# USDA-ARS-GBRU/itsxpress

Measured on AMD Instinct MI355X. Metric: reads/sec trimmed (ITS2, stand-in taxon Tracheophyta for Fungi), higher is better.
Workload: dtype u8+f32

## Files before the change

### include/itsx_hip.h

```cpp
#ifndef ITSX_HIP_H
#define ITSX_HIP_H
#include <stdint.h>

#ifdef __cplusplus
extern "C" {
#endif

#define ITSX_ABI_VERSION 6

enum {
  ITSX_OK            =  0,
  ITSX_E_ARG         = -1,
  ITSX_E_IO          = -2,
  ITSX_E_FORMAT      = -3,
  ITSX_E_DEVICE      = -4,
  ITSX_E_UNSUPPORTED = -5,
  ITSX_E_COLLISION   = -6,
  ITSX_E_NOMEM       = -7
};

typedef struct itsx_ctx itsx_ctx;
typedef struct itsx_stream itsx_stream;
typedef struct itsx_keyset itsx_keyset;
typedef struct itsx_twriter itsx_twriter;
// ... 158 lines not shown
int itsx_keep_pair_records(itsx_ctx *ctx, int on);
int itsx_write_trimmed_paired_samples(itsx_ctx *ctx, const char *const *out1_paths, const char *const *out2_paths, int32_t n_samples,
                                      int compression, int trim_ccs, const char *left_prefix, const char *right_prefix,
                                      const int32_t *start, const int32_t *stop, const int32_t *tlen, int64_t *n_written_per_sample);
int64_t itsx_deflate_block_bytes(void);
int64_t itsx_deflate_bound(int64_t nbytes, int32_t n_ranges);
int itsx_deflate_device(itsx_ctx *ctx, const char *text, int64_t nbytes, const int64_t *bounds, int32_t n_ranges, char *out, int64_t out_cap,
                        int64_t *out_bounds);
int itsx_inflate_device(itsx_ctx *ctx, const char *gz, int64_t nbytes, int64_t *text_len, int64_t *n_members);
int itsx_inflate_fetch(itsx_ctx *ctx, char *out, int64_t out_cap);
int itsx_debug_inflate_host(const char *gz, int64_t nbytes, char *out, int64_t out_cap, int64_t *text_len, int64_t *n_members, int32_t *reason);
int64_t itsx_debug_inflate_candidates(const char *gz, int64_t nbytes, int64_t *positions, int64_t cap);
int itsx_debug_inflate_where(itsx_ctx *ctx, int64_t *where, int64_t n);
int itsx_set_device_inflate(itsx_ctx *ctx, int on);
int itsx_parse_device(itsx_ctx *ctx, const char *text, int64_t nbytes, int keep_qual, int64_t *n_records);
#define ITSX_PARSE_OFF 0
#define ITSX_PARSE_TOFF 1
#define ITSX_PARSE_SEQ 2
#define ITSX_PARSE_QUAL 3
#define ITSX_PARSE_TITLES 4
int itsx_parse_fetch(itsx_ctx *ctx, int32_t plane, int64_t lo, int64_t hi, void *out);
int itsx_debug_parse_host(const char *text, int64_t nbytes, int64_t *off, int64_t *toff, int64_t cap_records, char *seq, char *qual, int64_t cap_bases,
                          char *titles, int64_t cap_titles, int64_t *n_records, int64_t *n_bases, int64_t *n_title_bytes, int32_t *reason, int64_t *bad_record);
int itsx_parse_pairs_device(itsx_ctx *ctx, const char *text1, int64_t nbytes1, const char *text2, int64_t nbytes2, int64_t *n_pairs, int32_t *flags, int64_t *max_total);
int itsx_parse_pairs_fetch(itsx_ctx *ctx, int32_t side, int32_t plane, int64_t lo, int64_t hi, void *out);
int itsx_debug_parse_pairs_host(const char *text1, int64_t nbytes1, const char *text2, int64_t nbytes2, int64_t *off1, int64_t *toff1, char *seq1, char *qual1, char *titles1,
                                int64_t *off2, int64_t *toff2, char *seq2, char *qual2, char *titles2, int64_t cap_records, int64_t cap_bases, int64_t cap_titles,
                                int64_t *n_pairs, int64_t *sizes, int32_t *flags, int64_t *max_total, int32_t *reason, int32_t *bad_side, int64_t *bad_record);
int itsx_debug_pair_pass_host(char *seq, const char *qual, int64_t nbytes, int32_t *flags);
int itsx_set_device_parse(itsx_ctx *ctx, int on);
int itsx_debug_huffman_lengths(const uint32_t *freq, int32_t n, int32_t maxbits, uint8_t *lengths);

int itsx_derep(itsx_ctx *ctx, int strand_both, int minseqlength, int64_t *n_unique);
int itsx_cluster(itsx_ctx *ctx, double id, int strand_both, int64_t *n_unique);
int itsx_cluster_multi(itsx_ctx *ctx, itsx_ctx *const *helpers, int32_t n_helpers, double id, int strand_both, int64_t *n_unique);
int itsx_get_cluster(const itsx_ctx *ctx, double *pct_id, int64_t *order, int64_t *n_order);
int itsx_cluster_samples(itsx_ctx *ctx, double id, int strand_both, int64_t *n_unique);
int itsx_align_clusters(itsx_ctx *ctx, int64_t *n_aligned, float *ms_kernels);
int itsx_get_cluster_cigars(const itsx_ctx *ctx, int64_t *offs , char *text);
int itsx_get_derep(const itsx_ctx *ctx, int64_t *rep_of, int8_t *strand, int64_t *uniq_of);
int itsx_unique_keys(itsx_ctx *ctx, uint64_t seed, uint64_t *fwd, uint64_t *rc);
int itsx_set_active_uniques(itsx_ctx *ctx, const uint8_t *active);
int itsx_get_uniques(const itsx_ctx *ctx, int64_t *seed_read, int64_t *abundance);

int itsx_search(itsx_ctx *ctx, double T, double F1, double F2, double F3);
enum { ITSX_ROWS_FULL = 0, ITSX_ROWS_COMPACT = 1, ITSX_ROWS_LAZY = 2 };
int itsx_set_rows_mode(itsx_ctx *ctx, int mode);
int itsx_set_kept_rows(itsx_ctx *ctx, int on);
int64_t itsx_lazy_pending(const itsx_ctx *ctx);
int itsx_lazy_pending_profiles(const itsx_ctx *ctx, int32_t *flags);
int itsx_lazy_pending_uniques(itsx_ctx *ctx, uint8_t *flags);
int itsx_set_partial_coords(itsx_ctx *ctx, int on);
int itsx_lazy_complete(itsx_ctx *ctx, const int32_t *flags);
int64_t itsx_domz_count(const itsx_ctx *ctx);
int itsx_get_domz(const itsx_ctx *ctx, int64_t *domZ );
int itsx_set_domz(itsx_ctx *ctx, const int64_t *domZ );
int itsx_search_finalize(itsx_ctx *ctx, double domE);
int64_t itsx_num_domains(const itsx_ctx *ctx);
int itsx_get_domains(const itsx_ctx *ctx, itsx_domain *rows );
int itsx_align_domains(itsx_ctx *ctx, int64_t *n_aligned, float *ms_kernels);
int itsx_get_alignments(const itsx_ctx *ctx, itsx_alignment *out );
int64_t itsx_num_pairtraces(const itsx_ctx *ctx);
int itsx_get_pairtraces(const itsx_ctx *ctx, itsx_pairtrace *rows, int64_t row_size);

int itsx_trim_coords(itsx_ctx *ctx, const char *left_prefix, const char *right_prefix,
                     int32_t *start, int32_t *stop, int32_t *tlen, int32_t *in_ddict);
int itsx_rep_coords(itsx_ctx *ctx, const char *left_prefix, const char *right_prefix,
                    int32_t *start, int32_t *stop, int32_t *tlen, int32_t *in_ddict);

int itsx_domz_device(itsx_ctx *ctx, int64_t **d_domz, int64_t *n);
int itsx_trim_coords_device(itsx_ctx *ctx, const char *left_prefix, const char *right_prefix, int32_t **d_rows, int64_t *n_rows);
int itsx_rep_coords_device(itsx_ctx *ctx, const char *left_prefix, const char *right_prefix, int32_t **d_rows, int64_t *n_rows);
int itsx_derep_device(itsx_ctx *ctx, const int32_t **d_rep_of, const int32_t **d_uniq_of, const int8_t **d_strand, const int32_t **d_seed_read);
int itsx_unique_keys128_device(itsx_ctx *ctx, uint64_t seed_a, uint64_t seed_b, int64_t gidx_base, int64_t **d_tuples, int64_t *n_unique);
int itsx_unique_keys128(itsx_ctx *ctx, uint64_t seed_a, uint64_t seed_b, int64_t gidx_base, int64_t *tuples);

int itsx_write_uc(const itsx_ctx *ctx, const char *path);
int itsx_write_rep_fasta(const itsx_ctx *ctx, const char *path);
int itsx_write_domtbl(const itsx_ctx *ctx, const char *path);
int itsx_write_derep_arrays(const char *uc_path, const char *rep_path, int64_t n, const int64_t *rep_of, const int8_t *strand,
                            const int32_t *len, const char *names, const int64_t *name_offsets, const char *seed_bases,
                            const int64_t *seed_offs, int64_t n_seeds);
int itsx_write_domtbl_arrays(const char *path, const itsx_domain *rows, int64_t n_rows, int64_t Z, const int64_t *domz, int32_t n_profiles,
                             const char *prof_names, const int64_t *prof_name_offsets, const int32_t *prof_M, const float *prof_tau,
                             const float *prof_lambda, const char *target_names, const int64_t *target_name_offsets);
int itsx_write_domtbl_arrays_ali(const char *path, const itsx_domain *rows, int64_t n_rows, int64_t Z, const int64_t *domz, int32_t n_profiles,
                                 const char *prof_names, const int64_t *prof_name_offsets, const int32_t *prof_M, const float *prof_tau,
                                 const float *prof_lambda, const char *target_names, const int64_t *target_name_offsets,
                                 const itsx_alignment *ali);
const char *itsx_writers_last_error(void);
int itsx_profile_params(const itsx_ctx *ctx, int i, int32_t *M, float *evparam6);
int itsx_get_unique_seqs(itsx_ctx *ctx, char *bases, int64_t cap, int64_t *offsets);

int itsx_get_read_names(const itsx_ctx *ctx, char *names, int64_t cap, int64_t *offsets);

int itsx_get_stats(const itsx_ctx *ctx, itsx_stats *out, int64_t out_size);
int itsx_release_scratch(itsx_ctx *ctx);
int64_t itsx_switches(const itsx_ctx *ctx, char *buf, int64_t cap);
int64_t itsx_switch_registry(char *buf, int64_t cap);

int itsx_write_trimmed_fastq(const char *seq_path, const char *out_path, int compression, int trim_ccs,
                             const int32_t *start, const int32_t *stop, int64_t n_records,
                             int64_t *n_written, int64_t *total_len);
int itsx_twriter_open(const char *out_path, int compression, int trim_ccs, itsx_twriter **w);
int itsx_twriter_set_mode(itsx_twriter *w, int32_t mode);
int itsx_twriter_set_device(itsx_twriter *w, itsx_ctx *ctx);
// ... 42 lines not shown
```

### itsxpress_amd/_lib.py

```python
import ctypes as C
import os
import subprocess

import numpy as np

_HERE = os.path.dirname(os.path.abspath(__file__))
LIB_PATH = os.path.join(_HERE, "libitsx_hip.so")
ABI_VERSION = 6
_LIB = None


class EngineError(subprocess.SubprocessError):

    def __init__(self, code, message):
        super().__init__("itsx_hip error %d: %s" % (code, message))
        self.code = code
        self.message = message


DOMAIN_DTYPE = np.dtype([("rep", "<i8"), ("prof", "<i4"), ("tlen", "<i4"), ("ienv", "<i4"), ("jenv", "<i4"),
                         ("dom_idx", "<i4"), ("ndom", "<i4"), ("flags", "<i4"), ("envsc", "<f4"),
                         ("domcorrection", "<f4"), ("dombias", "<f4"), ("bitscore", "<f4"), ("lnP", "<f8"),
                         ("seq_score", "<f4"), ("seq_bias", "<f4"), ("seq_reported", "<i4"),
                         ("dom_reported", "<i4")], align=True)
# ... 18 lines not shown
                ("n_uniq_multi_winner", "<i8"), ("n_reads_multi_winner", "<i8"), ("n_uniq_region_cap", "<i8"),
                ("n_reads_region_cap", "<i8"), ("n_mr_clustered", "<i8"), ("n_mr_failed", "<i8"), ("n_mr_envelopes", "<i8"),
                ("ms_ensemble", "<f4"), ("ms_deflate", "<f4"), ("n_mr_distinct", "<i8"), ("n_slab_shrinks", "<i8"), ("ms_vit_kernel", "<f4"), ("n_tw_units_host", "<i4"),
                ("n_mr_fail_kind", "<i8", (8,)), ("n_rows_resident", "<i8"),
                ("lazy", "<i4"), ("n_bound_launches", "<i4"), ("n_lazy_pending_profiles", "<i8"), ("n_lazy_completed", "<i8"), ("n_lazy_completed_profiles", "<i8"), ("n_mr_overflow", "<i8"), ("ms_lazy_complete", "<f4"), ("lazy_bound_maxdiff", "<f4"), ("n_lazy_evaluated", "<i8"), ("n_lazy_round1", "<i8"),
                ("n_lazy_pending", "<i8"), ("n_lazy_reruns", "<i8"), ("bound_rows", "<i8"), ("ms_bound_kernel", "<f4"),
                ("ms_lazy_select", "<f4"),
                ("share_B", "<i4"), ("share_batches", "<i4"), ("share_nodes", "<i8"), ("share_chains", "<i8"), ("msv_rows", "<i8"), ("msv_rows_full", "<i8"),
                ("bound_rows_full", "<i8"), ("n_share_helpers", "<i8"), ("share_mismatch", "<i8"), ("ms_share_build", "<f4"), ("share_frac", "<f4"),
                ("two_sided", "<i4"), ("n_bwd_launches", "<i4"), ("n_joined", "<i8"), ("bwd_chains", "<i8"), ("gamma_nodes", "<i8"), ("bwd_rows", "<i8"),
                ("two_fwd_rows", "<i8"), ("two_bwd_rows", "<i8"), ("two_rows_full", "<i8"), ("join_maxdiff", "<f4"), ("ms_bwd_bound", "<f4"),
                ("n_lazy_topup", "<i8"), ("ms_lazy_topup", "<f4"), ("ms_lazy_topup_stages", "<f4"),
                ("ms_inflate", "<f4"), ("n_inflate_members", "<i4"), ("n_inflate_device", "<i8"), ("n_inflate_declined", "<i8")]
STATS_TAIL_FIELDS = [("ms_parse", "<f4"), ("parse_reserved", "<i4"), ("n_parse_device", "<i8"), ("n_parse_declined", "<i8")]
STATS_DTYPE_ALL = np.dtype(STATS_FIELDS + STATS_TAIL_FIELDS, align=True)
_head = np.dtype(STATS_FIELDS, align=True)
STATS_DTYPE = np.dtype({"names": list(_head.names), "formats": [_head.fields[k][0] for k in _head.names],
                        "offsets": [_head.fields[k][1] for k in _head.names], "itemsize": STATS_DTYPE_ALL.itemsize})

EXPORTS = ["itsx_abi_version", "itsx_last_error", "itsx_create", "itsx_destroy", "itsx_load_profiles_file",
           "itsx_load_profiles_mem", "itsx_profile_name", "itsx_profile_tables", "itsx_set_reads", "itsx_set_reads_view", "itsx_set_reads_device", "itsx_domz_device", "itsx_trim_coords_device",
           "itsx_rep_coords_device", "itsx_derep_device", "itsx_unique_keys128_device",
           "itsx_load_reads_file", "itsx_derep", "itsx_cluster", "itsx_cluster_multi", "itsx_cluster_samples", "itsx_get_cluster", "itsx_get_derep", "itsx_unique_keys", "itsx_set_active_uniques", "itsx_get_uniques",
           "itsx_search", "itsx_get_domz", "itsx_set_domz", "itsx_search_finalize", "itsx_num_domains",
           "itsx_get_domains", "itsx_num_pairtraces", "itsx_get_pairtraces", "itsx_trim_coords",
           "itsx_rep_coords", "itsx_write_uc", "itsx_write_rep_fasta", "itsx_write_domtbl", "itsx_get_stats", "itsx_switches", "itsx_switch_registry", "itsx_release_scratch",
           "itsx_debug_read_hashes", "itsx_debug_read_samples", "itsx_debug_sorted_uniques", "itsx_debug_packed_read", "itsx_debug_detmath", "itsx_debug_logf", "itsx_debug_dust", "itsx_debug_calibrate", "itsx_debug_issue", "itsx_shard_text", "itsx_shard_last_error", "itsx_owner_verdicts",
           "itsx_write_trimmed_fastq", "itsx_write_trimmed_paired", "itsx_trim_last_error",
           "itsx_merge_buffers", "itsx_merge_pairs_files", "itsx_merge_pairs_load", "itsx_merge_tables",
           "itsx_orient_load_db", "itsx_orient", "itsx_orient_apply", "itsx_write_oriented_fastq",
           "itsx_io_read", "itsx_io_free", "itsx_io_codecs", "itsx_fastq_ids",
           "itsx_load_reads_files", "itsx_set_samples", "itsx_num_samples", "itsx_select_sample",
           "itsx_io_parallel_inflates", "itsx_io_cache_clear", "itsx_get_read_names",
           "itsx_set_rows_mode", "itsx_lazy_pending", "itsx_domz_count", "itsx_lazy_pending_profiles", "itsx_lazy_complete",
           "itsx_load_reads_file_shard", "itsx_unique_keys128", "itsx_write_derep_arrays", "itsx_write_domtbl_arrays",
           "itsx_writers_last_error", "itsx_profile_params", "itsx_get_unique_seqs",
           "itsx_load_reads_text", "itsx_stream_open", "itsx_stream_next", "itsx_stream_close", "itsx_stream_last_error", "itsx_stream_records_bound",
           "itsx_stream_open_shared", "itsx_stream_open_threads", "itsx_stream_base", "itsx_stream_progress", "itsx_stream_next_records", "itsx_count_records",
           "itsx_merge_pairs_load_text", "itsx_merge_pair_index", "itsx_merge_pairs_load_files", "itsx_twriter_set_mode", "itsx_write_range",
           "itsx_keyset_create", "itsx_keyset_destroy", "itsx_keyset_size", "itsx_keyset_assign",
           "itsx_twriter_open", "itsx_twriter_text", "itsx_twriter_coords", "itsx_twriter_update", "itsx_twriter_close",
           "itsx_lazy_pending_uniques", "itsx_set_partial_coords", "itsx_set_kept_rows",
           "itsx_keep_records", "itsx_write_trimmed_samples",
           "itsx_keep_pair_records", "itsx_write_trimmed_paired_samples",
           "itsx_deflate_block_bytes", "itsx_deflate_bound", "itsx_deflate_device", "itsx_debug_huffman_lengths",
           "itsx_twriter_set_device",
           "itsx_inflate_device", "itsx_inflate_fetch", "itsx_debug_inflate_host", "itsx_debug_inflate_candidates", "itsx_debug_inflate_where", "itsx_set_device_inflate",
           "itsx_parse_device", "itsx_parse_fetch", "itsx_debug_parse_host", "itsx_set_device_parse",
           "itsx_parse_pairs_device", "itsx_parse_pairs_fetch", "itsx_debug_parse_pairs_host", "itsx_debug_pair_pass_host",
           "itsx_debug_set_domains", "itsx_debug_get_rows",
           "itsx_debug_scan", "itsx_debug_select", "itsx_debug_region_keys", "itsx_debug_lazy_pairs",
           "itsx_set_sample_sharing", "itsx_sample_sharing_info", "itsx_sample_sharing_times", "itsx_debug_sample_classes",
           "itsx_align_domains", "itsx_get_alignments", "itsx_write_domtbl_arrays_ali",
           "itsx_align_clusters", "itsx_get_cluster_cigars"]


def lib():
    global _LIB
    if _LIB is not None:
        return _LIB
    if not os.path.exists(LIB_PATH):
        raise FileNotFoundError(
            "%s not found: build the HIP engine first (python -c 'import __graft_entry__ as g; g.build()' "
            "or make -C itsxpress_amd/csrc). There is no CPU fallback." % LIB_PATH)
    L = C.CDLL(LIB_PATH)
    vp, i32, i64, f64, cp = C.c_void_p, C.c_int, C.c_int64, C.c_double, C.c_char_p
    sig = {
        "itsx_abi_version": (i32, []),
        "itsx_last_error": (cp, [vp]),
        "itsx_create": (vp, [i32, i32]),
        "itsx_destroy": (None, [vp]),
        "itsx_load_profiles_file": (i32, [vp, cp, vp]),
        "itsx_load_profiles_mem": (i32, [vp, cp, i64, vp]),
        "itsx_profile_name": (i32, [vp, i32, vp, i32]),
        "itsx_profile_tables": (i32, [vp, i32, vp, vp, vp, vp]),
        "itsx_set_reads": (i32, [vp, vp, vp, i64, vp, vp]),
        "itsx_set_reads_view": (i32, [vp, vp, vp, i64, vp, vp]),
        "itsx_set_reads_device": (i32, [vp, vp, vp, i64, vp, vp]),
        "itsx_domz_device": (i32, [vp, vp, vp]),
        "itsx_trim_coords_device": (i32, [vp, cp, cp, vp, vp]),
        "itsx_rep_coords_device": (i32, [vp, cp, cp, vp, vp]),
        "itsx_derep_device": (i32, [vp, vp, vp, vp, vp]),
        "itsx_unique_keys128_device": (i32, [vp, C.c_uint64, C.c_uint64, i64, vp, vp]),
        "itsx_load_reads_file": (i32, [vp, cp, vp]),
        "itsx_load_reads_file_shard": (i32, [vp, cp, i32, i32, vp, vp, vp]),
        "itsx_load_reads_text": (i32, [vp, vp, i64, vp]),
        "itsx_stream_open": (i32, [cp, vp]),
        "itsx_stream_next": (i32, [vp, i64, vp, vp, vp]),
        "itsx_stream_close": (i32, [vp, i32]),
        "itsx_stream_records_bound": (i64, [vp]),
        "itsx_stream_open_shared": (i32, [cp, cp, vp, vp]),
        "itsx_stream_open_threads": (i32, [cp, i32, vp]),
        "itsx_stream_base": (vp, [vp]),
        "itsx_stream_progress": (i32, [vp, vp, vp, vp]),
        "itsx_stream_next_records": (i32, [vp, i64, vp, vp, vp, vp]),
        "itsx_count_records": (i64, [vp, i64]),
        "itsx_merge_pairs_load_text": (i32, [vp, vp, i64, vp, i64, i32, f64, i32, vp, vp]),
        "itsx_merge_pair_index": (i32, [vp, vp, i64]),
        "itsx_merge_pairs_load_files": (i32, [vp, vp, vp, vp, i32, i32, f64, i32, vp, vp]),
        "itsx_twriter_set_mode": (i32, [vp, i32]),
        "itsx_write_range": (i32, [cp, vp, i64]),
        "itsx_stream_last_error": (cp, []),
        "itsx_keyset_create": (vp, []),
        "itsx_keyset_destroy": (None, [vp]),
        "itsx_keyset_size": (i64, [vp]),
        "itsx_keyset_assign": (i32, [vp, vp, i64, i32, vp, vp]),
        "itsx_twriter_open": (i32, [cp, i32, i32, vp]),
# ... 8 lines not shown
        "itsx_keep_records": (i32, [vp, i32]),
        "itsx_write_trimmed_samples": (i32, [vp, vp, i32, i32, i32, cp, cp, vp, vp, vp, vp]),
        "itsx_keep_pair_records": (i32, [vp, i32]),
        "itsx_write_trimmed_paired_samples": (i32, [vp, vp, vp, i32, i32, i32, cp, cp, vp, vp, vp, vp]),
        "itsx_deflate_block_bytes": (i64, []),
        "itsx_deflate_bound": (i64, [i64, i32]),
        "itsx_deflate_device": (i32, [vp, vp, i64, vp, i32, vp, i64, vp]),
        "itsx_debug_huffman_lengths": (i32, [vp, i32, i32, vp]),
        "itsx_inflate_device": (i32, [vp, vp, i64, vp, vp]),
        "itsx_inflate_fetch": (i32, [vp, vp, i64]),
        "itsx_debug_inflate_host": (i32, [vp, i64, vp, i64, vp, vp, vp]),
        "itsx_debug_inflate_candidates": (i64, [vp, i64, vp, i64]),
        "itsx_debug_inflate_where": (i32, [vp, vp, i64]),
        "itsx_set_device_inflate": (i32, [vp, i32]),
        "itsx_parse_device": (i32, [vp, vp, i64, i32, vp]),
        "itsx_parse_fetch": (i32, [vp, i32, i64, i64, vp]),
        "itsx_debug_parse_host": (i32, [vp, i64, vp, vp, i64, vp, vp, i64, vp, i64, vp, vp, vp, vp, vp]),
        "itsx_set_device_parse": (i32, [vp, i32]),
        "itsx_parse_pairs_device": (i32, [vp, vp, i64, vp, i64, vp, vp, vp]),
        "itsx_parse_pairs_fetch": (i32, [vp, i32, i32, i64, i64, vp]),
        "itsx_debug_parse_pairs_host": (i32, [vp, i64, vp, i64, vp, vp, vp, vp, vp, vp, vp, vp, vp, vp, i64, i64, i64, vp, vp, vp, vp, vp, vp, vp]),
        "itsx_debug_pair_pass_host": (i32, [vp, vp, i64, vp]),
        "itsx_debug_set_domains": (i32, [vp, vp, i64, vp, i32, i32]),
        "itsx_debug_get_rows": (i64, [vp, vp, i64]),
        "itsx_unique_keys128": (i32, [vp, C.c_uint64, C.c_uint64, i64, vp]),
        "itsx_write_derep_arrays": (i32, [cp, cp, i64, vp, vp, vp, vp, vp, vp, vp, i64]),
        "itsx_write_domtbl_arrays": (i32, [cp, vp, i64, i64, vp, i32, vp, vp, vp, vp, vp, vp, vp]),
        "itsx_write_domtbl_arrays_ali": (i32, [cp, vp, i64, i64, vp, i32, vp, vp, vp, vp, vp, vp, vp, vp]),
        "itsx_writers_last_error": (cp, []),
        "itsx_profile_params": (i32, [vp, i32, vp, vp]),
        "itsx_get_unique_seqs": (i32, [vp, vp, i64, vp]),
        "itsx_derep": (i32, [vp, i32, i32, vp]),
        "itsx_cluster": (i32, [vp, f64, i32, vp]),
        "itsx_cluster_multi": (i32, [vp, vp, i32, f64, i32, vp]),
        "itsx_cluster_samples": (i32, [vp, f64, i32, vp]),
        "itsx_get_cluster": (i32, [vp, vp, vp, vp]),
        "itsx_align_clusters": (i32, [vp, vp, vp]),
        "itsx_get_cluster_cigars": (i32, [vp, vp, vp]),
        "itsx_merge_buffers": (i32, [vp, cp, cp, vp, cp, cp, vp, i64, i32, f64, i32, vp, vp, vp, vp, vp, vp]),
        "itsx_merge_pairs_files": (i32, [vp, cp, cp, cp, i32, f64, i32, vp, vp]),
        "itsx_merge_pairs_load": (i32, [vp, cp, cp, i32, f64, i32, vp, vp]),
        "itsx_merge_tables": (i32, [vp, vp, vp, vp, vp]),
        "itsx_orient_load_db": (i32, [vp, cp, vp]),
        "itsx_orient": (i32, [vp, vp, vp, vp]),
        "itsx_orient_apply": (i32, [vp, vp, vp, vp, vp]),
        "itsx_write_oriented_fastq": (i32, [cp, cp, vp, i64, vp]),
        "itsx_unique_keys": (i32, [vp, C.c_uint64, vp, vp]),
        "itsx_set_active_uniques": (i32, [vp, vp]),
        "itsx_get_derep": (i32, [vp, vp, vp, vp]),
        "itsx_get_uniques": (i32, [vp, vp, vp]),
        "itsx_search": (i32, [vp, f64, f64, f64, f64]),
        "itsx_set_rows_mode": (i32, [vp, i32]),
        "itsx_lazy_pending": (i64, [vp]),
        "itsx_lazy_pending_profiles": (i32, [vp, vp]),
        "itsx_lazy_complete": (i32, [vp, vp]),
        "itsx_domz_count": (i64, [vp]),
        "itsx_get_domz": (i32, [vp, vp]),
        "itsx_set_domz": (i32, [vp, vp]),
        "itsx_search_finalize": (i32, [vp, f64]),
        "itsx_num_domains": (i64, [vp]),
        "itsx_get_domains": (i32, [vp, vp]),
        "itsx_align_domains": (i32, [vp, vp, vp]),
        "itsx_get_alignments": (i32, [vp, vp]),
        "itsx_num_pairtraces": (i64, [vp]),
        "itsx_get_pairtraces": (i32, [vp, vp, i64]),
        "itsx_trim_coords": (i32, [vp, cp, cp, vp, vp, vp, vp]),
        "itsx_rep_coords": (i32, [vp, cp, cp, vp, vp, vp, vp]),
        "itsx_write_uc": (i32, [vp, cp]),
        "itsx_write_rep_fasta": (i32, [vp, cp]),
        "itsx_write_domtbl": (i32, [vp, cp]),
        "itsx_get_stats": (i32, [vp, vp, i64]),
        "itsx_switches": (i64, [vp, vp, i64]),
        "itsx_release_scratch": (i32, [vp]),
        "itsx_switch_registry": (i64, [vp, i64]),
        "itsx_debug_read_hashes": (i32, [vp, vp, vp]),
        "itsx_debug_read_samples": (i32, [vp, vp, vp]),
        "itsx_debug_sorted_uniques": (i32, [vp, vp]),
        "itsx_debug_packed_read": (i32, [vp, i64, vp, vp, vp, vp]),
        "itsx_debug_detmath": (i32, [vp, vp, i64, vp, vp]),
        "itsx_debug_logf": (i32, [vp, vp, i64, vp]),
        "itsx_debug_dust": (i32, [vp, vp]),
        "itsx_debug_scan": (i32, [vp, vp, i64, vp, i32]),
        "itsx_debug_select": (i32, [vp, i32, vp, i64, vp, i32, vp, vp, vp, i32, vp, i64, vp, i64, vp, vp, i32, vp, vp, i64, vp, vp, vp]),
        "itsx_debug_region_keys": (i32, [vp, vp, i64, vp, i64, vp, vp]),
        "itsx_debug_lazy_pairs": (i64, [vp, vp, i64, vp]),
        "itsx_debug_calibrate": (i32, [vp, i32, f64, i32, vp, vp]),
        "itsx_debug_issue": (i32, [vp, i32, i32, i32, vp, vp]),
        "itsx_shard_text": (i32, [C.c_char_p, i32, vp, C.c_char_p, vp, vp]),
        "itsx_shard_last_error": (C.c_char_p, []),
        "itsx_owner_verdicts": (i32, [vp, vp, i64, vp]),
        "itsx_write_trimmed_fastq": (i32, [cp, cp, i32, i32, vp, vp, i64, vp, vp]),
        "itsx_write_trimmed_paired": (i32, [cp, cp, cp, cp, i32, i32, vp, vp, i64, vp, vp, vp, vp]),
        "itsx_trim_last_error": (cp, []),
        "itsx_io_read": (i32, [cp, vp, vp]),
        "itsx_fastq_ids": (i32, [cp, vp, vp, vp]),
        "itsx_io_free": (None, [vp]),
        "itsx_io_codecs": (i32, []),
        "itsx_io_parallel_inflates": (i64, []),
        "itsx_io_cache_clear": (None, []),
        "itsx_get_read_names": (i32, [vp, vp, i64, vp]),
        "itsx_load_reads_files": (i32, [vp, vp, i32, vp]),
        "itsx_set_samples": (i32, [vp, vp, i32]),
        "itsx_num_samples": (i32, [vp]),
        "itsx_select_sample": (i32, [vp, i32]),
        "itsx_set_sample_sharing": (i32, [vp, i32]),
        "itsx_sample_sharing_info": (i32, [vp, vp, vp, vp]),
# ... 12 lines not shown
```

### itsxpress_amd/csrc/engine.hip

```cpp
#include <algorithm>
#include <chrono>
#include <cmath>
#include <cstdio>
#include <cstring>
#include <functional>
#include <map>
#include <memory>
#include <numeric>
#include <atomic>
#include <condition_variable>
#include <mutex>
#include <string_view>
#include <thread>
#include <unordered_map>
#include "detmath.h"
#include "engine.h"
#include "k_api.h"
#include "deflate_codes.h"
#include "inflate_codes.h"
#include "fastq_rec.h"
#include "twriter_dev.h"
#include "cluster_multi.h"
#include "fastq_io.h"
#include "iupac.h"
// ... 343 lines not shown
  bool compact_rows = false; double compact_zmax = 1e9, compact_dome_min = 1e-2, compact_lnp = 0; int compact_ncls = 0;
  DBuf<itsx_domain> w_domscratch; DBuf<int8_t> w_cls; DBuf<unsigned long long> w_bestc; DBuf<int32_t> w_keep, w_keeppos, w_keeptmp;
  int64_t rows_before_compaction = 0;
  int rows_mode = -1;
  bool lazy = false;
  bool domz_exchanged = false;
  int64_t lazy_pending = 0;
  double sF1 = 1e-6, sF3 = 1e-6;
  std::vector<int64_t> domz_ub;
  std::vector<int64_t> domz_loc, domz_ub_loc;
  bool completing = false;
  std::vector<int32_t> h_plist; DBuf<int32_t> d_plist;
  int64_t s_Uc = 0; int s_Lcap = 0;
  DBuf<float> l_fb; DBuf<uint32_t> l_b10, l_thr; DBuf<uint8_t> l_done; DBuf<unsigned long long> l_smask; DBuf<int32_t> l_scnt, l_spos, l_scan, l_has; DBuf<unsigned long long> l_gtop, l_sure;
  DBuf<PairRec> l_pairs; DBuf<int64_t> l_seg, l_zub; DBuf<int32_t> l_pflag; DBuf<uint8_t> l_uflag; bool partial_coords = false; bool kept_rows = false; std::vector<int32_t> lazy_pending_prof;
  std::vector<uint16_t> thr_memo; std::vector<char> thr_memo_have; double thr_memo_F1 = -1.0; int thr_memo_Ppad = 0;
  DBuf<int32_t> w_coords4; DBuf<int64_t> w_keys128; DBuf<uint64_t> w_hf1, w_hr1;
  std::vector<int32_t> h_sorted_active;
  DBuf<LenTables> d_lt;
  std::vector<int64_t> domz;
  std::vector<itsx_domain> h_dom;
  struct AliRow { int32_t prof, dom_idx; int64_t rep; itsx_alignment a; };
  bool have_ali = false; std::vector<AliRow> h_ali;
  void drop_alignments() { have_ali = false; std::vector<AliRow>().swap(h_ali); }
  bool alignments_live() const { return have_ali && have_search && have_final; }
  DBuf<PairRec> w_al_pairs; DBuf<RegionRec> w_al_regions; DBuf<RegionOut> w_al_rout; DBuf<int32_t> w_al_rep; DBuf<WaveDesc> w_al_waves; DBuf<itsx_alignment> w_al_out;
  std::vector<itsx_pairtrace> h_trace;

  DBuf<uint64_t> w_hf, w_hr; DBuf<unsigned long long> w_keys; DBuf<int32_t> w_vals, w_is_seed, w_seed_rank, w_scan_tmp, w_hist, w_cursor, w_tmp2;
  DBuf<uint32_t> w_slot_of; DBuf<unsigned int> w_ncoll;
  DBuf<uint16_t> w_thr, w_res; DBuf<int32_t> w_tjb, w_cnt, w_total, w_rows, w_rcnt, w_rpref, w_scan2, w_b, w_rrows;
  DBuf<int64_t> w_seg_start, w_idx, w_rseg, w_dz, w_counters, w_useg;
  DBuf<int32_t> w_rrep, w_ruq, w_rurank;
  DBuf<WaveDesc> w_waves, w_rw; DBuf<RegionRec> w_raw; DBuf<float> w_slab, w_eslab;
  DBuf<int32_t> w_mrcnt, w_mroff, w_mrlen, w_mrloff, w_mrrows, w_mrulist, w_mrulist2, w_mru; DBuf<int64_t> w_mrrowoff; DBuf<MrRec> w_mr; DBuf<MrOut> w_mrout; DBuf<int64_t> w_n2off; DBuf<float> w_n2sc, w_mrslab;
  DBuf<uint8_t> w_mrscratch; DBuf<WaveDesc> w_mrwaves;
  DBuf<RegionRec> w_pool, w_pool_sorted; DBuf<int32_t> w_pool_k; DBuf<unsigned long long> w_pool_n, w_pool_key; int64_t pool_cap = 0;
  DBuf<int32_t> w_mrsel; DBuf<int64_t> w_mrselrow; DBuf<MrBig> w_mrbig; DBuf<uint8_t> w_mrarena; DBuf<int32_t> w_mrenv; DBuf<WaveDesc> w_mrbigwaves;
  DBuf<int32_t> w_cl, w_cr;
  DBuf<int8_t> w_side; DBuf<unsigned long long> w_bl, w_br; DBuf<int32_t> w_uind, w_us, w_ue, w_ut, w_rs, w_re, w_rt, w_ri, w_uflag;

  struct ShareBatch { int32_t k0, k1; int64_t node0, nnodes; int32_t nsplit; int64_t gnode0, gnnodes; };
  bool share_on = false; int share_B = 32, share_logB = 5, share_maxd = 0;
  DBuf<unsigned long long> sh_tab, sh_mask_s, sh_mask, sh_counters, msv_xb; DBuf<uint8_t> sh_depth_s, sh_depth;
  DBuf<int32_t> sh_src, sh_parent_s, sh_parent, sh_nn_s, sh_nn, sh_node0_s, sh_node0, sh_order, sh_ulen, sh_uorder, sh_inv, sh_flag, sh_pos, sh_bstart, sh_cursor, sh_segk, sh_scan, sh_cuts;
  std::vector<ShareBatch> sh_batches; std::vector<int32_t> sh_segk_h;
  DBuf<uint4> sh_mgslots; size_t sh_mgslots_half = 0;
  DBuf<uint4> sh_mslots; size_t sh_mslots_half = 0, sh_fslots_half = 0; DBuf<uint32_t> sh_pass, sh_need; DBuf<int32_t> sh_real, sh_segflat, sh_segdepth, sh_wc, sh_woff; DBuf<int64_t> sh_bnd;
  DBuf<uint16_t> sh_res_chk; DBuf<float> sh_fb_chk;
  ShareDev sh_dev{};
  std::string switches_at_search;
  struct TopUp { bool valid = false, list_live = false ; int64_t NP = 0; std::vector<int64_t> seg_start; std::vector<int32_t> total; int32_t u0 = 0, Uc = 0; } topup;
  DBuf<unsigned long long> l_zneed, l_zsplit, l_tcnt; DBuf<int32_t> l_slot, l_pslot; DBuf<uint32_t> l_cut;
  std::vector<unsigned long long> h_zneed;
  bool prev_lazy = false; int prev_P = 0; int64_t prev_U = 0, prev_Uc = 0;
  std::vector<int32_t> h_merge_index;
  bool keep_records = false;
  struct Records {
    bool have = false;
    DBuf<uint8_t> seq, qual, titles;
    const uint8_t *seq_p = nullptr;
    DBuf<int64_t> off, toff;
    NameList h_titles;
    void drop() { have = false; seq_p = nullptr; seq.release(); qual.release(); titles.release(); off.release(); toff.release(); h_titles.clear(); }
  } rec;
  bool keep_pair_records = false;
  struct PairRecords {
    bool have = false; int64_t n = 0;
    DBuf<uint8_t> s1, q1, t1, s2, q2, t2;
    DBuf<int64_t> o1, to1, o2, to2;
    DBuf<int32_t> pair_read;
    std::vector<int64_t> pstart;
    void drop()
    {
      have = false; n = 0; pstart.clear(); pair_read.release();
      s1.release(); q1.release(); t1.release(); s2.release(); q2.release(); t2.release(); o1.release(); to1.release(); o2.release(); to2.release();
    }
  } prec;
  DBuf<TrimRec> w_trec2; DBuf<int32_t> w_ttlen;
  DBuf<TrimRec> w_trec; DBuf<int64_t> w_tcnt, w_ttot, w_tblk, w_tfirst, w_tbounds; DBuf<int32_t> w_tstart, w_tstop; DBuf<uint32_t> w_tout;
  DBuf<DeflateBlock> w_dblk; DBuf<uint32_t> w_dtok, w_dtext; DBuf<uint8_t> w_dslots, w_dpacked; DBuf<int32_t> w_dsizes; DBuf<int64_t> w_ddst;
  DBuf<uint8_t> tw_raw; DBuf<int32_t> tw_ls, tw_le; DBuf<int64_t> tw_lblk, tw_qsrc, tw_info;
  std::mutex tw_mu; bool tw_failed = false; float tw_ms_deflate = 0;
  DBuf<uint8_t> inf_gz, inf_text; DBuf<int64_t> inf_counts, inf_base, inf_list, inf_where; DBuf<InflateMember> inf_mem; DBuf<int32_t> inf_status;
  int64_t inf_len = -1, n_inf_device = 0, n_inf_declined = 0; bool device_inflate = false; std::mutex inf_mu;
  DBuf<uint8_t> ps_text, ps_seq, ps_qual, ps_titles; DBuf<int64_t> ps_lblk, ps_nl, ps_blk, ps_off, ps_toff, ps_info;
  int64_t ps_n = -1, ps_nb = 0, ps_nt = 0, n_parse_device = 0, n_parse_declined = 0; bool ps_qual_kept = false, device_parse = false; std::mutex ps_mu;
  struct PairSide { DBuf<uint8_t> seq, qual, titles; DBuf<int64_t> off, toff; int64_t nb = 0, nt = 0; } pp[2];
  int64_t pp_n = -1; DBuf<unsigned long long> pp_info;
  bool two_on = false; int share_maxrd = 0; int32_t Ub = 0; size_t sh_gslots_off = 0;
  DBuf<uint8_t> sh_rdepth_s, sh_rdepth; DBuf<unsigned long long> sh_rmask_s, sh_rmask, sh_keys, sh_keys2;
  DBuf<int32_t> sh_rparent_s, sh_rparent, sh_jlev_s, sh_jown_s, sh_endrow_s, sh_rsteps_s, sh_rnn_s, sh_rnode0_s, sh_endrow, sh_jlev, sh_jsrc, sh_jownb;
  DBuf<int32_t> sh_border_s, sh_invb, sh_bsegk, sh_rnn, sh_rnode0, sh_border, sh_bulen, sh_rsrc, sh_bsteps, sh_vals;
  DBuf<uint8_t> sh_sorttmp;
  std::vector<int32_t> sh_bsegk_h;
  BShareDev sh_bdev{};
  DBuf<uint32_t> sh_needb; DBuf<uint16_t> sh_resb; DBuf<int32_t> sh_cntb, sh_totalb, sh_realb, sh_bsegflat, sh_bsegdepth, sh_bwc, sh_bwoff; DBuf<int64_t> sh_bbnd, sh_bseg_start;
  DBuf<PairRec> sh_bpairs; DBuf<WaveDesc> sh_bwaves;
};

#define CTXCHK(c)                                   \
  if (!(c)) return ITSX_E_ARG;
#define SET_ERR(ctx, code, msg) do { (ctx)->set_error(msg); return (code); } while (0)
#undef HIPCHK
#define HIPCHK(expr)                                                                      \
  do {                                                                                    \
// ... 1695 lines not shown
  hipStream_t st = ctx->st;
  launch_compact_best(d_rows, NR, ctx->w_cls.p, ctx->compact_ncls, ctx->compact_lnp, ctx->w_bestc.p, st);
  HIPCHK(ctx->w_keep.alloc((size_t)NR + 1)); HIPCHK(ctx->w_keeppos.alloc((size_t)NR + 1)); HIPCHK(ctx->w_keeptmp.alloc((size_t)scan_tmp_elems(NR + 1)));
  launch_compact_mark(d_rows, NR, ctx->w_cls.p, ctx->compact_ncls, ctx->compact_lnp, ctx->w_bestc.p, ctx->w_keep.p, st);
  launch_exclusive_scan(ctx->w_keep.p, ctx->w_keeppos.p, NR + 1, ctx->w_keeptmp.p, st);
  int32_t kept = 0;
  HIPCHK(hipMemcpyAsync(&kept, ctx->w_keeppos.p + NR, sizeof(kept), hipMemcpyDeviceToHost, st));
  HIPCHK(hipStreamSynchronize(st));
  DBuf<itsx_domain> &small = *ctx->dom_bufs[di];
  HIPCHK(small.alloc((size_t)std::max<int32_t>(kept, 1), true));
  launch_compact_scatter(d_rows, NR, ctx->w_keep.p, ctx->w_keeppos.p, small.p, st);
  ctx->rows_before_compaction += NR;
  ctx->dom_n[di] = kept;
  return ITSX_OK;
}

static int search_rows_mode(const itsx_ctx *ctx)
{
  int mode = ctx->rows_mode;
  if (mode < 0) {
    mode = ITSX_ROWS_FULL;
    if (sw_get("ITSX_COMPACT_ROWS") && atoi(sw_get("ITSX_COMPACT_ROWS")) != 0) mode = ITSX_ROWS_COMPACT;
    if (const char *e = sw_get("ITSX_ROWS")) mode = !strcmp(e, "lazy") ? ITSX_ROWS_LAZY : !strcmp(e, "compact") ? ITSX_ROWS_COMPACT : ITSX_ROWS_FULL;
  }
  if (mode == ITSX_ROWS_LAZY && sw_get("ITSX_KEEP_TRACE")) mode = ITSX_ROWS_COMPACT;
  return mode;
}

static int search_active(itsx_ctx *ctx, double T, double F1, double F2, double F3)
{
  CTXCHK(ctx);
  if (!ctx->have_derep) SET_ERR(ctx, ITSX_E_ARG, "itsx_search called before itsx_derep / itsx_cluster");
  if (ctx->P <= 0) SET_ERR(ctx, ITSX_E_ARG, "no profiles loaded");
  ctx->F2 = F2; ctx->have_vit = F2 < F1;
  ctx->switches_at_search = sw_report();
  HIPCHK(hipSetDevice(ctx->device));
  hipStream_t st = ctx->st;
  const int P = ctx->P, G = ctx->G, Ppad = G * 64, U = ctx->U_active;
  ctx->T = T;
  ctx->h_dom.clear(); ctx->drop_alignments(); ctx->h_trace.clear(); ctx->trace_sorted = false;
  ctx->domz.assign((size_t)P * ctx->S, 0);
  itsx_stats &S = ctx->stats;
  S.n_pairs = (int64_t)U * P; S.n_past_msv = S.n_past_bias = S.n_past_fwd = S.n_regions = S.n_multidomain = S.n_domains = S.n_domain_overflow = 0;
  S.ms_msv = S.ms_filters = S.ms_domains = S.ms_msv_kernel = S.ms_fwd_kernel = S.ms_bwd_kernel = S.ms_env_kernel = S.ms_bias_kernel = S.ms_decode_kernel = 0; S.n_batches = 0; S.ms_ensemble = 0; S.n_mr_clustered = S.n_mr_distinct = S.n_mr_failed = S.n_mr_envelopes = 0; S.n_slab_shrinks = 0; S.n_mr_overflow = 0; S.ms_vit_kernel = 0; for (int k = 0; k < 8; k++) S.n_mr_fail_kind[k] = 0; S.n_rows_resident = 0; S.msv_cells = 0; S.msv_launches = 0; S.fwd_rows = 0; S.env_rows = 0; S.n_env_unique = 0;
  ctx->npairs_padded = 0; ctx->dom_n.clear(); ctx->trace_u0 = 0; ctx->n_chunks = 0;
  ctx->have_search = true; ctx->have_final = false; ctx->domz_on_device = false; ctx->topup.valid = false; ctx->topup.list_live = false; ctx->injected = false;
  const int mode = search_rows_mode(ctx);
  ctx->compact_rows = mode != ITSX_ROWS_FULL;
  ctx->lazy = mode == ITSX_ROWS_LAZY;
  ctx->lazy_pending = 0; ctx->domz_exchanged = false; ctx->sF1 = F1; ctx->sF3 = F3;
  ctx->domz_ub.assign((size_t)P * ctx->S, 0);
  if (ctx->compact_rows)
    for (auto &b : ctx->dom_bufs) if (b && b->cap * sizeof(itsx_domain) > ((size_t)256 << 20)) b->release();
  S.lazy = ctx->lazy; S.n_lazy_evaluated = S.n_lazy_round1 = S.n_lazy_pending = S.n_lazy_reruns = 0; S.n_lazy_completed = S.n_lazy_completed_profiles = S.n_lazy_pending_profiles = 0; S.ms_lazy_complete = 0; S.lazy_bound_maxdiff = 0; S.ms_bound_kernel = S.ms_lazy_select = 0; S.bound_rows = 0; S.n_bound_launches = 0; S.n_lazy_topup = 0; S.ms_lazy_topup = 0; S.ms_lazy_topup_stages = 0;
  if (ctx->compact_rows && U > 0) { const int rc = compact_setup(ctx); if (rc != ITSX_OK) return rc; }
  if (U == 0) return ITSX_OK;

  const int Lcap = ctx->Lmax + 1;
  std::vector<LenTables> lt((size_t)Lcap);
  std::vector<int32_t> tjb((size_t)Lcap, 0);
  std::vector<char> present((size_t)Lcap, 0);
  int64_t cells_active = 0;
  {
    const int32_t Ua = ctx->U, Uact = ctx->U_active;
    const int Th = Ua >= (1 << 19) ? std::max(1, std::min(8, itsx_io::io_threads())) : 1;
    std::vector<std::vector<char>> pres((size_t)Th); std::vector<int64_t> csum((size_t)Th, 0);
    on_threads(Th, [&](int t) {
      std::vector<char> &pr = pres[(size_t)t]; pr.assign((size_t)Lcap, 0);
      int64_t c = 0;
      for (int64_t u = (int64_t)Ua * t / Th, hi = (int64_t)Ua * (t + 1) / Th; u < hi; u++) {
        const int32_t L = ctx->h_len[ctx->h_seed_read[(size_t)u]];
        pr[(size_t)L] = 1;
        if (Uact == Ua) c += L;
      }
      csum[(size_t)t] = c;
    });
    for (int t = 0; t < Th; t++) { cells_active += csum[(size_t)t]; for (int L = 0; L < Lcap; L++) present[(size_t)L] |= pres[(size_t)t][(size_t)L]; }
    if (Uact != Ua) for (int32_t u : ctx->h_sorted_active) cells_active += ctx->h_len[ctx->h_seed_read[(size_t)u]];
  }
  for (int L = 0; L < Lcap; L++) {
    LenTables &t = lt[L]; memset(&t, 0, sizeof(t));
    if (L == 0) continue;
    const float p1 = (float)L / (float)(L + 1);
    t.p1 = p1;
    t.nullsc = (float)((double)(float)L * log((double)p1) + log(1. - (double)p1));
    t.bias_a = (float)L * logf(p1);
    t.bias_b = logf((float)(1. - (double)p1));
    t.lognn3 = log((double)((float)L / (float)(L + 3)));
    t.tjb = host_tjb_b(L);
    tjb[L] = t.tjb;
    {
      const double n = (double)L;
      const double c = 1.0 + (2.0 * log(2.0 * (n + 3.0) / (3.0 * (n + 2.0))) + n * log((n + 3.0) / (n + 2.0))) / 0.69314718055994529;
      const double margin = std::max(0.02, 6.0 * (n + (double)MMAX) * 5.9604644775390625e-8 / 0.69314718055994529);
      t.lazy_c = nextafterf((float)(c + margin), 1e30f);
    }
    { const float w = roundf((float)(500.0 / 0.69314718055994529) * logf((2.0f + 1.0f) / ((float)L + 2.0f + 1.0f)));
      t.vmove = (w >= 32767.0f) ? 32767 : (w <= -32768.0f) ? -32768 : (int)w; }
  }
  if (ctx->thr_memo_F1 != F1 || ctx->thr_memo_Ppad != Ppad) { ctx->thr_memo.clear(); ctx->thr_memo_have.clear(); ctx->thr_memo_F1 = F1; ctx->thr_memo_Ppad = Ppad; }
  if (ctx->thr_memo_have.size() < (size_t)Lcap) { ctx->thr_memo_have.resize((size_t)Lcap, 0); ctx->thr_memo.resize((size_t)Lcap * Ppad, 257); }
  std::vector<uint16_t> thr((size_t)Lcap * Ppad, 257);
  for (int L = 1; L < Lcap; L++) {
    if (!present[L]) continue;
    if (ctx->thr_memo_have[(size_t)L]) { memcpy(&thr[(size_t)L * Ppad], &ctx->thr_memo[(size_t)L * Ppad], (size_t)Ppad * sizeof(uint16_t)); continue; }
    ctx->thr_memo_have[(size_t)L] = 2;
    for (int p = 0; p < P; p++) {
// ... 198 lines not shown
  if (n_uniques_shared) *n_uniques_shared = ctx->sc.n_shared;
  if (n_rows_expanded) *n_rows_expanded = ctx->sc.n_expanded;
  return ITSX_OK;
}
int itsx_sample_sharing_times(const itsx_ctx *ctx, float *ms_classes, float *ms_expand)
{
  CTXCHK(ctx && ctx->have_search);
  if (ms_classes) *ms_classes = ctx->sc.ms_classes;
  if (ms_expand) *ms_expand = ctx->sc.ms_expand;
  return ITSX_OK;
}
int itsx_debug_sample_classes(itsx_ctx *ctx, int32_t *class_of, int64_t n)
{
  CTXCHK(ctx && ctx->have_search && (class_of || n == 0));
  if (ctx->sc.n_classes <= 0) SET_ERR(ctx, ITSX_E_ARG, "itsx_debug_sample_classes: the last search built no score classes (itsx_sample_sharing_info reports 0)");
  if (n != (int64_t)ctx->U) SET_ERR(ctx, ITSX_E_ARG, "itsx_debug_sample_classes: n is not the number of uniques");
  HIPCHK(hipSetDevice(ctx->device));
  if (n) { HIPCHK(hipMemcpyAsync(class_of, ctx->sc_class_of.p, (size_t)n * 4, hipMemcpyDeviceToHost, ctx->st)); HIPCHK(hipStreamSynchronize(ctx->st)); }
  return ITSX_OK;
}

struct PairList {
  PairRec *pairs = nullptr; PairOut *pout = nullptr;
  int64_t NP = 0;
  std::vector<int64_t> seg_start;
  std::vector<int32_t> total;
  const int64_t *d_seg_start = nullptr;
};

static int build_waves(itsx_ctx *ctx, const PairList &pl, std::vector<WaveDesc> &waves, std::vector<char> &wgeneric, std::vector<int32_t> &rows)
{
  hipStream_t st = ctx->st;
  const int P = ctx->P;
  waves.clear(); wgeneric.clear();
  for (int pass = 0; pass < 2; pass++)
    for (int p = 0; p < P; p++) {
      if ((int)ctx->generic_q[p] != pass) continue;
      for (int64_t k = 0; k < pl.total[(size_t)p]; k += 64) {
        WaveDesc w{}; w.prof = p; w.first = pl.seg_start[(size_t)p] + k; w.count = (int32_t)std::min<int64_t>(64, pl.total[(size_t)p] - k);
        waves.push_back(w); wgeneric.push_back((char)pass);
      }
    }
  const int NW = (int)waves.size();
  DBuf<WaveDesc> &d_waves = ctx->w_waves; DBuf<int32_t> &d_rows = ctx->w_rows;
  HIPCHK(upload(d_waves, waves, st)); HIPCHK(d_rows.alloc((size_t)std::max(NW, 1)));
  rows.assign((size_t)NW, 0);
  if (NW == 0) return ITSX_OK;
  hipLaunchKernelGGL(k_wave_rows_pairs, dim3((NW + 255) / 256), dim3(256), 0, st, d_waves.p, NW, pl.pairs, d_rows.p);
  HIPCHK(hipMemcpyAsync(rows.data(), d_rows.p, (size_t)NW * 4, hipMemcpyDeviceToHost, st));
  HIPCHK(hipStreamSynchronize(st));
  return ITSX_OK;
}

static int domain_pipeline(itsx_ctx *ctx, const PairList &pl, const int32_t *d_sorted, double T, double F1, double F3, const std::function<int()> *next_msv)
{
  hipStream_t st = ctx->st;
  const int P = ctx->P;
  itsx_stats &S = ctx->stats;
  const int64_t NP = pl.NP;
  const size_t di = ctx->dom_n.size();
  ctx->dom_n.push_back(0);
  while (ctx->dom_bufs.size() <= di) ctx->dom_bufs.emplace_back(new DBuf<itsx_domain>());
  DBuf<itsx_domain> &d_dom = ctx->compact_rows ? ctx->w_domscratch : *ctx->dom_bufs[di];
  if (NP == 0) return ITSX_OK;
  StageTimer tm_list(st);
  std::vector<WaveDesc> waves; std::vector<char> wgeneric; std::vector<int32_t> rows;
  { const int rc = build_waves(ctx, pl, waves, wgeneric, rows); if (rc != ITSX_OK) return rc; }
  const int NW = (int)waves.size();
  DBuf<WaveDesc> &d_waves = ctx->w_waves;
  S.ms_msv += tm_list.stop();

  if (ctx->slab_gb <= 0.0) {
    ctx->slab_gb = 16.0;
    size_t fr = 0, tot = 0;
    if (hipMemGetInfo(&fr, &tot) == hipSuccess) ctx->slab_gb = std::min(64.0, std::max(1.0, (double)fr / (double)(1ull << 30) / 4.0));
  }
  double slab_gb = ctx->slab_gb;
  if (const char *e = sw_get("ITSX_SLAB_GB")) slab_gb = std::max(0.25, atof(e));
  {
    size_t fr = 0, tot = 0;
    if (hipMemGetInfo(&fr, &tot) == hipSuccess) {
      const double room = ((double)fr / 4.0 + (double)ctx->w_slab.cap * 4.0) / (double)(1ull << 30);
      if (slab_gb > room) { slab_gb = std::max(0.0625, room); S.n_slab_shrinks++; }
    }
  }
  const int64_t row_bytes = 12 * 64 * 4;
  int64_t budget_rows = (int64_t)(slab_gb * (1 << 30)) / row_bytes;
  static const bool adapt = !(sw_get("ITSX_SLAB_ADAPT") && atoi(sw_get("ITSX_SLAB_ADAPT")) == 0);
  if (adapt && !sw_get("ITSX_SLAB_GB")) {
    int64_t total_rows = 0;
    for (int w = 0; w < NW; w++) total_rows += rows[(size_t)w];
    const int64_t floor_rows = ((int64_t)4 << 30) / row_bytes, have_rows = (int64_t)(ctx->w_slab.cap / (12 * 64));
    const int64_t want_rows = std::max(total_rows / 8 + 1, floor_rows);
    budget_rows = std::min(budget_rows, 2 * have_rows >= want_rows ? have_rows : want_rows);
  }
  DBuf<RegionRec> &d_raw = ctx->w_raw;
  HIPCHK(d_raw.alloc((size_t)NP * MAXDOM));
  if (ctx->pool_cap <= 0) ctx->pool_cap = 1 << 16;
  RegionPoolView pv{nullptr, nullptr, 0};
 pool_retry:
  HIPCHK(ctx->w_pool.alloc((size_t)ctx->pool_cap)); HIPCHK(ctx->w_pool_k.alloc((size_t)ctx->pool_cap)); HIPCHK(ctx->w_pool_n.alloc(2));
  HIPCHK(hipMemsetAsync(ctx->w_pool_n.p, 0, 2 * sizeof(unsigned long long), st));
  const itsx_stats stats_before = S;
  {
    StageTimer tm(st);
    struct Batch { int w0, w1; int64_t r; };
    std::vector<Batch> batches;
// ... 55 lines not shown
    for (size_t bi = 0; bi < batches.size(); bi++) {
      const Batch &bt = batches[bi];
      const int w0 = bt.w0, w1 = bt.w1;
      a.slab_plane = bt.r * 6 * 64;
      const bool more = bi + 1 < batches.size();
      if (ctx->have_vit) { const size_t t = lazy.begin(&S.ms_vit_kernel); launch_vit(va, w1 - w0, w0, st); lazy.end(t); }
      { const size_t t = lazy.begin(&S.ms_fwd_kernel); launch_filters_fwd(a, w1 - w0, w0, wgeneric[w0], st); lazy.end(t); }
      { const size_t t = lazy.begin(&S.ms_bwd_kernel); launch_bwd_decode(a, w1 - w0, w0, wgeneric[w0], st); lazy.end(t); }
      if (more && overlap) {
        HIPCHK(hipEventRecord(ctx->ev_a, st)); HIPCHK(hipStreamWaitEvent(ctx->st2, ctx->ev_a, 0));
        bias_batch(batches[bi + 1], ctx->st2, lazy2);
        HIPCHK(hipEventRecord(ctx->ev_b, ctx->st2));
      }
      { const size_t t = lazy.begin(&S.ms_decode_kernel); launch_decode(a, w1 - w0, w0, st); lazy.end(t); }
      if (more && overlap) HIPCHK(hipStreamWaitEvent(st, ctx->ev_b, 0));
      else if (more) bias_batch(batches[bi + 1], st, lazy);
      for (int w = w0; w < w1; w++) S.fwd_rows += (int64_t)(rows[w] - 1) * waves[w].count;
      S.n_batches++;
    }
    lazy2.collect();
    lazy.collect();
    S.ms_filters += tm.stop();
  }
  {
    unsigned long long pn = 0;
    HIPCHK(hipMemcpyAsync(&pn, ctx->w_pool_n.p, sizeof(pn), hipMemcpyDeviceToHost, st));
    HIPCHK(hipStreamSynchronize(st));
    if ((int64_t)pn > ctx->pool_cap) {
      while (ctx->pool_cap < (int64_t)pn) ctx->pool_cap *= 2;
      const float keep_ms = S.ms_filters;
      S = stats_before; S.ms_filters = keep_ms; S.n_slab_shrinks++;
      goto pool_retry;
    }
    if (pn > 0) {
      std::vector<RegionRec> hr((size_t)pn); std::vector<int32_t> hk((size_t)pn);
      HIPCHK(hipMemcpyAsync(hr.data(), ctx->w_pool.p, (size_t)pn * sizeof(RegionRec), hipMemcpyDeviceToHost, st));
      HIPCHK(hipMemcpyAsync(hk.data(), ctx->w_pool_k.p, (size_t)pn * 4, hipMemcpyDeviceToHost, st));
      HIPCHK(hipStreamSynchronize(st));
      std::vector<size_t> ord((size_t)pn);
      std::iota(ord.begin(), ord.end(), (size_t)0);
      auto key = [&](size_t i) { return ((unsigned long long)(uint32_t)hr[i].pair << 24) | (unsigned long long)(uint32_t)hk[i]; };
      std::sort(ord.begin(), ord.end(), [&](size_t x, size_t y) { return key(x) < key(y); });
      std::vector<RegionRec> sr((size_t)pn); std::vector<unsigned long long> sk((size_t)pn);
      for (size_t i = 0; i < (size_t)pn; i++) { sr[i] = hr[ord[i]]; sk[i] = key(ord[i]); }
      HIPCHK(upload(ctx->w_pool_sorted, sr, st)); HIPCHK(upload(ctx->w_pool_key, sk, st));
      HIPCHK(hipStreamSynchronize(st));
      pv.rec = ctx->w_pool_sorted.p; pv.key = ctx->w_pool_key.p; pv.n = (int64_t)pn;
    }
  }
  if (next_msv) { const int rc = (*next_msv)(); if (rc != ITSX_OK) return rc; }
  StageTimer tm_dom(st);
  int64_t NMR = 0;
  const bool ensemble = !(sw_get("ITSX_NO_ENSEMBLE") && atoi(sw_get("ITSX_NO_ENSEMBLE")) != 0);
  if (ensemble) {
    DBuf<int32_t> &mrcnt = ctx->w_mrcnt, &mroff = ctx->w_mroff, &stmp = ctx->w_scan2;
    HIPCHK(mrcnt.alloc((size_t)NP + 2)); HIPCHK(mroff.alloc((size_t)NP + 2)); HIPCHK(stmp.alloc((size_t)scan_tmp_elems(NP + 2)));
    launch_mr_count(pl.pout, d_raw.p, pv, NP, mrcnt.p, st);
    launch_exclusive_scan(mrcnt.p, mroff.p, NP + 1, stmp.p, st);
    int32_t tot = 0;
    HIPCHK(hipMemcpyAsync(&tot, mroff.p + NP, 4, hipMemcpyDeviceToHost, st));
    HIPCHK(hipStreamSynchronize(st));
    NMR = tot;
    if (NMR > 0) {
      StageTimer tm_e(st);
      static_assert(sizeof(MrRec) == sizeof(RegionRec), "MrRec is handed to the region memoisation kernels as a RegionRec");
      HIPCHK(ctx->w_mr.alloc((size_t)NMR));
      launch_mr_fill(pl.pout, d_raw.p, pv, NP, mroff.p, ctx->w_mr.p, st);
      DBuf<unsigned long long> &rkeys = ctx->w_keys; DBuf<int32_t> &rvals = ctx->w_vals; DBuf<uint32_t> &rslot = ctx->w_slot_of;
      DBuf<int32_t> &rrep = ctx->w_rrep, &ruq = ctx->w_ruq, &rurank = ctx->w_rurank, &rscan = ctx->w_scan_tmp;
      const uint64_t tsize = region_table_size(NMR);
      HIPCHK(rkeys.alloc(tsize)); HIPCHK(rvals.alloc(tsize)); HIPCHK(rslot.alloc((size_t)NMR + 1));
      HIPCHK(rrep.alloc((size_t)NMR + 1)); HIPCHK(ruq.alloc((size_t)NMR + 1)); HIPCHK(rurank.alloc((size_t)NMR + 1)); HIPCHK(rscan.alloc((size_t)scan_tmp_elems(NMR + 1)));
      HIPCHK(hipMemsetAsync(rkeys.p, 0, tsize * sizeof(unsigned long long), st));
      HIPCHK(hipMemsetAsync(rvals.p, 0x7f, tsize * sizeof(int32_t), st));
      HIPCHK(hipMemsetAsync(ruq.p, 0, ((size_t)NMR + 1) * sizeof(int32_t), st));
      const RegionRec *mr_as_regions = (const RegionRec *)ctx->w_mr.p;
      launch_region_keys(ctx->rd, mr_as_regions, NMR, pl.pairs, d_sorted, ctx->d_seed_read.p, rkeys.p, rvals.p, tsize - 1, rslot.p, st);
      launch_region_resolve(ctx->rd, mr_as_regions, NMR, pl.pairs, d_sorted, ctx->d_seed_read.p, rvals.p, rslot.p, rrep.p, ruq.p, st);
      launch_exclusive_scan(ruq.p, rurank.p, NMR + 1, rscan.p, st);
      int32_t NU = 0;
      HIPCHK(hipMemcpyAsync(&NU, rurank.p + NMR, 4, hipMemcpyDeviceToHost, st));
      HIPCHK(hipStreamSynchronize(st));
      DBuf<int32_t> &ulist0 = ctx->w_mrulist, &ulist = ctx->w_mrulist2, &ulen = ctx->w_mrlen, &newpos = ctx->w_mrloff, &mru = ctx->w_mru;
      HIPCHK(ulist0.alloc((size_t)NU + 1)); HIPCHK(ulist.alloc((size_t)NU + 1)); HIPCHK(ulen.alloc((size_t)NU + 2)); HIPCHK(newpos.alloc((size_t)NU + 2)); HIPCHK(mru.alloc((size_t)NMR + 1));
      launch_mr_ulist(NMR, ctx->w_mr.p, rrep.p, ruq.p, rurank.p, ulist0.p, ulen.p, mru.p, st);
      std::vector<int32_t> hlen((size_t)NU), ord((size_t)NU), hpos((size_t)NU);
      HIPCHK(hipMemcpyAsync(hlen.data(), ulen.p, (size_t)NU * 4, hipMemcpyDeviceToHost, st));
      HIPCHK(hipStreamSynchronize(st));
      std::iota(ord.begin(), ord.end(), 0);
      std::stable_sort(ord.begin(), ord.end(), [&](int32_t x, int32_t y) { return hlen[(size_t)x] < hlen[(size_t)y]; });
      std::vector<int64_t> hn2((size_t)NU + 1, 0), hrow((size_t)NU + 1, 0);
      for (int32_t x = 0; x < NU; x++) {
        const int32_t o = ord[(size_t)x];
        hpos[(size_t)o] = x;
        hn2[(size_t)x + 1] = hn2[(size_t)x] + hlen[(size_t)o];
        hrow[(size_t)x + 1] = hrow[(size_t)x] + hlen[(size_t)o] + 1;
      }
      HIPCHK(hipMemcpyAsync(newpos.p, hpos.data(), (size_t)NU * 4, hipMemcpyHostToDevice, st));
      launch_mr_reorder(NU, NMR, newpos.p, ulist0.p, ulist.p, mru.p, st);
      HIPCHK(upload(ctx->w_n2off, hn2, st)); HIPCHK(upload(ctx->w_mrrowoff, hrow, st));
      HIPCHK(ctx->w_mrout.alloc((size_t)NU)); HIPCHK(ctx->w_n2sc.alloc((size_t)hn2[(size_t)NU] + 1));
      static const int lanes_long = sw_get("ITSX_MR_LONG_LANES") ? std::max(1, std::min(MR_LANES, atoi(sw_get("ITSX_MR_LONG_LANES")))) : MR_LANES_LONG;
      static const double frac_long = sw_get("ITSX_MR_LONG_FRAC") ? atof(sw_get("ITSX_MR_LONG_FRAC")) : MR_LONG_FRAC;
      const int64_t n_long = std::min<int64_t>(NU, (int64_t)(frac_long * (double)NU));
      const int64_t waves_target = sw_get("ITSX_MR_WAVES") ? atoll(sw_get("ITSX_MR_WAVES")) : 4096;
      const int lanes_norm = waves_target <= 0 ? MR_LANES : (int)std::max<int64_t>(2, std::min<int64_t>(MR_LANES, (NU + waves_target - 1) / waves_target));
      std::vector<WaveDesc> mw;
// ... 90 lines not shown
              WaveDesc d{}; d.prof = -1; d.first = (int64_t)(x - x0); d.count = (int32_t)std::min<size_t>(MR_LANES_LONG, x1 - x);
              d.rows = hlen[(size_t)ord[(size_t)sel[x + d.count - 1]]] + 1;
              bw.push_back(d);
            }
            std::vector<int32_t> selb(sel.begin() + x0, sel.begin() + x1);
            HIPCHK(upload(ctx->w_mrsel, selb, st)); HIPCHK(upload(ctx->w_mrselrow, srow, st)); HIPCHK(upload(ctx->w_mrbig, big, st)); HIPCHK(upload(ctx->w_mrbigwaves, bw, st));
            if ((size_t)rows * MRV * 4 > ctx->w_mrslab.cap) HIPCHK(ctx->w_mrslab.alloc((size_t)rows * MRV * 4));
            HIPCHK(ctx->w_mrarena.alloc((size_t)arena));
            MrArgs mb{};
            mb.rd = ctx->rd; mb.sorted_uniq = d_sorted; mb.seed_read = ctx->d_seed_read.p; mb.prof = ctx->d_prof.p; mb.pairs = pl.pairs;
            mb.mr = ctx->w_mr.p; mb.ulist = ulist.p; mb.u0 = 0; mb.waves = ctx->w_mrbigwaves.p; mb.slab = (float4 *)ctx->w_mrslab.p;
            mb.rowoff = ctx->w_mrrowoff.p; mb.rowoff0 = 0; mb.n2off = ctx->w_n2off.p; mb.n2sc = ctx->w_n2sc.p; mb.out = ctx->w_mrout.p;
            mb.scratch = nullptr; mb.sel = ctx->w_mrsel.p; mb.sel_rowoff = ctx->w_mrselrow.p; mb.big = ctx->w_mrbig.p; mb.arena = ctx->w_mrarena.p; mb.envpool = ctx->w_mrenv.p;
            launch_mr_ensemble_big(mb, (int)bw.size(), st);
            x0 = x1;
          }
        }
      }
      S.ms_ensemble += tm_e.stop();
      HIPCHK(hipGetLastError());
      S.n_mr_clustered += NMR; S.n_mr_distinct += NU;
    }
  }
  DBuf<int32_t> &d_rcnt = ctx->w_rcnt, &d_rpref = ctx->w_rpref, &d_scan_tmp = ctx->w_scan2;
  HIPCHK(d_rcnt.alloc((size_t)NP + 1)); HIPCHK(d_rpref.alloc((size_t)NP + 1)); HIPCHK(d_scan_tmp.alloc((size_t)scan_tmp_elems(NP + 1)));
  HIPCHK(hipMemsetAsync(d_rcnt.p, 0, ((size_t)NP + 1) * 4, st));
  RegionListArgs rl{};
  rl.pout = pl.pout; rl.raw = d_raw.p; rl.pv = pv; rl.npairs = NP;
  if (NMR > 0) { rl.mr_off = ctx->w_mroff.p; rl.mr_u = ctx->w_mru.p; rl.mrout = ctx->w_mrout.p; rl.envpool = ctx->w_mrenv.p; }
  {
    DBuf<int64_t> &d_c = ctx->w_counters;
    HIPCHK(d_c.alloc(16));
    HIPCHK(hipMemsetAsync(d_c.p, 0, 16 * sizeof(int64_t), st));
    launch_region_list_count(rl, d_rcnt.p, (unsigned long long *)d_c.p, st);
    int64_t hc[10] = {0};
    HIPCHK(hipMemcpyAsync(hc, d_c.p, sizeof(hc), hipMemcpyDeviceToHost, st));
    HIPCHK(hipStreamSynchronize(st));
    S.n_mr_failed += hc[0]; S.n_mr_envelopes += hc[1];
    for (int k = 0; k < 8; k++) S.n_mr_fail_kind[k] += hc[2 + k];
  }
  launch_exclusive_scan(d_rcnt.p, d_rpref.p, NP + 1, d_scan_tmp.p, st);
  std::vector<int32_t> bound((size_t)P + 1);
  {
    DBuf<int64_t> &d_idx = ctx->w_idx; DBuf<int32_t> &d_b = ctx->w_b;
    HIPCHK(upload(d_idx, pl.seg_start, st)); HIPCHK(d_b.alloc((size_t)P + 1));
    hipLaunchKernelGGL(k_gather_i32, dim3((P + 1 + 255) / 256), dim3(256), 0, st, d_rpref.p, d_idx.p, P + 1, d_b.p);
    HIPCHK(hipMemcpyAsync(bound.data(), d_b.p, ((size_t)P + 1) * 4, hipMemcpyDeviceToHost, st));
    HIPCHK(hipStreamSynchronize(st));
  }
  std::vector<int64_t> rseg((size_t)P + 1, 0);
  std::vector<int32_t> rtotal((size_t)P);
  for (int p = 0; p < P; p++) { rtotal[p] = bound[p + 1] - bound[p]; rseg[p + 1] = rseg[p] + ((int64_t)rtotal[p] + 63) / 64 * 64; S.n_domains += rtotal[p]; }
  const int64_t NR = rseg[P];
  ctx->dom_n[di] = NR;
  HIPCHK(ctx->d_pair_region0.alloc((size_t)NP));
  HIPCHK(ctx->d_regions.alloc((size_t)std::max<int64_t>(NR, 1)));
  HIPCHK(d_dom.alloc((size_t)std::max<int64_t>(NR, 1)));
  HIPCHK(hipMemsetAsync(d_dom.p, 0xFF, (size_t)std::max<int64_t>(NR, 1) * sizeof(itsx_domain), st));
  if (NR > 0) {
    DBuf<int64_t> &d_rseg = ctx->w_rseg;
    HIPCHK(upload(d_rseg, rseg, st));
    launch_region_offsets(NP, pl.pairs, d_rpref.p, pl.d_seg_start, d_rseg.p, ctx->d_pair_region0.p, st);
    HIPCHK(hipMemsetAsync(ctx->d_regions.p, 0xFF, (size_t)NR * sizeof(RegionRec), st));
    launch_region_list_fill(rl, ctx->d_pair_region0.p, ctx->d_regions.p, st);
    DBuf<unsigned long long> &rkeys = ctx->w_keys; DBuf<int32_t> &rvals = ctx->w_vals; DBuf<uint32_t> &rslot = ctx->w_slot_of;
    DBuf<int32_t> &rrep = ctx->w_rrep, &ruq = ctx->w_ruq, &rurank = ctx->w_rurank, &rscan = ctx->w_scan_tmp;
    const uint64_t tsize = region_table_size(NR);
    HIPCHK(rkeys.alloc(tsize)); HIPCHK(rvals.alloc(tsize)); HIPCHK(rslot.alloc((size_t)NR + 1));
    HIPCHK(rrep.alloc((size_t)NR + 1)); HIPCHK(ruq.alloc((size_t)NR + 1)); HIPCHK(rurank.alloc((size_t)NR + 1));
    HIPCHK(rscan.alloc((size_t)scan_tmp_elems(NR + 1))); HIPCHK(ctx->d_upos.alloc((size_t)NR + 1));
    HIPCHK(hipMemsetAsync(rkeys.p, 0, tsize * sizeof(unsigned long long), st));
    HIPCHK(hipMemsetAsync(rvals.p, 0x7f, tsize * sizeof(int32_t), st));
    HIPCHK(hipMemsetAsync(ruq.p, 0, ((size_t)NR + 1) * sizeof(int32_t), st));
    launch_region_keys(ctx->rd, ctx->d_regions.p, NR, pl.pairs, d_sorted, ctx->d_seed_read.p, rkeys.p, rvals.p, tsize - 1, rslot.p, st);
    launch_region_resolve(ctx->rd, ctx->d_regions.p, NR, pl.pairs, d_sorted, ctx->d_seed_read.p, rvals.p, rslot.p, rrep.p, ruq.p, st);
    launch_exclusive_scan(ruq.p, rurank.p, NR + 1, rscan.p, st);
    std::vector<int32_t> ub((size_t)P + 1);
    {
      DBuf<int64_t> &d_idx = ctx->w_idx; DBuf<int32_t> &d_b = ctx->w_b;
      HIPCHK(upload(d_idx, rseg, st)); HIPCHK(d_b.alloc((size_t)P + 1));
      hipLaunchKernelGGL(k_gather_i32, dim3((P + 1 + 255) / 256), dim3(256), 0, st, rurank.p, d_idx.p, P + 1, d_b.p);
      HIPCHK(hipMemcpyAsync(ub.data(), d_b.p, ((size_t)P + 1) * 4, hipMemcpyDeviceToHost, st));
      HIPCHK(hipStreamSynchronize(st));
    }
    std::vector<int64_t> useg((size_t)P + 1, 0);
    std::vector<int32_t> utotal((size_t)P);
    for (int p = 0; p < P; p++) { utotal[p] = ub[p + 1] - ub[p]; useg[p + 1] = useg[p] + ((int64_t)utotal[p] + 63) / 64 * 64; S.n_env_unique += utotal[p]; }
    const int64_t NU = useg[P];
    DBuf<int64_t> &d_useg = ctx->w_useg;
    HIPCHK(upload(d_useg, useg, st));
    HIPCHK(ctx->d_ulist.alloc((size_t)std::max<int64_t>(NU, 1))); HIPCHK(ctx->d_rout.alloc((size_t)std::max<int64_t>(NU, 1)));
    HIPCHK(hipMemsetAsync(ctx->d_rout.p, 0, (size_t)std::max<int64_t>(NU, 1) * sizeof(RegionOut), st));
    launch_region_upos(NR, ctx->d_regions.p, pl.pairs, ruq.p, rurank.p, d_rseg.p, d_useg.p, ctx->d_upos.p, ctx->d_ulist.p, st);
    launch_region_upos_follow(NR, rrep.p, ruq.p, ctx->d_upos.p, st);
    std::vector<WaveDesc> rw; std::vector<char> rgen;
    for (int pass = 0; pass < 2; pass++)
      for (int p = 0; p < P; p++) {
        if ((int)ctx->generic_q[p] != pass) continue;
        for (int64_t k = 0; k < utotal[p]; k += 64) {
          WaveDesc w{}; w.prof = p; w.first = useg[p] + k; w.count = (int32_t)std::min<int64_t>(64, utotal[p] - k);
          rw.push_back(w); rgen.push_back((char)pass);
        }
      }
    const int NRW = (int)rw.size();
    DBuf<WaveDesc> &d_rw = ctx->w_rw; DBuf<int32_t> &d_rrows = ctx->w_rrows;
    HIPCHK(upload(d_rw, rw, st)); HIPCHK(d_rrows.alloc((size_t)NRW));
    hipLaunchKernelGGL(k_wave_rows_regions, dim3((NRW + 255) / 256), dim3(256), 0, st, d_rw.p, NRW, ctx->d_ulist.p, d_rrows.p);
    std::vector<int32_t> rrows((size_t)NRW);
    HIPCHK(hipMemcpyAsync(rrows.data(), d_rrows.p, (size_t)NRW * 4, hipMemcpyDeviceToHost, st));
    HIPCHK(hipStreamSynchronize(st));
    const int64_t erow_bytes = 104 * 64 * 4;
    int64_t ebudget = (int64_t)(slab_gb * (1 << 30)) / erow_bytes;
    LazyTimers elazy(st);
    DBuf<float> &d_eslab = ctx->w_eslab; int64_t ealloc = (int64_t)(d_eslab.cap / (104 * 64));
    if (adapt && !sw_get("ITSX_SLAB_GB")) {
      int64_t total_rows = 0;
      for (int w = 0; w < NRW; w++) total_rows += rrows[(size_t)w];
      ebudget = std::min(ebudget, std::max(std::max(total_rows / 4 + 1, ((int64_t)2 << 30) / erow_bytes), ealloc));
    }
    int w0 = 0;
    while (w0 < NRW) {
      int w1 = w0; int64_t r = 0;
      while (w1 < NRW && rgen[w1] == rgen[w0] && (w1 == w0 || r + rrows[w1] <= ebudget)) { rw[w1].slab = r; rw[w1].rows = rrows[w1]; r += rrows[w1]; w1++; }
      if (r > ealloc) {
        if (d_eslab.alloc((size_t)r * 104 * 64) != hipSuccess) {
          (void)hipGetLastError();
          ealloc = 0;
          if (w1 - w0 <= 1) SET_ERR(ctx, ITSX_E_NOMEM, "no device memory left for the envelope slab of a single wave");
          ebudget = std::max<int64_t>(r / 2, rrows[(size_t)w0]);
          S.n_slab_shrinks++;
          continue;
        }
        ealloc = r;
      }
      HIPCHK(hipMemcpyAsync(d_rw.p + w0, rw.data() + w0, (size_t)(w1 - w0) * sizeof(WaveDesc), hipMemcpyHostToDevice, st));
      EnvArgs a{};
      a.rd = ctx->rd; a.sorted_uniq = d_sorted; a.seed_read = ctx->d_seed_read.p; a.prof = ctx->d_prof.p; a.lt = ctx->d_lt.p;
      a.pairs = pl.pairs; a.regions = ctx->d_ulist.p; a.rout = ctx->d_rout.p; a.waves = d_rw.p; a.slab = d_eslab.p;
      { const size_t t = elazy.begin(&S.ms_env_kernel); launch_envelopes(a, w1 - w0, w0, rgen[w0], st); elazy.end(t); }
      for (int w = w0; w < w1; w++) S.env_rows += (int64_t)(rrows[w] - 1) * rw[w].count;
      w0 = w1;
    }
    ScoreArgs sa{};
    sa.rd = ctx->rd; sa.sorted_uniq = d_sorted; sa.seed_read = ctx->d_seed_read.p; sa.prof = ctx->d_prof.p; sa.lt = ctx->d_lt.p;
    sa.flogsum = ctx->d_flogsum.p; sa.pairs = pl.pairs; sa.pout = pl.pout; sa.regions = ctx->d_regions.p; sa.rout = ctx->d_rout.p;
    sa.pair_region0 = ctx->d_pair_region0.p; sa.upos = ctx->d_upos.p; sa.dom = d_dom.p; sa.npairs = NP; sa.T = T;
    if (NMR > 0) { sa.mr = ctx->w_mr.p; sa.mr_u = ctx->w_mru.p; sa.mrout = ctx->w_mrout.p; sa.n2off = ctx->w_n2off.p; sa.n2sc = ctx->w_n2sc.p; sa.mr_off = ctx->w_mroff.p; }
    sa.domz = ctx->d_domz32.p; sa.usample = ctx->dev_usample(); sa.P = ctx->P;
    launch_score(sa, st);
    if (ctx->compact_rows) {
      { const int rc = compact_segment(ctx, d_dom.p, NR, di); if (rc != ITSX_OK) return rc; }
    }
  }
  S.ms_domains += tm_dom.stop();
  {
    DBuf<int64_t> &d_c = ctx->w_counters;
    HIPCHK(d_c.alloc(8));
    HIPCHK(hipMemsetAsync(d_c.p, 0, 8 * sizeof(int64_t), st));
    hipLaunchKernelGGL(k_pair_counters, dim3((unsigned)std::min<int64_t>(4096, (NP + 255) / 256)), dim3(256), 0, st, pl.pout, NP, (unsigned long long *)d_c.p);
    int64_t hc[8];
    HIPCHK(hipMemcpyAsync(hc, d_c.p, sizeof(hc), hipMemcpyDeviceToHost, st));
    HIPCHK(hipStreamSynchronize(st));
    S.n_past_bias += hc[0]; S.n_past_fwd += hc[1]; S.n_regions += hc[2]; S.n_domain_overflow += hc[3]; S.n_multidomain += hc[4];
  }
  HIPCHK(hipGetLastError());
  return ITSX_OK;
}


namespace itsx {
__global__ void k_dbg_group_count(const PairRec *__restrict__ pairs, int64_t NP, const unsigned long long *__restrict__ smask, const int8_t *__restrict__ cls, int ncls, unsigned long long *__restrict__ cnt)
{
  const int64_t i = (int64_t)blockIdx.x * blockDim.x + threadIdx.x;
  if (i >= NP || !((smask[i >> 6] >> (i & 63)) & 1ull)) return;
  const PairRec pr = pairs[i];
  if (pr.prof < 0) return;
  atomicAdd(&cnt[(size_t)pr.useq * ncls + cls[pr.prof]], 1ull);
}
__global__ void k_dbg_group_hist(const unsigned long long *__restrict__ cnt, int64_t ng, unsigned long long *__restrict__ hist)
{
  const int64_t i = (int64_t)blockIdx.x * blockDim.x + threadIdx.x;
  if (i >= ng) return;
  const unsigned long long c = cnt[i];
  const int b = c <= 4 ? (int)c : c <= 8 ? 5 : c <= 16 ? 6 : 7;
  atomicAdd(&hist[b], 1ull);
  if (c > 1) atomicAdd(&hist[8], c - 1);
  if (c > 2) atomicAdd(&hist[9], c - 2);
}
}

static int select_compact(itsx_ctx *ctx, const PairRec *pairs, int64_t NP, int P, const std::vector<int64_t> &seg_start, const int64_t *d_seg_start, PairList &sub, int64_t &nsel)
{
  hipStream_t st = ctx->st;
  const int64_t nch = (NP + 63) >> 6;
  launch_exclusive_scan(ctx->l_scnt.p, ctx->l_spos.p, nch + 1, ctx->l_scan.p, st);
  std::vector<int32_t> bound((size_t)P + 1);
  {
    DBuf<int64_t> &d_idx = ctx->w_idx; DBuf<int32_t> &d_b = ctx->w_b;
    HIPCHK(upload(d_idx, seg_start, st)); HIPCHK(d_b.alloc((size_t)P + 1));
    hipLaunchKernelGGL(k_gather_chunk_i32, dim3((P + 1 + 255) / 256), dim3(256), 0, st, ctx->l_spos.p, d_idx.p, P + 1, d_b.p);
    HIPCHK(hipMemcpyAsync(bound.data(), d_b.p, ((size_t)P + 1) * 4, hipMemcpyDeviceToHost, st));
    HIPCHK(hipStreamSynchronize(st));
  }
  sub.seg_start.assign((size_t)P + 1, 0); sub.total.assign((size_t)P, 0);
  for (int p = 0; p < P; p++) { sub.total[(size_t)p] = bound[(size_t)p + 1] - bound[(size_t)p]; sub.seg_start[(size_t)p + 1] = sub.seg_start[(size_t)p] + ((int64_t)sub.total[(size_t)p] + 63) / 64 * 64; }
  sub.NP = sub.seg_start[(size_t)P];
  nsel = (int64_t)bound[(size_t)P] - bound[0];
  if (sub.NP == 0) return ITSX_OK;
  HIPCHK(ctx->l_pairs.alloc((size_t)sub.NP)); HIPCHK(ctx->d_pout.alloc((size_t)sub.NP));
  HIPCHK(hipMemsetAsync(ctx->l_pairs.p, 0xFF, (size_t)sub.NP * sizeof(PairRec), st));
  HIPCHK(hipMemsetAsync(ctx->d_pout.p, 0, (size_t)sub.NP * sizeof(PairOut), st));
  HIPCHK(upload(ctx->l_seg, sub.seg_start, st));
  launch_lazy_scatter(pairs, NP, ctx->l_smask.p, ctx->l_spos.p, d_seg_start, ctx->l_seg.p, ctx->l_pairs.p, st);
  sub.pairs = ctx->l_pairs.p; sub.pout = ctx->d_pout.p; sub.d_seg_start = ctx->l_seg.p;
  return ITSX_OK;
}
static int select_alloc(itsx_ctx *ctx, int64_t NP)
{
  if (NP & 63) SET_ERR(ctx, ITSX_E_DEVICE, "lazy stage: the pair list is not padded to whole chunks of 64");
  const int64_t nch = NP >> 6;
  HIPCHK(ctx->l_smask.alloc((size_t)nch + 1)); HIPCHK(ctx->l_scnt.alloc((size_t)nch + 2)); HIPCHK(ctx->l_spos.alloc((size_t)nch + 2));
  HIPCHK(ctx->l_scan.alloc((size_t)scan_tmp_elems(nch + 2)));
  return ITSX_OK;
}

static int lazy_rounds(itsx_ctx *ctx, const PairList &pl, const int32_t *d_sorted, int32_t u0, int32_t Uc, double T, double F1, double F3, const std::function<int()> *next_msv)
{
  hipStream_t st = ctx->st;
  const int P = ctx->P, ncls = ctx->compact_ncls;
  itsx_stats &S = ctx->stats;
  const int64_t NP = pl.NP;
  HIPCHK(ctx->l_fb.alloc((size_t)NP + 1)); HIPCHK(ctx->l_b10.alloc((size_t)NP + 1)); HIPCHK(ctx->l_done.alloc((size_t)NP + 1));
  { const int rc = select_alloc(ctx, NP); if (rc != ITSX_OK) return rc; }
  HIPCHK(ctx->l_gtop.alloc((size_t)Uc * ncls + 1));
  HIPCHK(hipMemsetAsync(ctx->l_done.p, 0, (size_t)NP + 1, st));
  HIPCHK(hipMemsetAsync(ctx->l_gtop.p, 0, ((size_t)Uc * ncls + 1) * sizeof(unsigned long long), st));
  if (ctx->share_on) {
    const int maxd = ctx->share_maxd, DS = maxd + 1;
    const bool two = ctx->two_on;
    std::vector<int32_t> segflat, segdepth, segbatch;
    for (size_t bi = 0; bi < ctx->sh_batches.size(); bi++) {
      const auto &b = ctx->sh_batches[bi];
      if (b.k0 < u0 || b.k0 >= u0 + Uc) continue;
      for (int d = 0; d < DS; d++) { segflat.push_back(ctx->sh_segk_h[bi * SHARE_SEGS + d] - u0); segdepth.push_back(d); segbatch.push_back((int32_t)bi); }
    }
    const int nseg = (int)segdepth.size();
    segflat.push_back(Uc);
    if ((int64_t)nseg * P + 1 >= (1ll << 31)) SET_ERR(ctx, ITSX_E_UNSUPPORTED, "prefix sharing: too many (batch, depth, profile) segments in one chunk");
    HIPCHK(upload(ctx->sh_segflat, segflat, st)); HIPCHK(upload(ctx->sh_segdepth, segdepth, st, 1)); HIPCHK(upload(ctx->w_rcnt, pl.total, st));
    HIPCHK(ctx->sh_bnd.alloc((size_t)(nseg + 1) * P)); HIPCHK(ctx->sh_wc.alloc((size_t)nseg * P + 2)); HIPCHK(ctx->sh_woff.alloc((size_t)nseg * P + 2));
    HIPCHK(ctx->sh_scan.alloc((size_t)scan_tmp_elems((int64_t)nseg * P + 2)));
    launch_share_bounds(pl.pairs, pl.d_seg_start, ctx->w_rcnt.p, ctx->sh_segflat.p, nseg, P, ctx->sh_bnd.p, st);
    launch_share_wcount(ctx->sh_bnd.p, nseg, P, ctx->sh_wc.p, st);
    launch_exclusive_scan(ctx->sh_wc.p, ctx->sh_woff.p, (int64_t)nseg * P + 1, ctx->sh_scan.p, st);
    std::vector<int32_t> woff((size_t)nseg * P + 1);
    HIPCHK(hipMemcpyAsync(woff.data(), ctx->sh_woff.p, woff.size() * 4, hipMemcpyDeviceToHost, st));
    HIPCHK(hipStreamSynchronize(st));
    const int NW = woff.back();
    HIPCHK(ctx->w_waves.alloc((size_t)std::max(NW, 1))); HIPCHK(ctx->w_counters.alloc(512));
    HIPCHK(hipMemsetAsync(ctx->w_counters.p, 0, 512 * sizeof(int64_t), st));
    const bool dump = sw_get("ITSX_PASSA_DUMP") != nullptr;
    const bool share_check = sw_get("ITSX_SHARE_CHECK") && atoi(sw_get("ITSX_SHARE_CHECK")) != 0;
    const bool want_check = sw_get("ITSX_LAZY_CHECK_BOUND") || share_check;
    const bool need_rows = dump || (want_check && !two);
    const int Wn = (P + 31) / 32;
    launch_share_rows(Uc, Wn, ctx->sh_need.p, ctx->sh_ulen.p + u0, two ? ctx->sh_endrow.p + u0 : nullptr, ctx->sh_segflat.p, nseg, ctx->sh_segdepth.p, ctx->share_B, 0,
// ... 417 lines not shown
  if (NP == 0) { S.ms_msv += tm_list.stop(); ctx->dom_n.push_back(0); while (ctx->dom_bufs.size() < ctx->dom_n.size()) ctx->dom_bufs.emplace_back(new DBuf<itsx_domain>()); return ITSX_OK; }
  if (NP >= (1ll << 31)) SET_ERR(ctx, ITSX_E_UNSUPPORTED, "more than 2^31 surviving (representative, profile) pairs");
  DBuf<int64_t> &d_seg_start = ctx->w_seg_start;
  HIPCHK(upload(d_seg_start, seg_start, st));
  ctx->topup.list_live = false;
  HIPCHK(ctx->d_pairs.alloc((size_t)NP));
  if (!lazy_now) {
    HIPCHK(ctx->d_pout.alloc((size_t)NP));
    HIPCHK(hipMemsetAsync(ctx->d_pout.p, 0, (size_t)NP * sizeof(PairOut), st));
  }
  launch_pair_fill(d_res.p, P, U, nchunks, d_cnt.p, d_seg_start.p, d_total.p, d_ulen, ctx->d_pairs.p, st);
  S.ms_msv += tm_list.stop();
  const int64_t zub_scale = sw_get("ITSX_LAZY_ZUB_SCALE") ? std::max<int64_t>(1, atoll(sw_get("ITSX_LAZY_ZUB_SCALE"))) : 1;
  if (!ctx->completing)
    for (int p = 0; p < P; p++)
      for (int32_t sm = 0; sm < ctx->S; sm++) ctx->domz_ub_loc[(size_t)sm * P + p] += (int64_t)real[p] * zub_scale;
  PairList pl;
  pl.pairs = ctx->d_pairs.p; pl.pout = lazy_now ? nullptr : ctx->d_pout.p; pl.NP = NP; pl.seg_start = seg_start; pl.total = total; pl.d_seg_start = d_seg_start.p;
  const std::function<int()> next_msv = [&]() -> int {
    const bool msv_overlap = !(sw_get("ITSX_MSV_OVERLAP") && atoi(sw_get("ITSX_MSV_OVERLAP")) == 0);
    if (msv_overlap && ctx->next_u0 >= 0 && ctx->st2 && !ctx->keep_trace) {
      if (!ctx->ev_msv0) {
        HIPCHK(hipEventCreate(&ctx->ev_msv0)); HIPCHK(hipEventCreate(&ctx->ev_msv1));
        HIPCHK(hipEventCreateWithFlags(&ctx->ev_c, hipEventDisableTiming));
      }
      HIPCHK(hipEventRecord(ctx->ev_c, st)); HIPCHK(hipStreamWaitEvent(ctx->st2, ctx->ev_c, 0));
      HIPCHK(hipEventRecord(ctx->ev_msv0, ctx->st2));
      msv_for(ctx->next_u0, ctx->next_U, ctx->st2, sw_get("ITSX_MSV_PAD") ? atoi(sw_get("ITSX_MSV_PAD")) : 40000);
      HIPCHK(hipEventRecord(ctx->ev_msv1, ctx->st2));
      ctx->msv_pre_u0 = ctx->next_u0;
    }
    return ITSX_OK;
  };
  if (lazy_now) return lazy_rounds(ctx, pl, d_sorted, u0, U, T, F1, F3, &next_msv);
  { const int rc = domain_pipeline(ctx, pl, d_sorted, T, F1, F3, &next_msv); if (rc != ITSX_OK) return rc; }
  if (ctx->keep_trace) { const int rc = append_traces(ctx); if (rc != ITSX_OK) return rc; }
  return ITSX_OK;
}

int itsx_set_rows_mode(itsx_ctx *ctx, int mode)
{
  CTXCHK(ctx);
  if (mode < -1 || mode > ITSX_ROWS_LAZY) SET_ERR(ctx, ITSX_E_ARG, "itsx_set_rows_mode: mode must be -1 (environment), 0 (full), 1 (compact) or 2 (lazy)");
  ctx->rows_mode = mode;
  return ITSX_OK;
}
int64_t itsx_lazy_pending(const itsx_ctx *ctx) { return ctx ? ctx->lazy_pending : -1; }
int itsx_lazy_pending_profiles(const itsx_ctx *ctx, int32_t *flags)
{
  CTXCHK(ctx && flags && ctx->have_search);
  for (int p = 0; p < ctx->P; p++) flags[p] = (ctx->lazy && (size_t)p < ctx->lazy_pending_prof.size()) ? (ctx->lazy_pending_prof[(size_t)p] != 0) : 0;
  return ITSX_OK;
}
int itsx_set_partial_coords(itsx_ctx *ctx, int on) { CTXCHK(ctx); ctx->partial_coords = on != 0; return ITSX_OK; }
int itsx_set_kept_rows(itsx_ctx *ctx, int on) { CTXCHK(ctx); if (ctx->kept_rows != (on != 0)) { ctx->h_dom.clear(); ctx->drop_alignments(); } ctx->kept_rows = on != 0; return ITSX_OK; }
int itsx_lazy_pending_uniques(itsx_ctx *ctx, uint8_t *flags)
{
  CTXCHK(ctx && flags && ctx->have_search);
  if (ctx->U <= 0) return ITSX_OK;
  if (!ctx->lazy || !ctx->have_final || ctx->l_uflag.n < (size_t)ctx->U) { memset(flags, 0, (size_t)ctx->U); return ITSX_OK; }
  HIPCHK(hipSetDevice(ctx->device));
  HIPCHK(hipMemcpyAsync(flags, ctx->l_uflag.p, (size_t)ctx->U, hipMemcpyDeviceToHost, ctx->st));
  HIPCHK(hipStreamSynchronize(ctx->st));
  return ITSX_OK;
}
int itsx_lazy_complete(itsx_ctx *ctx, const int32_t *flags)
{
  CTXCHK(ctx && flags && ctx->have_search);
  if (!ctx->lazy) SET_ERR(ctx, ITSX_E_ARG, "itsx_lazy_complete: the last search was not a lazy one");
  if (ctx->injected) SET_ERR(ctx, ITSX_E_ARG, "itsx_lazy_complete: the row table was handed in (itsx_debug_set_domains): there are no pairs to evaluate");
  HIPCHK(hipSetDevice(ctx->device));
  hipStream_t st = ctx->st;
  const int P = ctx->P;
  ctx->h_plist.clear();
  for (int p = 0; p < P; p++) if (flags[p]) ctx->h_plist.push_back(p);
  if (ctx->h_plist.empty() || ctx->U_active == 0) return ITSX_OK;
  StageTimer tm(st);
  HIPCHK(upload(ctx->d_plist, ctx->h_plist, st));
  std::vector<int32_t> dz32((size_t)P * ctx->S, 0);
  HIPCHK(hipMemcpyAsync(dz32.data(), ctx->d_domz32.p, dz32.size() * 4, hipMemcpyDeviceToHost, st));
  HIPCHK(hipStreamSynchronize(st));
  for (int32_t sm = 0; sm < ctx->S; sm++) for (int p : ctx->h_plist) dz32[(size_t)sm * P + p] = 0;
  HIPCHK(hipMemcpyAsync(ctx->d_domz32.p, dz32.data(), dz32.size() * 4, hipMemcpyHostToDevice, st));
  ctx->completing = true;
  const int rc = run_chunks(ctx, ctx->T, ctx->sF1, ctx->sF3);
  ctx->completing = false;
  if (rc != ITSX_OK) { ctx->have_search = false; return rc; }
  HIPCHK(hipMemcpyAsync(dz32.data(), ctx->d_domz32.p, dz32.size() * 4, hipMemcpyDeviceToHost, st));
  HIPCHK(hipStreamSynchronize(st));
  for (int32_t sm = 0; sm < ctx->S; sm++)
    for (int p : ctx->h_plist) {
      const size_t z = (size_t)sm * P + p;
      ctx->domz_loc[z] = ctx->domz_ub_loc[z] = dz32[z];
      if (!ctx->domz_exchanged) ctx->domz[z] = ctx->domz_ub[z] = dz32[z];
    }
  ctx->have_final = false; ctx->drop_alignments();
  ctx->stats.n_lazy_completed_profiles += (int64_t)ctx->h_plist.size();
  ctx->stats.n_rows_resident = 0;
  for (int64_t r : ctx->dom_n) ctx->stats.n_rows_resident += r;
  ctx->stats.ms_lazy_complete += tm.stop();
  return ITSX_OK;
}

int itsx_get_domz(const itsx_ctx *ctx, int64_t *domZ)
{
  CTXCHK(ctx && domZ && ctx->have_search);
// ... 7 lines not shown
  for (size_t p = 0; p < ctx->domz.size(); p++) ctx->domz[p] = domZ[p];
  if (ctx->lazy) for (size_t p = 0; p < ctx->domz_ub.size(); p++) ctx->domz_ub[p] = domZ[ctx->domz.size() + p];
  ctx->domz_on_device = false; ctx->domz_exchanged = true;
  ctx->drop_alignments();
  return ITSX_OK;
}
int64_t itsx_domz_count(const itsx_ctx *ctx) { return ctx ? (int64_t)ctx->domz.size() * (ctx->lazy ? 2 : 1) : -1; }

int itsx_domz_device(itsx_ctx *ctx, int64_t **d_domz, int64_t *n)
{
  CTXCHK(ctx && d_domz && ctx->have_search);
  HIPCHK(hipSetDevice(ctx->device));
  const size_t m = ctx->domz.size(), mm = m * (ctx->lazy ? 2 : 1);
  HIPCHK(ctx->d_domz64.alloc(std::max<size_t>(mm, 1)));
  if (m) HIPCHK(hipMemcpyAsync(ctx->d_domz64.p, ctx->domz_loc.data(), m * 8, hipMemcpyHostToDevice, ctx->st));
  if (m && ctx->lazy) HIPCHK(hipMemcpyAsync(ctx->d_domz64.p + m, ctx->domz_ub_loc.data(), m * 8, hipMemcpyHostToDevice, ctx->st));
  HIPCHK(hipStreamSynchronize(ctx->st));
  ctx->domz_on_device = true; ctx->domz_exchanged = true;
  *d_domz = ctx->d_domz64.p;
  if (n) *n = (int64_t)mm;
  return ITSX_OK;
}

int itsx_debug_set_domains(itsx_ctx *ctx, const itsx_domain *rows, int64_t n_rows, const int64_t *seg_rows, int32_t n_segs, int mode)
{
  CTXCHK(ctx);
  if (!ctx->have_derep) SET_ERR(ctx, ITSX_E_ARG, "itsx_debug_set_domains called before itsx_derep / itsx_cluster");
  if (ctx->P <= 0) SET_ERR(ctx, ITSX_E_ARG, "no profiles loaded");
  if (mode < ITSX_ROWS_FULL || mode > ITSX_ROWS_LAZY) SET_ERR(ctx, ITSX_E_ARG, "itsx_debug_set_domains: mode must be 0 (full), 1 (compact) or 2 (lazy)");
  if (n_rows < 0 || n_segs < 0 || (n_rows > 0 && !rows) || (n_segs > 0 && !seg_rows)) SET_ERR(ctx, ITSX_E_ARG, "itsx_debug_set_domains: missing arrays");
  int64_t sum = 0;
  for (int32_t s = 0; s < n_segs; s++) {
    if (seg_rows[s] < 0 || seg_rows[s] > (int64_t)INT32_MAX - 4096) SET_ERR(ctx, ITSX_E_ARG, "itsx_debug_set_domains: segment " + std::to_string(s) + " has a row count outside [0, 2^31 - 4096]");
    sum += seg_rows[s];
  }
  if (sum != n_rows) SET_ERR(ctx, ITSX_E_ARG, "itsx_debug_set_domains: the segments hold " + std::to_string(sum) + " rows, " + std::to_string(n_rows) + " were given");
  for (int64_t i = 0; i < n_rows; i++) {
    const itsx_domain &d = rows[i];
    if (d.dom_idx < 0) continue;
    if (d.rep < 0 || d.rep >= ctx->U) SET_ERR(ctx, ITSX_E_ARG, "itsx_debug_set_domains: row " + std::to_string(i) + " names representative " + std::to_string(d.rep) + " of " + std::to_string(ctx->U));
    if (d.prof < 0 || d.prof >= ctx->P) SET_ERR(ctx, ITSX_E_ARG, "itsx_debug_set_domains: row " + std::to_string(i) + " names profile " + std::to_string(d.prof) + " of " + std::to_string(ctx->P));
  }
  HIPCHK(hipSetDevice(ctx->device));
  hipStream_t st = ctx->st;
  const size_t m = (size_t)ctx->P * ctx->S;
  ctx->switches_at_search = sw_report();
  ctx->searched_holders = false; ctx->h_dom.clear(); ctx->drop_alignments(); ctx->h_trace.clear(); ctx->trace_sorted = false;
  ctx->domz.assign(m, 0); ctx->domz_ub.assign(m, 0); ctx->domz_loc.assign(m, 0); ctx->domz_ub_loc.assign(m, 0);
  ctx->npairs_padded = 0; ctx->dom_n.clear(); ctx->n_chunks = n_segs;
  ctx->have_search = false; ctx->have_final = false; ctx->domz_on_device = false; ctx->topup.valid = false; ctx->topup.list_live = false; ctx->injected = true;
  ctx->compact_rows = mode != ITSX_ROWS_FULL; ctx->lazy = mode == ITSX_ROWS_LAZY;
  ctx->lazy_pending = 0; ctx->domz_exchanged = false; ctx->lazy_pending_prof.clear();
  itsx_stats &S = ctx->stats;
  S.lazy = ctx->lazy; S.n_domains = 0; S.n_lazy_pending = S.n_lazy_reruns = S.n_lazy_topup = S.n_lazy_completed = S.n_lazy_completed_profiles = S.n_lazy_pending_profiles = 0;
  for (int64_t i = 0; i < n_rows; i++) S.n_domains += rows[i].dom_idx >= 0;
  HIPCHK(ctx->d_domz32.alloc(std::max<size_t>(m, 1)));
  HIPCHK(hipMemsetAsync(ctx->d_domz32.p, 0, std::max<size_t>(m, 1) * 4, st));
  if (ctx->compact_rows) { const int rc = compact_setup(ctx); if (rc != ITSX_OK) return rc; }
  int64_t o = 0;
  for (int32_t s = 0; s < n_segs; s++) {
    const size_t di = ctx->dom_n.size();
    const int64_t NR = seg_rows[s];
    ctx->dom_n.push_back(0);
    while (ctx->dom_bufs.size() <= di) ctx->dom_bufs.emplace_back(new DBuf<itsx_domain>());
    if (NR > 0) {
      DBuf<itsx_domain> &d_dom = mode == ITSX_ROWS_COMPACT ? ctx->w_domscratch : *ctx->dom_bufs[di];
      HIPCHK(d_dom.alloc((size_t)NR));
      HIPCHK(hipMemcpyAsync(d_dom.p, rows + o, (size_t)NR * sizeof(itsx_domain), hipMemcpyHostToDevice, st));
      HIPCHK(hipStreamSynchronize(st));
      ctx->dom_n[di] = NR;
      if (mode == ITSX_ROWS_COMPACT) { const int rc = compact_segment(ctx, d_dom.p, NR, di); if (rc != ITSX_OK) return rc; }
    }
    o += NR;
  }
  HIPCHK(hipStreamSynchronize(st));
  HIPCHK(hipGetLastError());
  S.n_rows_resident = 0;
  for (int64_t r : ctx->dom_n) S.n_rows_resident += r;
  ctx->have_search = true;
  return ITSX_OK;
}

int64_t itsx_debug_get_rows(itsx_ctx *ctx, itsx_domain *rows, int64_t cap)
{
  if (!ctx || !ctx->have_search) return ITSX_E_ARG;
  int64_t n = 0;
  for (int64_t r : ctx->dom_n) n += std::max<int64_t>(r, 0);
  if (!rows || cap < n) return n;
  HIPCHK(hipSetDevice(ctx->device));
  HIPCHK(hipStreamSynchronize(ctx->st));
  int64_t o = 0;
  for (size_t c = 0; c < ctx->dom_n.size(); c++) {
    if (ctx->dom_n[c] <= 0) continue;
    HIPCHK(hipMemcpy(rows + o, ctx->dom_bufs[c]->p, (size_t)ctx->dom_n[c] * sizeof(itsx_domain), hipMemcpyDeviceToHost));
    o += ctx->dom_n[c];
  }
  return n;
}

static int finalize_lazy(itsx_ctx *ctx, double domE)
{
  hipStream_t st = ctx->st;
  const size_t m = ctx->domz.size();
  DBuf<int64_t> &d_dz = ctx->domz_on_device ? ctx->d_domz64 : ctx->w_dz;
  if (ctx->domz_on_device) {
    if (m) { HIPCHK(hipMemcpyAsync(ctx->domz.data(), d_dz.p, m * 8, hipMemcpyDeviceToHost, st)); HIPCHK(hipMemcpyAsync(ctx->domz_ub.data(), d_dz.p + m, m * 8, hipMemcpyDeviceToHost, st)); }
  } else {
    std::vector<int64_t> both(ctx->domz); both.insert(both.end(), ctx->domz_ub.begin(), ctx->domz_ub.end());
    HIPCHK(upload(d_dz, both, st, 2));
  }
  const int32_t U = ctx->U; const int ncls = std::max(ctx->compact_ncls, 1);
  HIPCHK(ctx->l_sure.alloc((size_t)U * ncls + 1)); HIPCHK(ctx->l_has.alloc((size_t)U + 1)); HIPCHK(ctx->w_counters.alloc(16));
  HIPCHK(hipMemsetAsync(ctx->l_sure.p, 0, ((size_t)U * ncls + 1) * sizeof(unsigned long long), st));
  HIPCHK(hipMemsetAsync(ctx->l_has.p, 0, ((size_t)U + 1) * sizeof(int32_t), st));
  HIPCHK(hipMemsetAsync(ctx->w_counters.p, 0, 16 * sizeof(int64_t), st));
  HIPCHK(ctx->l_pflag.alloc((size_t)std::max(ctx->P, 1)));
  HIPCHK(hipMemsetAsync(ctx->l_pflag.p, 0, (size_t)std::max(ctx->P, 1) * 4, st));
  HIPCHK(ctx->l_uflag.alloc((size_t)U + 1));
  HIPCHK(hipMemsetAsync(ctx->l_uflag.p, 0, (size_t)U + 1, st));
  {
    const size_t Pn = (size_t)std::max(ctx->P, 1);
    std::vector<unsigned long long> init(2 * Pn), split(Pn, 0);
    for (size_t p = 0; p < Pn; p++) {
      init[2 * p] = 0; init[2 * p + 1] = ~0ull;
      if (p < ctx->domz.size() && ctx->S == 1) {
        double lo = (double)ctx->domz[p], hi = (double)std::max(ctx->domz_ub[p], ctx->domz[p]);
        if (ctx->topup.valid && ctx->n_chunks == 1 && p < ctx->topup.total.size()) hi = std::min(hi, std::max(lo, (double)ctx->topup.total[p]));
        split[p] = (unsigned long long)(lo + 0.6 * (hi - lo));
      }
    }
    HIPCHK(upload(ctx->l_zneed, init, st)); HIPCHK(upload(ctx->l_zsplit, split, st));
  }
  for (size_t c = 0; c < ctx->dom_n.size(); c++)
    if (ctx->dom_n[c] > 0) launch_finalize_lazy(ctx->dom_bufs[c]->p, ctx->dom_n[c], d_dz.p, d_dz.p + m, domE, ctx->dev_usample(), ctx->P, st);
  for (size_t c = 0; c < ctx->dom_n.size(); c++)
    if (ctx->dom_n[c] > 0) launch_lazy_sure(ctx->dom_bufs[c]->p, ctx->dom_n[c], ctx->w_cls.p, ncls, ctx->l_sure.p, ctx->l_has.p, st);
  for (size_t c = 0; c < ctx->dom_n.size(); c++)
    if (ctx->dom_n[c] > 0) launch_lazy_pending(ctx->dom_bufs[c]->p, ctx->dom_n[c], ctx->w_cls.p, ncls, ctx->l_sure.p, ctx->l_has.p, (unsigned long long *)ctx->w_counters.p, ctx->l_pflag.p, ctx->l_uflag.p, ctx->S == 1 ? ctx->l_zneed.p : nullptr, ctx->l_zsplit.p, domE, st);
  int64_t pend = 0;
  ctx->h_zneed.assign((size_t)std::max(ctx->P, 1) * 2, 0);
  HIPCHK(hipMemcpyAsync(ctx->h_zneed.data(), ctx->l_zneed.p, (size_t)std::max(ctx->P, 1) * 2 * sizeof(unsigned long long), hipMemcpyDeviceToHost, st));
  HIPCHK(hipMemcpyAsync(&pend, ctx->w_counters.p, sizeof(pend), hipMemcpyDeviceToHost, st));
  ctx->lazy_pending_prof.assign((size_t)std::max(ctx->P, 1), 0);
  HIPCHK(hipMemcpyAsync(ctx->lazy_pending_prof.data(), ctx->l_pflag.p, (size_t)std::max(ctx->P, 1) * 4, hipMemcpyDeviceToHost, st));
  HIPCHK(hipStreamSynchronize(st));
  { int np = 0; for (int32_t f : ctx->lazy_pending_prof) np += f != 0; ctx->stats.n_lazy_pending_profiles = np; }
  if (sw_get("ITSX_LAZY_FORCE_PENDING")) pend += atoll(sw_get("ITSX_LAZY_FORCE_PENDING"));
  ctx->lazy_pending = pend; ctx->stats.n_lazy_pending = pend;
  return ITSX_OK;
}

static int lazy_topup(itsx_ctx *ctx, double domE, bool *ran)
{
  (void)domE;
  *ran = false;
  const auto &tu = ctx->topup;
  if (sw_get("ITSX_LAZY_HIST")) fprintf(stderr, "[itsx] top-up: valid %d chunks %d samples %d pairs %lld\n", (int)tu.valid, ctx->n_chunks, ctx->S, (long long)tu.NP);
  if (!tu.valid || ctx->n_chunks != 1 || ctx->S != 1 || tu.NP <= 0) return ITSX_OK;
  if (sw_get("ITSX_LAZY_TOPUP") && atoi(sw_get("ITSX_LAZY_TOPUP")) == 0) return ITSX_OK;
  hipStream_t st = ctx->st;
  const int P = ctx->P;
  itsx_stats &S = ctx->stats;
  std::vector<int32_t> slot((size_t)P, -1), prof_of;
  for (int p = 0; p < P; p++) {
    if (!ctx->lazy_pending_prof[(size_t)p]) continue;
    if (ctx->h_zneed[(size_t)2 * p] == 0 && ctx->h_zneed[(size_t)2 * p + 1] == ~0ull) continue;
    slot[(size_t)p] = (int32_t)prof_of.size(); prof_of.push_back(p);
  }
  const int ns = (int)prof_of.size();
  if (ns == 0) return ITSX_OK;
  StageTimer tm(st);
  const int64_t NP = tu.NP;
  HIPCHK(upload(ctx->l_slot, slot, st)); HIPCHK(upload(ctx->l_pslot, prof_of, st));
  HIPCHK(upload(ctx->w_idx, tu.seg_start, st)); HIPCHK(upload(ctx->w_rcnt, tu.total, st));
  auto count_done = [&](std::vector<unsigned long long> &out) -> int {
    HIPCHK(ctx->l_tcnt.alloc((size_t)ns));
    HIPCHK(hipMemsetAsync(ctx->l_tcnt.p, 0, (size_t)ns * sizeof(unsigned long long), st));
    launch_topup_count(ctx->l_done.p, ctx->w_idx.p, ctx->w_rcnt.p, ctx->l_pslot.p, ns, ctx->l_tcnt.p, st);
    out.assign((size_t)ns, 0);
    HIPCHK(hipMemcpyAsync(out.data(), ctx->l_tcnt.p, (size_t)ns * sizeof(unsigned long long), hipMemcpyDeviceToHost, st));
    HIPCHK(hipStreamSynchronize(st));
    return ITSX_OK;
  };
  std::vector<unsigned long long> ndone;
  { const int rc = count_done(ndone); if (rc != ITSX_OK) return rc; }
  const int64_t nch = (NP + 63) >> 6;
  launch_topup_keys(ctx->d_pairs.p, NP, ctx->l_done.p, ctx->l_b10.p, ctx->l_slot.p, ctx->l_smask.p, ctx->l_scnt.p, nullptr, nullptr, nullptr, st);
  launch_exclusive_scan(ctx->l_scnt.p, ctx->l_spos.p, nch + 1, ctx->l_scan.p, st);
  int32_t M32 = 0;
  HIPCHK(hipMemcpyAsync(&M32, ctx->l_spos.p + nch, 4, hipMemcpyDeviceToHost, st));
  HIPCHK(hipStreamSynchronize(st));
  const int64_t M = M32;
  if (M <= 0) return ITSX_OK;
  HIPCHK(ctx->sh_keys.alloc((size_t)M + 1)); HIPCHK(ctx->sh_keys2.alloc((size_t)M + 1)); HIPCHK(ctx->sh_vals.alloc((size_t)M + 1)); HIPCHK(ctx->sh_uorder.alloc((size_t)M + 1));
  const size_t sort_bytes = order_sort_bytes(M);
  HIPCHK(ctx->sh_sorttmp.alloc(sort_bytes));
  launch_topup_keys(ctx->d_pairs.p, NP, ctx->l_done.p, ctx->l_b10.p, ctx->l_slot.p, ctx->l_smask.p, ctx->l_scnt.p, ctx->l_spos.p, ctx->sh_keys.p, ctx->sh_vals.p, st);
  if (order_sort(ctx->sh_sorttmp.p, sort_bytes, ctx->sh_keys.p, ctx->sh_keys2.p, ctx->sh_vals.p, ctx->sh_uorder.p, M, st) != 0) SET_ERR(ctx, ITSX_E_DEVICE, "top-up round: the radix sort failed");
  HIPCHK(hipStreamSynchronize(st));
  auto lower = [&](unsigned long long key, int64_t &pos) -> int {
    int64_t lo = 0, hi = M;
    while (lo < hi) {
      const int64_t mid = (lo + hi) >> 1; unsigned long long v = 0;
      HIPCHK(hipMemcpy(&v, ctx->sh_keys2.p + mid, 8, hipMemcpyDeviceToHost));
      if (v < key) lo = mid + 1; else hi = mid;
    }
    pos = lo; return ITSX_OK;
  };
  std::vector<uint32_t> cut((size_t)2 * ns, 0);
  bool any = false;
  for (int k = 0; k < ns; k++) {
    const int p = prof_of[(size_t)k];
    int64_t a = 0, b = 0;
    { const int rc = lower((unsigned long long)k << 32, a); if (rc != ITSX_OK) return rc; }
    { const int rc = lower((unsigned long long)(k + 1) << 32, b); if (rc != ITSX_OK) return rc; }
    const int64_t have = b - a;
    if (have <= 0) continue;
    const int64_t lo = ctx->domz[(size_t)p], hi = lo + have;
    int64_t from_top = 0, from_bottom = 0;
    const unsigned long long zl = ctx->h_zneed[(size_t)2 * p], zh = ctx->h_zneed[(size_t)2 * p + 1];
    if (zl > 0 && (int64_t)zl > lo) { const int64_t need = (int64_t)zl - lo; from_top = need + need / 50 + 64; }
    const bool both = sw_get("ITSX_LAZY_TOPUP") && atoi(sw_get("ITSX_LAZY_TOPUP")) == 2;
    if (both && zh != ~0ull && hi > (int64_t)zh) { const int64_t need = hi - (int64_t)zh; from_bottom = need + need / 4 + 64; }
    if (sw_get("ITSX_LAZY_HIST")) fprintf(stderr, "[itsx] top-up: profile %d bounds %lld .. %lld (%lld unevaluated), rows need >= %llu / <= %llu: best %lld, weakest %lld\n", p, (long long)lo, (long long)hi,
                                          (long long)have, zl, zh == ~0ull ? 0ull : zh, (long long)from_top, (long long)from_bottom);
    static const bool topup_all = !(sw_get("ITSX_LAZY_TOPUP_ALL") && atoi(sw_get("ITSX_LAZY_TOPUP_ALL")) == 0);
    const bool above = zh != ~0ull && hi > (int64_t)zh;
    if ((above && !both) || from_top + from_bottom > have - have / 3) {
      if (!topup_all) continue;
      cut[(size_t)2 * k] = 1u; cut[(size_t)2 * k + 1] = 0u;
      any = true;
      continue;
    }
    unsigned long long v = 0;
    if (from_top > 0) {
      HIPCHK(hipMemcpy(&v, ctx->sh_keys2.p + a + from_top - 1, 8, hipMemcpyDeviceToHost));
      cut[(size_t)2 * k] = std::max<uint32_t>(1u, 0xFFFFFFFFu - (uint32_t)(v & 0xFFFFFFFFull));
    }
    if (from_bottom > 0) {
      HIPCHK(hipMemcpy(&v, ctx->sh_keys2.p + b - from_bottom, 8, hipMemcpyDeviceToHost));
      cut[(size_t)2 * k + 1] = std::max<uint32_t>(1u, 0xFFFFFFFFu - (uint32_t)(v & 0xFFFFFFFFull));
      if (cut[(size_t)2 * k] > 0 && cut[(size_t)2 * k + 1] >= cut[(size_t)2 * k]) { cut[(size_t)2 * k] = cut[(size_t)2 * k + 1] = 0; continue; }
    }
    any = any || from_top > 0 || from_bottom > 0;
  }
  if (!any) return ITSX_OK;
  HIPCHK(upload(ctx->l_cut, cut, st));
  launch_topup_mark(ctx->d_pairs.p, NP, ctx->l_done.p, ctx->l_b10.p, ctx->l_slot.p, ctx->l_cut.p, ctx->l_smask.p, ctx->l_scnt.p, st);
  PairList sub; int64_t nsel = 0;
  { const int rc = select_compact(ctx, ctx->d_pairs.p, NP, P, tu.seg_start, ctx->w_seg_start.p, sub, nsel); if (rc != ITSX_OK) return rc; }
  if (sub.NP == 0) return ITSX_OK;
  const int32_t *d_sorted = (ctx->share_on ? ctx->sh_order.p : ctx->d_sorted_uniq.p) + tu.u0;
  ctx->trace_u0 = tu.u0;
  { StageTimer tp(st); const int rc = domain_pipeline(ctx, sub, d_sorted, ctx->T, ctx->sF1, ctx->sF3, nullptr); if (rc != ITSX_OK) return rc; S.ms_lazy_topup_stages += tp.stop(); }
  std::vector<int32_t> dz32((size_t)P * ctx->S, 0);
  HIPCHK(hipMemcpyAsync(dz32.data(), ctx->d_domz32.p, dz32.size() * 4, hipMemcpyDeviceToHost, st));
  HIPCHK(upload(ctx->w_idx, tu.seg_start, st)); HIPCHK(upload(ctx->w_rcnt, tu.total, st));
  { const int rc = count_done(ndone); if (rc != ITSX_OK) return rc; }
  for (size_t z = 0; z < dz32.size(); z++) { ctx->domz_loc[z] = dz32[z]; ctx->domz[z] = dz32[z]; }
  for (int k = 0; k < ns; k++) {
    const int p = prof_of[(size_t)k];
    const int64_t left = (int64_t)tu.total[(size_t)p] - (int64_t)ndone[(size_t)k];
    const int64_t hi = (int64_t)dz32[(size_t)p] + std::max<int64_t>(0, left);
    if (hi < ctx->domz_ub[(size_t)p]) { ctx->domz_ub[(size_t)p] = hi; ctx->domz_ub_loc[(size_t)p] = hi; }
    if (sw_get("ITSX_LAZY_HIST")) fprintf(stderr, "[itsx] top-up: profile %d now %d .. %lld\n", p, dz32[(size_t)p], (long long)ctx->domz_ub[(size_t)p]);
  }
  S.n_lazy_evaluated += nsel; S.n_lazy_topup += nsel;
  S.n_rows_resident = 0;
  for (int64_t r : ctx->dom_n) S.n_rows_resident += r;
  S.ms_lazy_topup += tm.stop();
  *ran = true;
  return ITSX_OK;
}

int itsx_search_finalize(itsx_ctx *ctx, double domE)
{
  CTXCHK(ctx && ctx->have_search);
  HIPCHK(hipSetDevice(ctx->device));
  if (ctx->injected && ctx->lazy && !ctx->domz_exchanged)
    SET_ERR(ctx, ITSX_E_ARG, "itsx_search_finalize: a lazy row table that was handed in (itsx_debug_set_domains) has no counters of its own: give both bounds with itsx_set_domz first");
  StageTimer tm(ctx->st);
  ctx->h_dom.clear(); ctx->drop_alignments();
  auto check_compaction = [&](const std::vector<int64_t> &z) -> int {
    int64_t zmax = 0;
    for (int64_t v : z) zmax = std::max(zmax, v);
    if ((double)zmax > ctx->compact_zmax || domE < ctx->compact_dome_min)
      SET_ERR(ctx, ITSX_E_UNSUPPORTED, "compacted domain rows: only the rows that are reported for every domZ <= " + std::to_string(ctx->compact_zmax) +
              " and every domE >= " + std::to_string(ctx->compact_dome_min) + " were kept, but finalize got domZ up to " + std::to_string(zmax) + " and domE " + std::to_string(domE) +
              " (raise ITSX_COMPACT_ZMAX / lower ITSX_COMPACT_DOME_MIN and search again)");
    return ITSX_OK;
  };
  if (ctx->lazy) {
    { const int rc = finalize_lazy(ctx, domE); if (rc != ITSX_OK) return rc; }
    { const int rc = check_compaction(ctx->domz_ub); if (rc != ITSX_OK) return rc; }
    if (ctx->lazy_pending > 0 && !ctx->domz_exchanged && !sw_get("ITSX_LAZY_NO_RERUN")) {
      const int64_t pend = ctx->lazy_pending;
      {
        bool ran = false;
        { const int rc = lazy_topup(ctx, domE, &ran); if (rc != ITSX_OK) return rc; }
        if (ran) {
          { const int rc = finalize_lazy(ctx, domE); if (rc != ITSX_OK) return rc; }
          ctx->stats.n_lazy_pending = pend;
          if (ctx->lazy_pending == 0) {
            ctx->stats.ms_finalize = tm.stop();
            ctx->have_final = true;
            return ITSX_OK;
          }
        }
      }
      if (!sw_get("ITSX_LAZY_NO_COMPLETE")) {
        std::vector<int32_t> flags(ctx->lazy_pending_prof);
        flags.resize((size_t)std::max(ctx->P, 1), 0);
        { const int rc = itsx_lazy_complete(ctx, flags.data()); if (rc != ITSX_OK) return rc; }
        { const int rc = finalize_lazy(ctx, domE); if (rc != ITSX_OK) return rc; }
        ctx->stats.n_lazy_pending = pend;
      }
      if (ctx->lazy_pending == 0) {
        ctx->stats.ms_finalize = tm.stop();
        ctx->have_final = true;
        return ITSX_OK;
      }
      const int keep = ctx->rows_mode;
      ctx->rows_mode = ITSX_ROWS_COMPACT;
      const int rc = itsx_search(ctx, ctx->T, ctx->sF1, ctx->F2, ctx->sF3);
      ctx->rows_mode = keep;
      if (rc != ITSX_OK) return rc;
      ctx->stats.n_lazy_reruns = 1; ctx->stats.n_lazy_pending = pend; ctx->stats.n_lazy_pending_profiles = 0; for (int32_t f : ctx->lazy_pending_prof) ctx->stats.n_lazy_pending_profiles += f != 0;
    } else {
      ctx->stats.ms_finalize = tm.stop();
      ctx->have_final = true;
      return ITSX_OK;
    }
  }
  {
    DBuf<int64_t> &d_dz = ctx->domz_on_device ? ctx->d_domz64 : ctx->w_dz;
    if (ctx->domz_on_device) {
      if (!ctx->domz.empty()) HIPCHK(hipMemcpyAsync(ctx->domz.data(), d_dz.p, ctx->domz.size() * 8, hipMemcpyDeviceToHost, ctx->st));
    } else HIPCHK(upload(d_dz, ctx->domz, ctx->st));
    for (size_t c = 0; c < ctx->dom_n.size(); c++)
      if (ctx->dom_n[c] > 0) launch_finalize(ctx->dom_bufs[c]->p, ctx->dom_n[c], d_dz.p, domE, ctx->dev_usample(), ctx->P, ctx->st);
    HIPCHK(hipStreamSynchronize(ctx->st));
    if (ctx->compact_rows) { const int rc = check_compaction(ctx->domz); if (rc != ITSX_OK) return rc; }
  }
  ctx->stats.ms_finalize = tm.stop();
  ctx->have_final = true;
  return ITSX_OK;
}

static int fetch_domains(const itsx_ctx *cctx)
{
  itsx_ctx *ctx = const_cast<itsx_ctx *>(cctx);
  if (ctx->compact_rows && !ctx->kept_rows) SET_ERR(ctx, ITSX_E_UNSUPPORTED, "the domain rows of this search were compacted (ITSX_COMPACT_ROWS=1): only coordinates are available, not the row table / domtbl.txt (itsx_set_kept_rows(ctx, 1) serves the rows that were kept)");
  if (ctx->compact_rows && !ctx->have_final) SET_ERR(ctx, ITSX_E_ARG, "the kept rows of a compact / lazy search are served after itsx_search_finalize");
  if (ctx->lazy && ctx->lazy_pending > 0) SET_ERR(ctx, ITSX_E_ARG, "the kept rows of a lazy search are served once no row is undecided (itsx_lazy_pending)");
  if (!ctx->h_dom.empty()) return ITSX_OK;
// ... 2598 lines not shown
```

### itsxpress_amd/csrc/k_api.h

```cpp
#pragma once
#include "engine.h"

#include "detmath.h"
namespace itsx {

struct ReadsDev {
  const uint32_t *words;
  const int64_t  *woff;
  const int32_t  *len;
  const int64_t  *excoff;
  const uint32_t *exc;
  int64_t         n;
};

void launch_hash_reads(const ReadsDev &rd, uint64_t seed, int strand_both, uint64_t *hf, uint64_t *hr, hipStream_t st, const int32_t *sample = nullptr);
void launch_table_insert(int64_t n, const int32_t *len, int minlen, const uint64_t *hf, const uint64_t *hr,
                         unsigned long long *keys, int32_t *vals, uint64_t mask, uint32_t *slot_of, hipStream_t st);
void launch_table_resolve(const ReadsDev &rd, const uint64_t *hf, const int32_t *vals, const uint32_t *slot_of,
                          int32_t *rep_of, int8_t *strand, int32_t *is_seed, unsigned int *n_collisions, hipStream_t st,
                          const int32_t *sample = nullptr);
void launch_uniques(int64_t n, const int32_t *rep_of, const int32_t *seed_rank, int32_t *uniq_of, int32_t *seed_read,
                    int32_t *abundance, hipStream_t st);
void launch_len_hist(int32_t U, const int32_t *seed_read, const int32_t *len, int32_t *hist, int32_t lcap, hipStream_t st, int32_t nb = 0 );
void launch_len_scatter(int32_t U, const int32_t *seed_read, const int32_t *len, int32_t *cursor, int32_t lcap,
// ... 528 lines not shown
  const int32_t *sorted_uniq, *seed_read;
  const DevProfile *prof;
  const LenTables *lt;
  const float *flogsum;
  const PairRec *pairs;
  const PairOut *pout;
  const RegionRec *regions;
  const RegionOut *rout;
  const int64_t *pair_region0;
  const int32_t *upos;
  itsx_domain *dom;
  int64_t npairs;
  double T;
  const MrRec *mr; const int32_t *mr_u; const MrOut *mrout; const int64_t *n2off; const float *n2sc; const int32_t *mr_off;
  int32_t *domz;
  const int32_t *usample;
  int32_t P;
};
void launch_score(const ScoreArgs &a, hipStream_t st);
void launch_region_count_fill(const PairOut *pout, const RegionRec *raw, int64_t npairs, const int32_t *pref,
                              const int64_t *seg_pair_start, const int64_t *seg_region_start, const int32_t *seg_of_pair_base,
                              RegionRec *out, hipStream_t st);

__host__ __device__ __forceinline__ unsigned long long rank_key(const itsx_domain &d)
{
  long long tenths = (long long)__builtin_rint((double)d.bitscore * 10.0) + (1ll << 23);
  if (tenths < 0) tenths = 0;
  if (tenths > (1ll << 24) - 1) tenths = (1ll << 24) - 1;
  const unsigned long long di = (unsigned long long)(d.dom_idx < 0 ? 0 : (d.dom_idx > 0xFFFFF ? 0xFFFFF : d.dom_idx));
  return ((unsigned long long)tenths << 40) | ((unsigned long long)(0xFFFFF - (d.prof & 0xFFFFF)) << 20) | (0xFFFFFull - di);
}

constexpr int LAZY_TENTHS_BIAS = 1 << 23;
struct LazyArgs {
  const PairRec *pairs; int64_t NP;
  const float *fb;
  const LenTables *lt;
  const int8_t *cls; int32_t ncls;
  const int32_t *sorted_uniq;
  uint32_t *b10;
  unsigned long long *gtop;
  int64_t ngroups;
  const unsigned long long *bestc;
  int64_t nbest;
  uint32_t *thr; int64_t nthr;
  uint8_t *done;
  unsigned long long *smask;
  int32_t *scnt;
};
void launch_lazy_bound(const LazyArgs &a, hipStream_t st);
void launch_pad_b10(int32_t P, const int64_t *seg_start , const int32_t *total , uint32_t *b10, hipStream_t st);
void launch_lazy_mark(const LazyArgs &a, int round, hipStream_t st);
void launch_lazy_scatter(const PairRec *pairs, int64_t NP, const unsigned long long *smask, const int32_t *spos, const int64_t *seg_old, const int64_t *seg_new,
                         PairRec *out, hipStream_t st);
void launch_finalize_lazy(itsx_domain *dom, int64_t n, const int64_t *zlb, const int64_t *zub, double domE, const int32_t *usample, int P, hipStream_t st);
void launch_lazy_sure(const itsx_domain *dom, int64_t n, const int8_t *cls, int ncls, unsigned long long *sure, int32_t *has, hipStream_t st);
void launch_lazy_pending(const itsx_domain *dom, int64_t n, const int8_t *cls, int ncls, const unsigned long long *sure, const int32_t *has,
                         unsigned long long *count, int32_t *prof_flag, uint8_t *uniq_flag, unsigned long long *zneed , const unsigned long long *zsplit , double domE, hipStream_t st);
void launch_topup_count(const uint8_t *done, const int64_t *seg_start, const int32_t *total, const int32_t *prof_of_slot, int nslots, unsigned long long *cnt, hipStream_t st);
void launch_topup_keys(const PairRec *pairs, int64_t NP, const uint8_t *done, const uint32_t *b10, const int32_t *slot_of_prof, unsigned long long *smask, int32_t *scnt, const int32_t *spos ,
                       unsigned long long *keys, int32_t *vals, hipStream_t st);
void launch_topup_mark(const PairRec *pairs, int64_t NP, uint8_t *done, const uint32_t *b10, const int32_t *slot_of_prof, const uint32_t *cutoff, unsigned long long *smask, int32_t *scnt, hipStream_t st);

}
```

### itsxpress_amd/csrc/k_float.hip

```cpp
#include "engine.h"
#include "k_api.h"
#include "detmath.h"
#include "k_vec.h"

namespace itsx {

#define TF(q, t) vldc(tf + ((q) * 8 + (t)) * 4)
enum { tBM = 0, tMM, tIM, tDM, tMD, tMI, tII, tDD };

struct Specials { float E, N, J, B, C, SCALE; };

template <int QT> struct Row { V4 m[QMAX], d[QMAX], i[QMAX]; };

struct T7 { V4 bm, mm, im, dm, md, mi, ii; };
DEV T7 ld7(const float *tf, int q)
{
  T7 t;
  t.bm = TF(q, tBM); t.mm = TF(q, tMM); t.im = TF(q, tIM); t.dm = TF(q, tDM);
  t.md = TF(q, tMD); t.mi = TF(q, tMI); t.ii = TF(q, tII);
  return t;
}
#define SCHED_FENCE() __builtin_amdgcn_sched_barrier(0)
#define WAIT_LGKM0() __builtin_amdgcn_s_waitcnt(0xC07F)

// ... 976 lines not shown
    const bool fin = aC == aC && aC > NINF && aC < __builtin_inff() && scaleproduct != __builtin_inff();
    if (go && fin) {
      auto word = [&](int row, int w) { return __float_as_uint(((const float *)eslab_at(a.slab, r0, row, w >> 2, lane))[w & 3]); };
      int i = Ld;
      uint32_t w6 = 0u;
      while (i >= 1) { w6 = word(i, 6); if (w6 >> 16 & 1u) break; i--; }
      int k = (int)(w6 & 0xffffu);
      bool okp = i >= 1 && k >= 1 && k <= 4 * Q;
      const int i2 = i, k2 = k;
      int i1 = i, k1 = k, st = 0;
      bool done = false;
      for (int step = 0; okp && step < Ld + 4 * QMAX + 2; step++) {
        const int q = (k - 1) % Q, z = (k - 1) / Q;
        const uint32_t nib = (word(i, q >> 1) >> ((q & 1) * 16 + z * 4)) & 15u;
        if (st == 0) {
          i1 = i; k1 = k;
          const int c = (int)(nib & 3u);
          if (c == 3) { done = true; break; }
          i--; k--; st = c;
        } else if (st == 1) { i--; st = (nib >> 2 & 1u) ? 1 : 0; }
        else { k--; st = (nib >> 3 & 1u) ? 2 : 0; }
        if (i < 1 || k < 1) okp = false;
      }
      if (okp && done) {
        o.hmm_from = k1; o.hmm_to = k2; o.ali_from = e.off + i1; o.ali_to = e.off + i2; o.oasc = aC; o.aligned = 1;
      }
    }
    out[e.ri] = o;
  }
}

DEV void count_reported(int32_t *domz, int prof, bool flag)
{
  unsigned long long todo = __ballot(flag);
  while (todo) {
    const int leader = __ffsll((long long)todo) - 1;
    const int p0 = __shfl(prof, leader, 64);
    const unsigned long long same = __ballot(flag && prof == p0) & todo;
    if ((int)(threadIdx.x & 63) == leader) atomicAdd(&domz[p0], __popcll(same));
    todo &= ~same;
  }
}

DEV float flogsum_dev(const float *tbl, float x, float y)
{
  const float mx = x > y ? x : y, mn = x > y ? y : x;
  return (mn == -__builtin_inff() || (mx - mn) >= 15.7f) ? mx : mx + tbl[(int)((mx - mn) * 1000.f)];
}

DEV void emit_domain(const ScoreArgs &a, int64_t slot, const PairRec &pr, const DevProfile *pp, const RegionRec &rg, const RegionOut &ro,
                     float domcorr, int dom_idx, int ndom, int poflags, float nullsc, float seq_score, float final_bias, int seq_rep,
                     int L, double lognn3, double log_omega)
{
  itsx_domain o;
  const int Ld = rg.jenv - rg.ienv + 1;
  float bits = (float)((double)ro.envsc + (double)(L - Ld) * lognn3);
  const float dombias = flogsum_dev(a.flogsum, 0.0f, (float)(log_omega + (double)domcorr));
  bits = (float)((double)(bits - (nullsc + dombias)) / kLn2);
  o.rep = a.sorted_uniq[pr.useq]; o.prof = pr.prof; o.tlen = L; o.ienv = rg.ienv; o.jenv = rg.jenv;
  o.dom_idx = dom_idx; o.ndom = ndom; o.flags = (rg.multi ? 1 : 0) | (poflags & 0xff);
  o.envsc = ro.envsc; o.domcorrection = domcorr; o.dombias = dombias; o.bitscore = bits;
  o.lnP = exp_logsurv((double)bits, (double)pp->ev[4], (double)pp->ev[5]);
  o.seq_score = seq_score; o.seq_bias = (float)((double)final_bias / kLn2);
  o.seq_reported = dom_idx >= 0 ? seq_rep : 0; o.dom_reported = 0;
  a.dom[slot] = o;
}

__global__ void __launch_bounds__(256) k_score(ScoreArgs a)
{
  const int64_t pi = (int64_t)blockIdx.x * blockDim.x + threadIdx.x;
  if (pi >= a.npairs) return;
  const PairOut po = a.pout[pi];
  if (!po.pass_fwd || po.ndom <= 0) return;
  const PairRec pr = a.pairs[pi];
  const DevProfile *pp = a.prof + pr.prof;
  const int L = pr.L;
  const LenTables lt = a.lt[L];
  const double log_omega = -5.545177444479562;
  const int64_t g0 = a.pair_region0[pi];
  const int nd_all = po.ndom;
  const float nullsc = po.nullsc;
  const int mr0 = a.mr_off ? a.mr_off[pi] : 0, mr1 = a.mr_off ? a.mr_off[pi + 1] : 0;
  if (nd_all == 1 && mr1 == mr0) {
    const RegionOut ro = a.rout[a.upos[g0]];
    if (!ro.ok) return;
    const RegionRec rg = a.regions[g0];
    const float dc = ro.domcorrection;
    const float seqbias = flogsum_dev(a.flogsum, 0.0f, (float)(log_omega + (double)dc));
    float seq_score = (float)((double)(po.fwdsc - (nullsc + seqbias)) / kLn2);
    float final_bias = seqbias;
    if (ro.envsc - dc > 0.0f) {
      const int Ld = rg.jenv - rg.ienv + 1;
      float sum_score = 0.0f; sum_score += ro.envsc;
      float sb = 0.0f; sb += dc;
      sb = flogsum_dev(a.flogsum, 0.0f, (float)(log_omega + (double)sb));
      sum_score = (float)((double)sum_score + (double)(L - Ld) * lt.lognn3);
      sum_score = (float)((double)(sum_score - (nullsc + sb)) / kLn2);
      if (Ld > 0 && sum_score > seq_score) { seq_score = sum_score; final_bias = sb; }
    } else {
      float sb = flogsum_dev(a.flogsum, 0.0f, (float)(log_omega + 0.0));
      float sum_score = (float)(0.0 + (double)L * lt.lognn3);
      sum_score = (float)((double)(sum_score - (nullsc + sb)) / kLn2);
      (void)sum_score;
    }
    const int seq_rep = ((double)seq_score >= a.T);
    emit_domain(a, g0, pr, pp, rg, ro, dc, 0, 1, po.flags, nullsc, seq_score, final_bias, seq_rep, L, lt.lognn3, log_omega);
// ... 292 lines not shown
```

### itsxpress_amd/csrc/k_lazy.hip

```cpp
#include "engine.h"
#include "k_api.h"
#include "detmath.h"
#include "k_vec.h"

namespace itsx {

constexpr int BP = BOUND_PAIRS;
typedef const f4 __attribute__((address_space(4))) *cf4q;
struct BT { f2 mm, im, dm, mi, ii, bm, md; float dd1, dd2; };
DEV BT ldbt(const float *tab, int j)
{
  const f4 a = *(cf4q)(uintptr_t)(tab + j * 16), b = *(cf4q)(uintptr_t)(tab + j * 16 + 4), c = *(cf4q)(uintptr_t)(tab + j * 16 + 8),
           d = *(cf4q)(uintptr_t)(tab + j * 16 + 12);
  BT t;
  t.mm = (f2){a.x, a.y}; t.im = (f2){a.z, a.w}; t.dm = (f2){b.x, b.y}; t.ii = (f2){b.z, b.w};
  t.bm = (f2){c.x, c.y}; t.dd1 = c.z; t.dd2 = c.w; t.mi = (f2){d.x, d.y}; t.md = (f2){d.z, d.w};
  return t;
}
DEV f2 pfma(f2 a, f2 b, f2 c) { return __builtin_elementwise_fma(a, b, c); }
DEV uint32_t lazy_tenths(float f, const LenTables &lt)
{
  if (f != f || f == __builtin_inff()) return (1u << 24) - 1;
  if (f == -__builtin_inff()) return 1u;
  const double bits = ((double)f - (double)lt.nullsc) / 0.69314718055994529 + (double)lt.lazy_c;
// ... 414 lines not shown
  if (pr.prof < 0 || a.done[i] || (int64_t)pr.useq * a.ncls + a.cls[pr.prof] != g) return;
  a.done[i] = 1;
  atomicOr(&a.smask[i >> 6], 1ull << (i & 63));
}
__global__ void __launch_bounds__(256) k_select_count(const unsigned long long *__restrict__ smask, int64_t nch, int32_t *__restrict__ scnt)
{
  const int64_t c = (int64_t)blockIdx.x * blockDim.x + threadIdx.x;
  if (c <= nch) scnt[c] = c < nch ? (int32_t)__popcll(smask[c]) : 0;
}
__global__ void __launch_bounds__(256) k_lazy_thr(LazyArgs a)
{
  const int64_t g = (int64_t)blockIdx.x * blockDim.x + threadIdx.x;
  if (g >= a.nthr) return;
  const int64_t su = a.sorted_uniq[g / a.ncls], idx = su * a.ncls + g % a.ncls;
  const unsigned long long bc = (su >= 0 && idx < a.nbest) ? a.bestc[idx] : 0ull;
  a.thr[g] = (uint32_t)(bc >> 40);
}
constexpr int MARK_K = 4;
static inline unsigned select_grid(int64_t NP) { const int64_t nw = (((NP + 63) >> 6) + 1 + MARK_K - 1) / MARK_K; return (unsigned)((nw + 3) / 4); }
__global__ void __launch_bounds__(256) k_lazy_mark(LazyArgs a)
{
  const int lane = threadIdx.x & 63;
  const int64_t nch = (a.NP + 63) >> 6;
  const int64_t c0 = ((int64_t)blockIdx.x * 4 + (threadIdx.x >> 6)) * MARK_K;
  if (c0 > nch) return;
  PairRec pr[MARK_K]; uint8_t dn[MARK_K]; uint32_t b[MARK_K], t[MARK_K]; int cl[MARK_K]; bool live[MARK_K];
#pragma unroll
  for (int k = 0; k < MARK_K; k++) {
    const int64_t i = (c0 + k) * 64 + lane;
    pr[k].useq = 0; pr[k].prof = -1; pr[k].xj = -1; pr[k].L = 0; dn[k] = 1; b[k] = 0;
    if (i < a.NP) { pr[k] = a.pairs[i]; dn[k] = a.done[i]; b[k] = a.b10[i]; }
  }
#pragma unroll
  for (int k = 0; k < MARK_K; k++) {
    live[k] = pr[k].prof >= 0 && !dn[k];
    cl[k] = 0;
    if (live[k]) cl[k] = a.cls[pr[k].prof];
  }
#pragma unroll
  for (int k = 0; k < MARK_K; k++) { t[k] = 0u; if (live[k]) t[k] = a.thr[(size_t)pr[k].useq * a.ncls + cl[k]]; }
#pragma unroll
  for (int k = 0; k < MARK_K; k++) {
    const int64_t c = c0 + k;
    if (c > nch) break;
    const int f = live[k] && b[k] >= t[k];
    if (f) a.done[c * 64 + lane] = 1;
    select_store(c * 64 + lane, nch, f, a.smask, a.scnt);
  }
}

constexpr int SCATTER_CHUNKS = 16;
__global__ void __launch_bounds__(256) k_lazy_scatter(const PairRec *__restrict__ pairs, int64_t NP, const unsigned long long *__restrict__ smask,
                                                      const int32_t *__restrict__ spos, const int64_t *__restrict__ seg_old,
                                                      const int64_t *__restrict__ seg_new, PairRec *__restrict__ out)
{
  const int lane = threadIdx.x & 63;
  const int64_t nch = (NP + 63) >> 6;
  const int64_t c0 = ((int64_t)blockIdx.x * 4 + (threadIdx.x >> 6)) * SCATTER_CHUNKS;
  for (int k = 0; k < SCATTER_CHUNKS; k++) {
    const int64_t c = c0 + k;
    if (c >= nch) return;
    const unsigned long long m = smask[c];
    if (!((m >> lane) & 1ull)) continue;
    const int64_t i = c * 64 + lane;
    const PairRec pr = pairs[i];
    const int32_t rank = spos[c] + (int32_t)__popcll(m & ((1ull << lane) - 1ull)) - spos[seg_old[pr.prof] >> 6];
    out[seg_new[pr.prof] + (int64_t)rank] = pr;
  }
}

__global__ void __launch_bounds__(256) k_finalize_lazy(itsx_domain *__restrict__ dom, int64_t n, const int64_t *__restrict__ zlb,
                                                       const int64_t *__restrict__ zub, double domE, const int32_t *__restrict__ usample, int P)
{
  const int64_t i = (int64_t)blockIdx.x * blockDim.x + threadIdx.x;
  if (i >= n) return;
  const itsx_domain d = dom[i];
  if (d.dom_idx < 0) return;
  int rep = 0;
  if (d.seq_reported) {
    const size_t z = (size_t)(usample ? usample[d.rep] * P : 0) + d.prof;
    const double p = det_exp(d.lnP);
    const double lo = (double)(zlb[z] > 1 ? zlb[z] : 1), hi = (double)(zub[z] > 1 ? zub[z] : 1);
    rep = (p * hi <= domE) ? 1 : (p * lo <= domE) ? 2 : 0;
  }
  dom[i].dom_reported = rep;
}

__global__ void __launch_bounds__(256) k_lazy_sure(const itsx_domain *__restrict__ dom, int64_t n, const int8_t *__restrict__ cls, int ncls,
                                                   unsigned long long *__restrict__ sure, int32_t *__restrict__ has)
{
  const int64_t i = (int64_t)blockIdx.x * blockDim.x + threadIdx.x;
  if (i >= n) return;
  const itsx_domain d = dom[i];
  if (d.dom_idx < 0 || d.dom_reported != 1) return;
  has[d.rep] = 1;
  atomicMax(&sure[(size_t)d.rep * ncls + cls[d.prof]], rank_key(d));
}
__global__ void __launch_bounds__(256) k_lazy_pending(const itsx_domain *__restrict__ dom, int64_t n, const int8_t *__restrict__ cls, int ncls,
                                                      const unsigned long long *__restrict__ sure, const int32_t *__restrict__ has,
                                                      unsigned long long *__restrict__ count, int32_t *__restrict__ prof_flag,
                                                      uint8_t *__restrict__ uniq_flag, unsigned long long *__restrict__ zneed, const unsigned long long *__restrict__ zsplit,
                                                      double domE)
{
  const int64_t i = (int64_t)blockIdx.x * blockDim.x + threadIdx.x;
  int c = 0;
  if (i < n) {
    const itsx_domain d = dom[i];
    if (d.dom_idx >= 0 && d.dom_reported == 2) c = !has[d.rep] || rank_key(d) > sure[(size_t)d.rep * ncls + cls[d.prof]];
    if (c) {
      prof_flag[d.prof] = 1; uniq_flag[d.rep] = 1;
      if (zneed) {
        const double z = domE / det_exp(d.lnP);
        if (z < 9.0e18) {
          const unsigned long long zf = (unsigned long long)z;
          if (zf + 2ull <= zsplit[d.prof]) atomicMax(&zneed[2 * d.prof], zf + 2ull);
          else atomicMin(&zneed[2 * d.prof + 1], zf > 2ull ? zf - 2ull : 0ull);
        } else atomicMin(&zneed[2 * d.prof + 1], (unsigned long long)9.0e18);
      }
    }
  }
  const unsigned long long m = __ballot(c);
  if (m && (threadIdx.x & 63) == (unsigned)__builtin_ctzll(m)) atomicAdd(count, (unsigned long long)__builtin_popcountll(m));
}

__global__ void __launch_bounds__(64) k_pad_b10(const int64_t *__restrict__ seg_start, const int32_t *__restrict__ total, uint32_t *__restrict__ b10)
{
  const int64_t e = seg_start[blockIdx.x] + total[blockIdx.x] + threadIdx.x;
  if (e < seg_start[blockIdx.x + 1]) b10[e] = 0u;
}
void launch_pad_b10(int32_t P, const int64_t *seg_start, const int32_t *total, uint32_t *b10, hipStream_t st)
{
  if (P > 0) hipLaunchKernelGGL(k_pad_b10, dim3((unsigned)P), dim3(64), 0, st, seg_start, total, b10);
}
void launch_lazy_bound(const LazyArgs &a, hipStream_t st)
{
  if (a.NP > 0) hipLaunchKernelGGL(k_lazy_bound, dim3((unsigned)((a.NP + 255) / 256)), dim3(256), 0, st, a);
}
void launch_lazy_mark(const LazyArgs &a, int round, hipStream_t st)
{
  const int64_t nch = (a.NP + 63) >> 6;
  if (round == 0) {
    (void)hipMemsetAsync(a.smask, 0, (size_t)nch * sizeof(unsigned long long), st);
    if (a.ngroups > 0) hipLaunchKernelGGL(k_lazy_first, dim3((unsigned)((a.ngroups + 255) / 256)), dim3(256), 0, st, a);
    hipLaunchKernelGGL(k_select_count, dim3((unsigned)((nch + 1 + 255) / 256)), dim3(256), 0, st, a.smask, nch, a.scnt);
  } else {
    if (a.nthr > 0) hipLaunchKernelGGL(k_lazy_thr, dim3((unsigned)((a.nthr + 255) / 256)), dim3(256), 0, st, a);
    hipLaunchKernelGGL(k_lazy_mark, dim3(select_grid(a.NP)), dim3(256), 0, st, a);
  }
}
void launch_lazy_scatter(const PairRec *pairs, int64_t NP, const unsigned long long *smask, const int32_t *spos, const int64_t *seg_old, const int64_t *seg_new,
                         PairRec *out, hipStream_t st)
{
  const int64_t nch = (NP + 63) >> 6, per_block = 4 * SCATTER_CHUNKS;
  if (NP > 0) hipLaunchKernelGGL(k_lazy_scatter, dim3((unsigned)((nch + per_block - 1) / per_block)), dim3(256), 0, st, pairs, NP, smask, spos, seg_old, seg_new, out);
}
void launch_finalize_lazy(itsx_domain *dom, int64_t n, const int64_t *zlb, const int64_t *zub, double domE, const int32_t *usample, int P, hipStream_t st)
{
  if (n > 0) hipLaunchKernelGGL(k_finalize_lazy, dim3((unsigned)((n + 255) / 256)), dim3(256), 0, st, dom, n, zlb, zub, domE, usample, P);
}
void launch_lazy_sure(const itsx_domain *dom, int64_t n, const int8_t *cls, int ncls, unsigned long long *sure, int32_t *has, hipStream_t st)
{
  if (n > 0) hipLaunchKernelGGL(k_lazy_sure, dim3((unsigned)((n + 255) / 256)), dim3(256), 0, st, dom, n, cls, ncls, sure, has);
}
void launch_lazy_pending(const itsx_domain *dom, int64_t n, const int8_t *cls, int ncls, const unsigned long long *sure, const int32_t *has,
                         unsigned long long *count, int32_t *prof_flag, uint8_t *uniq_flag, unsigned long long *zneed, const unsigned long long *zsplit, double domE, hipStream_t st)
{
  if (n > 0) hipLaunchKernelGGL(k_lazy_pending, dim3((unsigned)((n + 255) / 256)), dim3(256), 0, st, dom, n, cls, ncls, sure, has, count, prof_flag, uniq_flag, zneed, zsplit, domE);
}
__global__ void __launch_bounds__(256) k_topup_count(const uint8_t *__restrict__ done, const int64_t *__restrict__ seg_start, const int32_t *__restrict__ total,
                                                     const int32_t *__restrict__ prof_of_slot, unsigned long long *__restrict__ cnt)
{
  const int sl = blockIdx.y, p = prof_of_slot[sl];
  const int64_t base = seg_start[p], n = total[p];
  unsigned long long c = 0;
  for (int64_t i = (int64_t)blockIdx.x * 256 + threadIdx.x; i < n; i += (int64_t)gridDim.x * 256) c += done[base + i] != 0;
  for (int o = 32; o >= 1; o >>= 1) c += __shfl_xor(c, o, 64);
  if ((threadIdx.x & 63) == 0 && c) atomicAdd(&cnt[sl], c);
}
void launch_topup_count(const uint8_t *done, const int64_t *seg_start, const int32_t *total, const int32_t *prof_of_slot, int nslots, unsigned long long *cnt, hipStream_t st)
{
  if (nslots > 0) hipLaunchKernelGGL(k_topup_count, dim3(512, (unsigned)nslots), dim3(256), 0, st, done, seg_start, total, prof_of_slot, cnt);
}

__global__ void __launch_bounds__(256) k_topup_keys(const PairRec *__restrict__ pairs, int64_t NP, const uint8_t *__restrict__ done, const uint32_t *__restrict__ b10,
                                                    const int32_t *__restrict__ slot_of_prof, unsigned long long *__restrict__ smask, int32_t *__restrict__ scnt,
                                                    const int32_t *__restrict__ spos, unsigned long long *__restrict__ keys, int32_t *__restrict__ vals)
{
  const int lane = threadIdx.x & 63;
  const int64_t nch = (NP + 63) >> 6;
  const int64_t c0 = ((int64_t)blockIdx.x * 4 + (threadIdx.x >> 6)) * MARK_K;
  if (c0 > nch) return;
  if (!spos) {
    PairRec pr[MARK_K]; uint8_t dn[MARK_K];
#pragma unroll
    for (int k = 0; k < MARK_K; k++) {
      const int64_t i = (c0 + k) * 64 + lane;
      pr[k].useq = 0; pr[k].prof = -1; pr[k].xj = -1; pr[k].L = 0; dn[k] = 1;
      if (i < NP) { pr[k] = pairs[i]; dn[k] = done[i]; }
    }
    int sl[MARK_K];
#pragma unroll
    for (int k = 0; k < MARK_K; k++) { sl[k] = -1; if (pr[k].prof >= 0 && pr[k].xj >= 0 && !dn[k]) sl[k] = slot_of_prof[pr[k].prof]; }
#pragma unroll
    for (int k = 0; k < MARK_K; k++) {
      if (c0 + k > nch) break;
      select_store((c0 + k) * 64 + lane, nch, sl[k] >= 0, smask, scnt);
    }
// ... 1 lines not shown
  }
  unsigned long long m[MARK_K];
#pragma unroll
  for (int k = 0; k < MARK_K; k++) m[k] = c0 + k < nch ? smask[c0 + k] : 0ull;
#pragma unroll
  for (int k = 0; k < MARK_K; k++) {
    if (!((m[k] >> lane) & 1ull)) continue;
    const int64_t i = (c0 + k) * 64 + lane;
    const int32_t at = spos[c0 + k] + (int32_t)__popcll(m[k] & ((1ull << lane) - 1ull));
    const int sl = slot_of_prof[pairs[i].prof];
    keys[at] = ((unsigned long long)sl << 32) | (unsigned long long)(0xFFFFFFFFu - b10[i]); vals[at] = (int32_t)i;
  }
}
__global__ void __launch_bounds__(256) k_topup_mark(const PairRec *__restrict__ pairs, int64_t NP, uint8_t *__restrict__ done, const uint32_t *__restrict__ b10,
                                                    const int32_t *__restrict__ slot_of_prof, const uint32_t *__restrict__ cutoff,
                                                    unsigned long long *__restrict__ smask, int32_t *__restrict__ scnt)
{
  const int lane = threadIdx.x & 63;
  const int64_t nch = (NP + 63) >> 6;
  const int64_t c0 = ((int64_t)blockIdx.x * 4 + (threadIdx.x >> 6)) * MARK_K;
  if (c0 > nch) return;
  PairRec pr[MARK_K]; uint8_t dn[MARK_K]; uint32_t b[MARK_K];
#pragma unroll
  for (int k = 0; k < MARK_K; k++) {
    const int64_t i = (c0 + k) * 64 + lane;
    pr[k].useq = 0; pr[k].prof = -1; pr[k].xj = -1; pr[k].L = 0; dn[k] = 1; b[k] = 0;
    if (i < NP) { pr[k] = pairs[i]; dn[k] = done[i]; b[k] = b10[i]; }
  }
  int sl[MARK_K];
#pragma unroll
  for (int k = 0; k < MARK_K; k++) { sl[k] = -1; if (pr[k].prof >= 0 && pr[k].xj >= 0 && !dn[k]) sl[k] = slot_of_prof[pr[k].prof]; }
  uint32_t hi[MARK_K], lo[MARK_K];
#pragma unroll
  for (int k = 0; k < MARK_K; k++) { hi[k] = 0; lo[k] = 0; if (sl[k] >= 0) { hi[k] = cutoff[2 * sl[k]]; lo[k] = cutoff[2 * sl[k] + 1]; } }
#pragma unroll
  for (int k = 0; k < MARK_K; k++) {
    if (c0 + k > nch) break;
    const int f = (hi[k] > 0 && b[k] >= hi[k]) || (lo[k] > 0 && b[k] <= lo[k]);
    if (f) done[(c0 + k) * 64 + lane] = 1;
    select_store((c0 + k) * 64 + lane, nch, f, smask, scnt);
  }
}
void launch_topup_keys(const PairRec *pairs, int64_t NP, const uint8_t *done, const uint32_t *b10, const int32_t *slot_of_prof, unsigned long long *smask, int32_t *scnt,
                       const int32_t *spos, unsigned long long *keys, int32_t *vals, hipStream_t st)
{
  hipLaunchKernelGGL(k_topup_keys, dim3(select_grid(NP)), dim3(256), 0, st, pairs, NP, done, b10, slot_of_prof, smask, scnt, spos, keys, vals);
}
void launch_topup_mark(const PairRec *pairs, int64_t NP, uint8_t *done, const uint32_t *b10, const int32_t *slot_of_prof, const uint32_t *cutoff,
                       unsigned long long *smask, int32_t *scnt, hipStream_t st)
{
  hipLaunchKernelGGL(k_topup_mark, dim3(select_grid(NP)), dim3(256), 0, st, pairs, NP, done, b10, slot_of_prof, cutoff, smask, scnt);
}

}
```

### itsxpress_amd/csrc/switches.cpp

```cpp
#include "switches.h"
#include <cstdlib>
#include <cstring>

namespace itsx {

static const Switch g_sw[] = {
  {"ITSX_NO_ENSEMBLE", SW_HOOK, "multidomain regions keep their region as one envelope instead of hmmsearch's stochastic-traceback clustering (changes envelopes)"},
  {"ITSX_LAZY_ZUB_SCALE", SW_HOOK, "multiplies the lazy stage's upper bound on domZ: more undecided rows for the completion tests"},
  {"ITSX_LAZY_FORCE_PENDING", SW_HOOK, "treats rows as undecided so that the completion path runs"},
  {"ITSX_LAZY_NO_RERUN", SW_HOOK, "skips the full re-search safety net (leaves undecided rows undecided)"},
  {"ITSX_LAZY_NO_COMPLETE", SW_HOOK, "skips itsx_lazy_complete inside itsx_search_finalize (leaves undecided rows undecided)"},
  {"ITSX_COMPACT_ZMAX", SW_HOOK, "largest domZ the compact / lazy modes call a row 'certain' for (default 1e9); a value below the data's domZ can drop a winner"},
  {"ITSX_COMPACT_DOME_MIN", SW_HOOK, "smallest --domE the compact / lazy modes call a row 'certain' for (default 1e-2)"},
  {"ITSX_PASSA_DBG", SW_HOOK, "pass A diagnostic bits (no rows / no restore / no join): timings only, scores are garbage; 64: the shared MSV kernel counts its floored wave-rows, those with the xB branch and its waves by word layout (results unchanged; one stderr line per search)"},
  {"ITSX_MSV_PB", SW_HOOK, "profiles one block of the MSV filter takes its sequences through (1 .. 32; default: by the job's size, 1 for a small job): same cells"},
  {"ITSX_TWRITER_HOST_SLICE", SW_HOOK, "=1: a streamed writer with a device (itsx_twriter_set_device) slices every unit on the host, as it does a unit its line index does not fit (same file bytes)"},
  {"ITSX_ROWS", SW_MODE, "rows mode when the caller did not call itsx_set_rows_mode: full | compact | lazy (coordinates identical in all three)"},
  {"ITSX_COMPACT_ROWS", SW_MODE, "=1: rows mode compact (older spelling of ITSX_ROWS=compact)"},
  {"ITSX_QMASK", SW_MODE, "=none: vsearch's --qmask none for cluster_size / orient seeds (default dust, as vsearch)"},
  {"ITSX_KEEP_TRACE", SW_MODE, "keeps per-pair filter traces for itsx_get_pairtraces (forces the compact path of a lazy search)"},
  {"ITSX_GZIP_LEVEL", SW_MODE, "deflate level of the trimmed-FASTQ writers (default 6; output bytes differ, records do not)"},
  {"ITSX_DEVICE_DEFLATE", SW_MODE, "=1: the batch writers deflate gzip output on the device, and so do the outputs a StreamEngine plans (output bytes differ, records do not)"},
  {"ITSX_SHARE_SAMPLES", SW_MODE, "=1: every context shares the HMM stages across the samples of a batch, as after itsx_set_sample_sharing(ctx, 1) (full rows mode, S > 1; same rows, counters, coordinates and files)"},
  {"ITSX_TEST_HOOKS", SW_DIAG, "=1: honour the HOOK switches above"},
  {"ITSX_SHARE_CHECK", SW_DIAG, "runs the unshared kernels beside the shared ones and counts differences (itsx_stats.share_mismatch, join_maxdiff)"},
  {"ITSX_LAZY_CHECK_BOUND", SW_DIAG, "compares pass A's scores with HMMER's own Forward arithmetic (itsx_stats.lazy_bound_maxdiff)"},
  {"ITSX_LAZY_HIST", SW_DIAG, "prints the histogram of round-2 candidates per group"},
  {"ITSX_PASSA_DUMP", SW_DIAG, "prints every pass-A launch's waves and wave-rows (scripts/passa_launches.py)"},
  {"ITSX_TRACE_ALLOC", SW_DIAG, "prints every hipMalloc / free with its time"},
  {"ITSX_CL_DEBUG", SW_DIAG, "clustering: prints per-window counters"},
  {"ITSX_MR_DEBUG", SW_DIAG, "ensemble stage: prints per-batch counters"},
  {"ITSX_SHARE", SW_TUNING, "=0: no prefix sharing (round 4's schedule)"},
  {"ITSX_SHARE_TWO", SW_TUNING, "=0: one-sided (prefix-only) sharing for pass A"},
  {"ITSX_MSV_TWO", SW_TUNING, "=0: the MSV filter keeps the one-sided (prefix-only) schedule when pass A shares two-sidedly"},
  {"ITSX_SHARE_B", SW_TUNING, "rows per block of the prefix / suffix trees (default 32)"},
  {"ITSX_SHARE_GB", SW_TUNING, "budget of the saved row states, GB"},
  {"ITSX_SHARE_MIN", SW_TUNING, "smallest shared-row fraction for which the shared schedule is used (default 0.10)"},
  {"ITSX_SHARE_FWD_STREAMS", SW_TUNING, "1 | 2 streams for pass A's batches"},
  {"ITSX_SHARE_MSV_STREAMS", SW_TUNING, "1 | 2 streams for the MSV filter's batches"},
  {"ITSX_NO_CHAINREC", SW_TUNING, "pass A reads a chain's data through the round-5 arrays instead of its 64-byte record (A/B)"},
  {"ITSX_BOUND_FOLD", SW_TUNING, "=0: pass A's plain recurrences instead of the folded ones (also switches two-sided sharing off)"},
  {"ITSX_BOUND_RESCALE_EXP", SW_TUNING, "power of ten at which pass A rescales a row (default 20)"},
  {"ITSX_LAZY_TOPUP", SW_TUNING, "=0: undecided rows go straight to the full count of their profiles (no top-up round); =2: the round also looks for unreported pairs among a profile's weakest (rows settled from above)"},
  {"ITSX_LAZY_EXACT_BOUND", SW_TUNING, "pass A through the HMMER-order Forward kernel (A/B)"},
  {"ITSX_CHUNK_UNIQUES", SW_TUNING, "representatives per search chunk"},
  {"ITSX_MSV_OVERLAP", SW_TUNING, "=0: the next chunk's MSV filter does not run beside the domain stage"},
  {"ITSX_MSV_PAD", SW_TUNING, "dynamic LDS of the overlapped MSV launch (an occupancy cap)"},
  {"ITSX_MSV_WHOLE", SW_TUNING, "where the MSV filter keeps a lane's packed words: 2 (default) shared chains keep their wave's window of at most 16 words, loaded once per block; 1 the whole read when the launch's longest fits 37 words, as the unshared kernel always does; 0 16 words at a time everywhere (A/B arms: same cells; read at every launch)"},
  {"ITSX_MSV_FLOOR", SW_TUNING, "=0: the MSV filter's plain three-instruction row on every row instead of the floored two-instruction one (A/B arm: same cells; read at every launch)"},
  {"ITSX_BIAS_OVERLAP", SW_TUNING, "=0: the bias filter does not run on the second stream"},
  {"ITSX_ST2_PRIO", SW_TUNING, "priority of the second stream"},
  {"ITSX_LOAD_PRIORITY", SW_TUNING, "=0: loads do not use the high-priority stream"},
  {"ITSX_SLAB_GB", SW_TUNING, "DP slab budget, GB"},
  {"ITSX_SLAB_ADAPT", SW_TUNING, "=0: the slab budget does not adapt to the job"},
  {"ITSX_ALIGN_SLAB_MB", SW_TUNING, "itsx_align_domains: slab budget of one batch of waves, MB (default 4096; a small value forces several batches: same alignments)"},
  {"ITSX_DEFER_FREE_GB", SW_TUNING, "device memory kept on the deferred-free list, GB"},
  {"ITSX_MR_LONG_FRAC", SW_TUNING, "ensemble stage: share of regions taken as 'long'"},
  {"ITSX_MR_LONG_LANES", SW_TUNING, "ensemble stage: lanes per long region"},
  {"ITSX_MSV_BWD_WHOLE", SW_TUNING, "=1: the MSV filter's Backward chains copy their whole read to LDS first (A/B arm: same cells)"},
  {"ITSX_LAZY_TOPUP_ALL", SW_TUNING, "=0: a profile whose undecided rows need most of its pairs is left to the full count (itsx_lazy_complete) instead of taking all its unevaluated pairs in the top-up round (same rows)"},
  {"ITSX_MR_WAVES", SW_TUNING, "ensemble stage: waves a batch is spread over (lanes per wave = regions / this, 2 .. 64); 0 = waves of 64 lanes"},
  {"ITSX_MR_ONE_MAX", SW_TUNING, "ensemble stage: a batch of at most this many regions (default 2048) is walked one region per wave with the matrix in LDS; 0 = never"},
  {"ITSX_CIGAR_MB", SW_TUNING, "itsx_align_clusters: byte budget of one batch of pairs (direction bits and border rows), MB (default 2048; a small value forces several batches, and a pair larger than it runs alone: same alignments)"},
  {"ITSX_CL_NOSCORE", SW_TUNING, "clustering: skips the score-only pre-pass (A/B arm; the walk then aligns every candidate: same outcomes)"},
  {"ITSX_CL_NOPRECHECK", SW_TUNING, "clustering: skips the certificate pre-check (A/B arm: same outcomes)"},
  {"ITSX_CL_CAPACITY", SW_TUNING, "clustering: candidate-list capacity"},
  {"ITSX_CL_CCAP", SW_TUNING, "clustering: centroid capacity step"},
  {"ITSX_CL_HEAVY", SW_TUNING, "clustering: heavy-word split on / off"},
  {"ITSX_CL_HEAVY_MIN", SW_TUNING, "clustering: centroids a word needs to count as conserved"},
  {"ITSX_CL_ROWS", SW_TUNING, "clustering: alignment rows per lane"},
  {"ITSX_CL_WINDOW", SW_TUNING, "clustering: queries per speculative window"},
  {"ITSX_PACK_CHUNK", SW_TUNING, "reads per packing launch"},
  {"ITSX_PACK_ECAP", SW_TUNING, "initial capacity of the exception list"},
  {"ITSX_HUGEPAGES", SW_TUNING, "=0: host buffers without MADV_HUGEPAGE"},
  {"ITSX_IO_LIBDEFLATE", SW_TUNING, "=0: zlib instead of libdeflate when both are present"},
  {"ITSX_IO_THREADS", SW_TUNING, "host threads of the FASTQ readers / writers"},
  {"ITSX_IO_BLOCK_KB", SW_TUNING, "deflate unit of the block-parallel writer"},
  {"ITSX_DEVICE_INFLATE", SW_TUNING, "=1: the whole-file loaders of every context try a gzip file of independent members on the device first (same text; read at every load)"},
  {"ITSX_INFLATE_MEMBER_KB", SW_TUNING, "longest compressed member the device inflate takes (default 8192: twice the host writer's block); a file with a longer one is the host's"},
  {"ITSX_INFLATE_GRID", SW_TUNING, "most workgroups of the device inflate's launch (default: four per CU, what their LDS allows); fewer: each decodes more members in a row (same text)"},
  {"ITSX_DEVICE_PARSE", SW_TUNING, "=1: the whole-file loaders and the paired merge loaders of every context parse FASTQ text on the device (same reads; a text it declines is the host parser's; read at every load)"},
  {"ITSX_PARALLEL_INFLATE", SW_TUNING, "=0: single-stream inflate"},
  {"ITSX_PINFLATE_CHUNK_KB", SW_TUNING, "chunk of the block-parallel inflater"},
  {"ITSX_PARSE_MIN_MB", SW_TUNING, "smallest text parsed on several threads"},
  {"ITSX_TEXT_CACHE_GB", SW_TUNING, "inflated-text cache, GB"},
  {"ITSX_WRITE_MIN_MB", SW_TUNING, "smallest output written by several threads"},
  {"ITSX_WRITE_UNIT_KB", SW_TUNING, "unit of the streamed writer"},
  {"ITSX_STREAM_RESERVE_MB", SW_TUNING, "streamed loads: first reservation"},
  {"ITSX_STREAM_RESERVE_X", SW_TUNING, "streamed loads: growth factor"},
};
static const int g_nsw = (int)(sizeof(g_sw) / sizeof(g_sw[0]));

const Switch *sw_registry(int *n) { if (n) *n = g_nsw; return g_sw; }

static bool hooks_on() { const char *e = sw_get("ITSX_TEST_HOOKS"); return e && atoi(e) == 1; }

const char *sw_get(const char *name)
{
  const char *v = getenv(name);
  if (!v) return nullptr;
  for (int i = 0; i < g_nsw; i++)
    if (strcmp(g_sw[i].name, name) == 0) return (g_sw[i].kind == SW_HOOK && !hooks_on()) ? nullptr : v;
  return nullptr;
}

std::string sw_report()
{
  std::string out;
  const bool on = hooks_on();
  for (int i = 0; i < g_nsw; i++) {
    const char *v = getenv(g_sw[i].name);
    if (!v) continue;
    out += g_sw[i].name; out += "="; out += v;
// ... 8 lines not shown
```

### itsxpress_amd/engine.py

```python
import ctypes as C
import os

import numpy as np

from . import _lib
from ._lib import ALIGNMENT_DTYPE, DOMAIN_DTYPE, LAZY_PAIR_DTYPE, STATS_DTYPE_ALL, TRACE_DTYPE, EngineError


def _device_from_env():
    for k in ("ITSXPRESS_GPU", "LOCAL_RANK"):
        v = os.environ.get(k)
        if v is not None and v.strip() != "":
            return int(v)
    return 0


class _DevArray:

    def __init__(self, ptr, shape, typestr):
        self.__cuda_array_interface__ = {"shape": tuple(shape), "typestr": typestr, "data": (int(ptr), False), "version": 3,
                                         "strides": None}


def _devtensor(ptr, shape, typestr, device):
# ... 628 lines not shown
        self._chk(self.L.itsx_inflate_fetch(self.h, out.ctypes.data, n.value))
        self.inflate_members = int(m.value)
        return out[:n.value].tobytes()

    PARSE_PLANES = {"off": 0, "toff": 1, "seq": 2, "qual": 3, "titles": 4}

    def parse_fetch(self, plane, lo, hi):
        k = self.PARSE_PLANES[plane]
        n = max(int(hi) - int(lo), 0)
        out = np.empty(max(n, 1), np.int64 if k < 2 else np.uint8)
        self._chk(self.L.itsx_parse_fetch(self.h, k, int(lo), int(hi), out.ctypes.data))
        return out[:n].copy() if k < 2 else out[:n].tobytes()

    def parse_device(self, text, keep_qual=True):
        text = bytes(text)
        n = C.c_int64(0)
        self._chk(self.L.itsx_parse_device(self.h, text, len(text), int(bool(keep_qual)), C.byref(n)))
        n = int(n.value)
        off, toff = self.parse_fetch("off", 0, n + 1), self.parse_fetch("toff", 0, n + 1)
        return dict(n=n, off=off, toff=toff, seq=self.parse_fetch("seq", 0, int(off[-1])),
                    qual=self.parse_fetch("qual", 0, int(off[-1])) if keep_qual else None, titles=self.parse_fetch("titles", 0, int(toff[-1])))

    def parse_pairs_fetch(self, side, plane, lo, hi):
        k = self.PARSE_PLANES[plane]
        n = max(int(hi) - int(lo), 0)
        out = np.empty(max(n, 1), np.int64 if k < 2 else np.uint8)
        self._chk(self.L.itsx_parse_pairs_fetch(self.h, int(side), k, int(lo), int(hi), out.ctypes.data))
        return out[:n].copy() if k < 2 else out[:n].tobytes()

    def parse_pairs_device(self, text1, text2):
        text1, text2 = bytes(text1), bytes(text2)
        n, flags, mx = C.c_int64(0), C.c_int32(0), C.c_int64(0)
        self._chk(self.L.itsx_parse_pairs_device(self.h, text1, len(text1), text2, len(text2), C.byref(n), C.byref(flags), C.byref(mx)))
        n = int(n.value)
        sides = []
        for s in (0, 1):
            off, toff = self.parse_pairs_fetch(s, "off", 0, n + 1), self.parse_pairs_fetch(s, "toff", 0, n + 1)
            sides.append(dict(off=off, toff=toff, seq=self.parse_pairs_fetch(s, "seq", 0, int(off[-1])), qual=self.parse_pairs_fetch(s, "qual", 0, int(off[-1])),
                              titles=self.parse_pairs_fetch(s, "titles", 0, int(toff[-1]))))
        return dict(n=n, flags=int(flags.value), max_total=int(mx.value), sides=sides)

    def write_uc(self, path):
        self._chk(self.L.itsx_write_uc(self.h, os.fsencode(path)))

    def write_rep_fasta(self, path):
        self._chk(self.L.itsx_write_rep_fasta(self.h, os.fsencode(path)))

    def write_domtbl(self, path):
        self._chk(self.L.itsx_write_domtbl(self.h, os.fsencode(path)))

    def stats(self):
        s = np.zeros(1, STATS_DTYPE_ALL)
        self._chk(self.L.itsx_get_stats(self.h, s.ctypes.data, STATS_DTYPE_ALL.itemsize))
        return {k: (s[0][k].item() if s[0][k].ndim == 0 else s[0][k].tolist()) for k in STATS_DTYPE_ALL.names}

    def release_scratch(self):
        self._chk(self.L.itsx_release_scratch(self.h))

    def switches(self, now=False):
        h = None if now else self.h
        n = self.L.itsx_switches(h, None, 0)
        buf = C.create_string_buffer(int(n))
        self.L.itsx_switches(h, buf, n)
        return dict(line.split("=", 1) for line in buf.value.decode().split("\n") if "=" in line)

    def debug_set_domains(self, rows, seg_rows=None, mode="full"):
        rows = np.ascontiguousarray(rows, DOMAIN_DTYPE)
        seg = np.ascontiguousarray([len(rows)] if seg_rows is None else seg_rows, np.int64)
        m = {"full": 0, "compact": 1, "lazy": 2}.get(mode, mode)
        self._chk(self.L.itsx_debug_set_domains(self.h, rows.ctypes.data if rows.size else None, len(rows),
                                                seg.ctypes.data if seg.size else None, len(seg), int(m)))

    def debug_get_rows(self):
        n = int(self.L.itsx_debug_get_rows(self.h, None, 0))
        if n < 0:
            raise EngineError(n, self.L.itsx_last_error(self.h).decode())
        out = np.zeros(max(n, 1), DOMAIN_DTYPE)
        got = int(self.L.itsx_debug_get_rows(self.h, out.ctypes.data, n))
        if got != n:
            raise EngineError(min(got, -1), self.L.itsx_last_error(self.h).decode())
        return out[:n]

    def debug_lazy_pairs(self):
        bias = C.c_int32(0)
        n = int(self.L.itsx_debug_lazy_pairs(self.h, None, 0, C.byref(bias)))
        if n < 0:
            raise EngineError(n, self.L.itsx_last_error(self.h).decode())
        out = np.zeros(max(n, 1), LAZY_PAIR_DTYPE)
        got = int(self.L.itsx_debug_lazy_pairs(self.h, out.ctypes.data, n, C.byref(bias)))
        if got != n:
            raise EngineError(min(got, -1), self.L.itsx_last_error(self.h).decode())
        return out[:n], int(bias.value)

    def debug_read_hashes(self):
        f = np.zeros(self.n_reads, np.uint64)
        r = np.zeros(self.n_reads, np.uint64)
        self._chk(self.L.itsx_debug_read_hashes(self.h, f.ctypes.data, r.ctypes.data))
        return f, r

    def debug_read_samples(self):
        d = np.zeros(max(1, self.n_reads), np.int32)
        h = np.zeros(max(1, self.n_reads), np.int32)
        self._chk(self.L.itsx_debug_read_samples(self.h, d.ctypes.data, h.ctypes.data))
        return d[:self.n_reads], h[:self.n_reads]

    def debug_sorted_uniques(self):
        out = np.zeros(max(1, self.n_unique), np.int32)
# ... 59 lines not shown
```

Measured before the change: 4.948 million.

## Run lazy top-up round count-only, deferring multidomain pairs past the ensemble stage

The lazy top-up round now sends its pairs through the domain pipeline in a count-only mode. It skips row allocation, row writes and compaction. Pairs with multidomain regions skip the ensemble stage and are recorded in a deferred mask, and a second sub-round runs them only if a profile's row is still undecided. A by-need partial top-up mode is also added. Together these aim to cut the ensemble and row-materialisation work of the top-up round, at the cost of extra kernels, syncs and a possible second pass.

New measurement: 5.038 million (median of 6 runs). 1.02x the previous value.

```diff
diff --git a/include/itsx_hip.h b/include/itsx_hip.h
--- a/include/itsx_hip.h
+++ b/include/itsx_hip.h
@@ -234,6 +234,7 @@
 int itsx_lazy_pending_uniques(itsx_ctx *ctx, uint8_t *flags);
 int itsx_set_partial_coords(itsx_ctx *ctx, int on);
 int itsx_lazy_complete(itsx_ctx *ctx, const int32_t *flags);
+int itsx_topup_counters(const itsx_ctx *ctx, int64_t *counters );
 int64_t itsx_domz_count(const itsx_ctx *ctx);
 int itsx_get_domz(const itsx_ctx *ctx, int64_t *domZ );
 int itsx_set_domz(itsx_ctx *ctx, const int64_t *domZ );
diff --git a/itsxpress_amd/_lib.py b/itsxpress_amd/_lib.py
--- a/itsxpress_amd/_lib.py
+++ b/itsxpress_amd/_lib.py
@@ -94,7 +94,8 @@
            "itsx_debug_scan", "itsx_debug_select", "itsx_debug_region_keys", "itsx_debug_lazy_pairs",
            "itsx_set_sample_sharing", "itsx_sample_sharing_info", "itsx_sample_sharing_times", "itsx_debug_sample_classes",
            "itsx_align_domains", "itsx_get_alignments", "itsx_write_domtbl_arrays_ali",
-           "itsx_align_clusters", "itsx_get_cluster_cigars"]
+           "itsx_align_clusters", "itsx_get_cluster_cigars",
+           "itsx_topup_counters"]
 
 
 def lib():
@@ -209,6 +210,7 @@
         "itsx_search": (i32, [vp, f64, f64, f64, f64]),
         "itsx_set_rows_mode": (i32, [vp, i32]),
         "itsx_lazy_pending": (i64, [vp]),
+        "itsx_topup_counters": (i32, [vp, vp]),
         "itsx_lazy_pending_profiles": (i32, [vp, vp]),
         "itsx_lazy_complete": (i32, [vp, vp]),
         "itsx_domz_count": (i64, [vp]),
diff --git a/itsxpress_amd/csrc/engine.hip b/itsxpress_amd/csrc/engine.hip
--- a/itsxpress_amd/csrc/engine.hip
+++ b/itsxpress_amd/csrc/engine.hip
@@ -419,6 +419,10 @@
   std::string switches_at_search;
   struct TopUp { bool valid = false, list_live = false ; int64_t NP = 0; std::vector<int64_t> seg_start; std::vector<int32_t> total; int32_t u0 = 0, Uc = 0; } topup;
   DBuf<unsigned long long> l_zneed, l_zsplit, l_tcnt; DBuf<int32_t> l_slot, l_pslot; DBuf<uint32_t> l_cut;
+  DBuf<int32_t> l_src; DBuf<unsigned long long> l_dmask, l_defn, l_tcnt2;
+  int64_t n_topup_deferred = 0, n_topup_ensemble = 0, topup_deferred_live = 0 ;
+  std::vector<int64_t> topup_defp;
+  std::vector<int32_t> topup_profs, topup_partial;
   std::vector<unsigned long long> h_zneed;
   bool prev_lazy = false; int prev_P = 0; int64_t prev_U = 0, prev_Uc = 0;
   std::vector<int32_t> h_merge_index;
@@ -2220,7 +2224,7 @@
   ctx->domz_ub.assign((size_t)P * ctx->S, 0);
   if (ctx->compact_rows)
     for (auto &b : ctx->dom_bufs) if (b && b->cap * sizeof(itsx_domain) > ((size_t)256 << 20)) b->release();
-  S.lazy = ctx->lazy; S.n_lazy_evaluated = S.n_lazy_round1 = S.n_lazy_pending = S.n_lazy_reruns = 0; S.n_lazy_completed = S.n_lazy_completed_profiles = S.n_lazy_pending_profiles = 0; S.ms_lazy_complete = 0; S.lazy_bound_maxdiff = 0; S.ms_bound_kernel = S.ms_lazy_select = 0; S.bound_rows = 0; S.n_bound_launches = 0; S.n_lazy_topup = 0; S.ms_lazy_topup = 0; S.ms_lazy_topup_stages = 0;
+  S.lazy = ctx->lazy; S.n_lazy_evaluated = S.n_lazy_round1 = S.n_lazy_pending = S.n_lazy_reruns = 0; S.n_lazy_completed = S.n_lazy_completed_profiles = S.n_lazy_pending_profiles = 0; S.ms_lazy_complete = 0; S.lazy_bound_maxdiff = 0; S.ms_bound_kernel = S.ms_lazy_select = 0; S.bound_rows = 0; S.n_bound_launches = 0; S.n_lazy_topup = 0; S.ms_lazy_topup = 0; S.ms_lazy_topup_stages = 0; ctx->n_topup_deferred = ctx->n_topup_ensemble = 0;
   if (ctx->compact_rows && U > 0) { const int rc = compact_setup(ctx); if (rc != ITSX_OK) return rc; }
   if (U == 0) return ITSX_OK;
 
@@ -2525,7 +2529,7 @@
   return ITSX_OK;
 }
 
-static int domain_pipeline(itsx_ctx *ctx, const PairList &pl, const int32_t *d_sorted, double T, double F1, double F3, const std::function<int()> *next_msv)
+static int domain_pipeline(itsx_ctx *ctx, const PairList &pl, const int32_t *d_sorted, double T, double F1, double F3, const std::function<int()> *next_msv, bool count_only = false)
 {
   hipStream_t st = ctx->st;
   const int P = ctx->P;
@@ -2687,7 +2691,11 @@
   StageTimer tm_dom(st);
   int64_t NMR = 0;
   const bool ensemble = !(sw_get("ITSX_NO_ENSEMBLE") && atoi(sw_get("ITSX_NO_ENSEMBLE")) != 0);
-  if (ensemble) {
+  if (ensemble && count_only) {
+    HIPCHK(ctx->w_mrcnt.alloc((size_t)NP + 2));
+    launch_mr_count(pl.pout, d_raw.p, pv, NP, ctx->w_mrcnt.p, st);
+    launch_topup_defer(pl.pout, ctx->w_mrcnt.p, ctx->l_src.p, NP, ctx->l_done.p, ctx->l_dmask.p, ctx->l_defn.p, st);
+  } else if (ensemble) {
     DBuf<int32_t> &mrcnt = ctx->w_mrcnt, &mroff = ctx->w_mroff, &stmp = ctx->w_scan2;
     HIPCHK(mrcnt.alloc((size_t)NP + 2)); HIPCHK(mroff.alloc((size_t)NP + 2)); HIPCHK(stmp.alloc((size_t)scan_tmp_elems(NP + 2)));
     launch_mr_count(pl.pout, d_raw.p, pv, NP, mrcnt.p, st);
@@ -2884,11 +2892,13 @@
   std::vector<int32_t> rtotal((size_t)P);
   for (int p = 0; p < P; p++) { rtotal[p] = bound[p + 1] - bound[p]; rseg[p + 1] = rseg[p] + ((int64_t)rtotal[p] + 63) / 64 * 64; S.n_domains += rtotal[p]; }
   const int64_t NR = rseg[P];
-  ctx->dom_n[di] = NR;
+  ctx->dom_n[di] = count_only ? 0 : NR;
   HIPCHK(ctx->d_pair_region0.alloc((size_t)NP));
   HIPCHK(ctx->d_regions.alloc((size_t)std::max<int64_t>(NR, 1)));
-  HIPCHK(d_dom.alloc((size_t)std::max<int64_t>(NR, 1)));
-  HIPCHK(hipMemsetAsync(d_dom.p, 0xFF, (size_t)std::max<int64_t>(NR, 1) * sizeof(itsx_domain), st));
+  if (!count_only) {
+    HIPCHK(d_dom.alloc((size_t)std::max<int64_t>(NR, 1)));
+    HIPCHK(hipMemsetAsync(d_dom.p, 0xFF, (size_t)std::max<int64_t>(NR, 1) * sizeof(itsx_domain), st));
+  }
   if (NR > 0) {
     DBuf<int64_t> &d_rseg = ctx->w_rseg;
     HIPCHK(upload(d_rseg, rseg, st));
@@ -2976,11 +2986,11 @@
     ScoreArgs sa{};
     sa.rd = ctx->rd; sa.sorted_uniq = d_sorted; sa.seed_read = ctx->d_seed_read.p; sa.prof = ctx->d_prof.p; sa.lt = ctx->d_lt.p;
     sa.flogsum = ctx->d_flogsum.p; sa.pairs = pl.pairs; sa.pout = pl.pout; sa.regions = ctx->d_regions.p; sa.rout = ctx->d_rout.p;
-    sa.pair_region0 = ctx->d_pair_region0.p; sa.upos = ctx->d_upos.p; sa.dom = d_dom.p; sa.npairs = NP; sa.T = T;
+    sa.pair_region0 = ctx->d_pair_region0.p; sa.upos = ctx->d_upos.p; sa.dom = count_only ? nullptr : d_dom.p; sa.npairs = NP; sa.T = T;
     if (NMR > 0) { sa.mr = ctx->w_mr.p; sa.mr_u = ctx->w_mru.p; sa.mrout = ctx->w_mrout.p; sa.n2off = ctx->w_n2off.p; sa.n2sc = ctx->w_n2sc.p; sa.mr_off = ctx->w_mroff.p; }
     sa.domz = ctx->d_domz32.p; sa.usample = ctx->dev_usample(); sa.P = ctx->P;
     launch_score(sa, st);
-    if (ctx->compact_rows) {
+    if (ctx->compact_rows && !count_only) {
       { const int rc = compact_segment(ctx, d_dom.p, NR, di); if (rc != ITSX_OK) return rc; }
     }
   }
@@ -3021,7 +3031,7 @@
 }
 }
 
-static int select_compact(itsx_ctx *ctx, const PairRec *pairs, int64_t NP, int P, const std::vector<int64_t> &seg_start, const int64_t *d_seg_start, PairList &sub, int64_t &nsel)
+static int select_compact(itsx_ctx *ctx, const PairRec *pairs, int64_t NP, int P, const std::vector<int64_t> &seg_start, const int64_t *d_seg_start, PairList &sub, int64_t &nsel, bool want_src = false)
 {
   hipStream_t st = ctx->st;
   const int64_t nch = (NP + 63) >> 6;
@@ -3043,7 +3053,8 @@
   HIPCHK(hipMemsetAsync(ctx->l_pairs.p, 0xFF, (size_t)sub.NP * sizeof(PairRec), st));
   HIPCHK(hipMemsetAsync(ctx->d_pout.p, 0, (size_t)sub.NP * sizeof(PairOut), st));
   HIPCHK(upload(ctx->l_seg, sub.seg_start, st));
-  launch_lazy_scatter(pairs, NP, ctx->l_smask.p, ctx->l_spos.p, d_seg_start, ctx->l_seg.p, ctx->l_pairs.p, st);
+  if (want_src) HIPCHK(ctx->l_src.alloc((size_t)sub.NP));
+  launch_lazy_scatter(pairs, NP, ctx->l_smask.p, ctx->l_spos.p, d_seg_start, ctx->l_seg.p, ctx->l_pairs.p, st, want_src ? ctx->l_src.p : nullptr);
   sub.pairs = ctx->l_pairs.p; sub.pout = ctx->d_pout.p; sub.d_seg_start = ctx->l_seg.p;
   return ITSX_OK;
 }
@@ -3567,6 +3578,12 @@
   for (int p = 0; p < ctx->P; p++) flags[p] = (ctx->lazy && (size_t)p < ctx->lazy_pending_prof.size()) ? (ctx->lazy_pending_prof[(size_t)p] != 0) : 0;
   return ITSX_OK;
 }
+int itsx_topup_counters(const itsx_ctx *ctx, int64_t *counters)
+{
+  CTXCHK(ctx && counters);
+  counters[0] = ctx->n_topup_deferred; counters[1] = ctx->n_topup_ensemble;
+  return ITSX_OK;
+}
 int itsx_set_partial_coords(itsx_ctx *ctx, int on) { CTXCHK(ctx); ctx->partial_coords = on != 0; return ITSX_OK; }
 int itsx_set_kept_rows(itsx_ctx *ctx, int on) { CTXCHK(ctx); if (ctx->kept_rows != (on != 0)) { ctx->h_dom.clear(); ctx->drop_alignments(); } ctx->kept_rows = on != 0; return ITSX_OK; }
 int itsx_lazy_pending_uniques(itsx_ctx *ctx, uint8_t *flags)
@@ -3680,7 +3697,7 @@
   ctx->compact_rows = mode != ITSX_ROWS_FULL; ctx->lazy = mode == ITSX_ROWS_LAZY;
   ctx->lazy_pending = 0; ctx->domz_exchanged = false; ctx->lazy_pending_prof.clear();
   itsx_stats &S = ctx->stats;
-  S.lazy = ctx->lazy; S.n_domains = 0; S.n_lazy_pending = S.n_lazy_reruns = S.n_lazy_topup = S.n_lazy_completed = S.n_lazy_completed_profiles = S.n_lazy_pending_profiles = 0;
+  S.lazy = ctx->lazy; S.n_domains = 0; S.n_lazy_pending = S.n_lazy_reruns = S.n_lazy_topup = S.n_lazy_completed = S.n_lazy_completed_profiles = S.n_lazy_pending_profiles = 0; ctx->n_topup_deferred = ctx->n_topup_ensemble = 0;
   for (int64_t i = 0; i < n_rows; i++) S.n_domains += rows[i].dom_idx >= 0;
   HIPCHK(ctx->d_domz32.alloc(std::max<size_t>(m, 1)));
   HIPCHK(hipMemsetAsync(ctx->d_domz32.p, 0, std::max<size_t>(m, 1) * 4, st));
@@ -3778,10 +3795,45 @@
   return ITSX_OK;
 }
 
-static int lazy_topup(itsx_ctx *ctx, double domE, bool *ran)
+static int topup_bounds(itsx_ctx *ctx, bool with_deferred)
+{
+  hipStream_t st = ctx->st;
+  const auto &tu = ctx->topup;
+  const std::vector<int32_t> &prof_of = ctx->topup_profs;
+  const int ns = (int)prof_of.size(), P = ctx->P;
+  std::vector<int32_t> dz32((size_t)P * ctx->S, 0);
+  HIPCHK(hipMemcpyAsync(dz32.data(), ctx->d_domz32.p, dz32.size() * 4, hipMemcpyDeviceToHost, st));
+  HIPCHK(upload(ctx->w_idx, tu.seg_start, st)); HIPCHK(upload(ctx->w_rcnt, tu.total, st)); HIPCHK(upload(ctx->l_pslot, prof_of, st));
+  HIPCHK(ctx->l_tcnt.alloc((size_t)std::max(ns, 1)));
+  HIPCHK(hipMemsetAsync(ctx->l_tcnt.p, 0, (size_t)std::max(ns, 1) * sizeof(unsigned long long), st));
+  launch_topup_count(ctx->l_done.p, ctx->w_idx.p, ctx->w_rcnt.p, ctx->l_pslot.p, ns, ctx->l_tcnt.p, st);
+  std::vector<unsigned long long> ndone((size_t)ns, 0), ndef((size_t)ns, 0);
+  if (ns > 0) HIPCHK(hipMemcpyAsync(ndone.data(), ctx->l_tcnt.p, (size_t)ns * sizeof(unsigned long long), hipMemcpyDeviceToHost, st));
+  if (with_deferred && ns > 0) {
+    HIPCHK(ctx->l_tcnt2.alloc((size_t)ns));
+    HIPCHK(hipMemsetAsync(ctx->l_tcnt2.p, 0, (size_t)ns * sizeof(unsigned long long), st));
+    launch_topup_count_mask(ctx->l_dmask.p, ctx->w_idx.p, ctx->w_rcnt.p, ctx->l_pslot.p, ns, ctx->l_tcnt2.p, st);
+    HIPCHK(hipMemcpyAsync(ndef.data(), ctx->l_tcnt2.p, (size_t)ns * sizeof(unsigned long long), hipMemcpyDeviceToHost, st));
+  }
+  HIPCHK(hipStreamSynchronize(st));
+  ctx->topup_defp.assign((size_t)P, 0);
+  for (int k = 0; k < ns; k++) ctx->topup_defp[(size_t)prof_of[(size_t)k]] = (int64_t)ndef[(size_t)k];
+  for (size_t z = 0; z < dz32.size(); z++) { ctx->domz_loc[z] = dz32[z]; ctx->domz[z] = dz32[z]; }
+  for (int k = 0; k < ns; k++) {
+    const int p = prof_of[(size_t)k];
+    const int64_t left = (int64_t)tu.total[(size_t)p] - (int64_t)ndone[(size_t)k];
+    const int64_t hi = (int64_t)dz32[(size_t)p] + std::max<int64_t>(0, left);
+    if (hi < ctx->domz_ub[(size_t)p]) { ctx->domz_ub[(size_t)p] = hi; ctx->domz_ub_loc[(size_t)p] = hi; }
+    if (sw_get("ITSX_LAZY_HIST")) fprintf(stderr, "[itsx] top-up: profile %d now %d .. %lld\n", p, dz32[(size_t)p], (long long)ctx->domz_ub[(size_t)p]);
+  }
+  return ITSX_OK;
+}
+
+static int lazy_topup(itsx_ctx *ctx, double domE, bool *ran, bool rest = false)
 {
   (void)domE;
   *ran = false;
+  if (!rest) { ctx->topup_deferred_live = 0; ctx->topup_partial.clear(); }
   const auto &tu = ctx->topup;
   if (sw_get("ITSX_LAZY_HIST")) fprintf(stderr, "[itsx] top-up: valid %d chunks %d samples %d pairs %lld\n", (int)tu.valid, ctx->n_chunks, ctx->S, (long long)tu.NP);
   if (!tu.valid || ctx->n_chunks != 1 || ctx->S != 1 || tu.NP <= 0) return ITSX_OK;
@@ -3793,6 +3845,7 @@
   for (int p = 0; p < P; p++) {
     if (!ctx->lazy_pending_prof[(size_t)p]) continue;
     if (ctx->h_zneed[(size_t)2 * p] == 0 && ctx->h_zneed[(size_t)2 * p + 1] == ~0ull) continue;
+    if (rest && std::find(ctx->topup_partial.begin(), ctx->topup_partial.end(), p) == ctx->topup_partial.end()) continue;
     slot[(size_t)p] = (int32_t)prof_of.size(); prof_of.push_back(p);
   }
   const int ns = (int)prof_of.size();
@@ -3801,17 +3854,6 @@
   const int64_t NP = tu.NP;
   HIPCHK(upload(ctx->l_slot, slot, st)); HIPCHK(upload(ctx->l_pslot, prof_of, st));
   HIPCHK(upload(ctx->w_idx, tu.seg_start, st)); HIPCHK(upload(ctx->w_rcnt, tu.total, st));
-  auto count_done = [&](std::vector<unsigned long long> &out) -> int {
-    HIPCHK(ctx->l_tcnt.alloc((size_t)ns));
-    HIPCHK(hipMemsetAsync(ctx->l_tcnt.p, 0, (size_t)ns * sizeof(unsigned long long), st));
-    launch_topup_count(ctx->l_done.p, ctx->w_idx.p, ctx->w_rcnt.p, ctx->l_pslot.p, ns, ctx->l_tcnt.p, st);
-    out.assign((size_t)ns, 0);
-    HIPCHK(hipMemcpyAsync(out.data(), ctx->l_tcnt.p, (size_t)ns * sizeof(unsigned long long), hipMemcpyDeviceToHost, st));
-    HIPCHK(hipStreamSynchronize(st));
-    return ITSX_OK;
-  };
-  std::vector<unsigned long long> ndone;
-  { const int rc = count_done(ndone); if (rc != ITSX_OK) return rc; }
   const int64_t nch = (NP + 63) >> 6;
   launch_topup_keys(ctx->d_pairs.p, NP, ctx->l_done.p, ctx->l_b10.p, ctx->l_slot.p, ctx->l_smask.p, ctx->l_scnt.p, nullptr, nullptr, nullptr, st);
   launch_exclusive_scan(ctx->l_scnt.p, ctx->l_spos.p, nch + 1, ctx->l_scan.p, st);
@@ -3853,13 +3895,17 @@
     if (sw_get("ITSX_LAZY_HIST")) fprintf(stderr, "[itsx] top-up: profile %d bounds %lld .. %lld (%lld unevaluated), rows need >= %llu / <= %llu: best %lld, weakest %lld\n", p, (long long)lo, (long long)hi,
                                           (long long)have, zl, zh == ~0ull ? 0ull : zh, (long long)from_top, (long long)from_bottom);
     static const bool topup_all = !(sw_get("ITSX_LAZY_TOPUP_ALL") && atoi(sw_get("ITSX_LAZY_TOPUP_ALL")) == 0);
+    const bool by_need = sw_get("ITSX_LAZY_TOPUP_ALL") && atoi(sw_get("ITSX_LAZY_TOPUP_ALL")) == 2 && !(sw_get("ITSX_TOPUP_COUNT_ONLY") && atoi(sw_get("ITSX_TOPUP_COUNT_ONLY")) == 0);
     const bool above = zh != ~0ull && hi > (int64_t)zh;
-    if ((above && !both) || from_top + from_bottom > have - have / 3) {
-      if (!topup_all) continue;
+    if (by_need && !rest && above && from_bottom == 0 && (int64_t)zh > lo) { const int64_t need = (int64_t)zh - lo; from_top = std::max(from_top, need + need / 50 + 64); }
+    const bool partial = by_need && !rest && from_bottom == 0 && from_top > 0 && from_top < have;
+    if (rest || (!partial && ((above && !both) || from_top + from_bottom > have - have / 3))) {
+      if (!topup_all && !rest) continue;
       cut[(size_t)2 * k] = 1u; cut[(size_t)2 * k + 1] = 0u;
       any = true;
       continue;
     }
+    if (partial && (above || from_top > have - have / 3)) ctx->topup_partial.push_back(p);
     unsigned long long v = 0;
     if (from_top > 0) {
       HIPCHK(hipMemcpy(&v, ctx->sh_keys2.p + a + from_top - 1, 8, hipMemcpyDeviceToHost));
@@ -3875,29 +3921,58 @@
   if (!any) return ITSX_OK;
   HIPCHK(upload(ctx->l_cut, cut, st));
   launch_topup_mark(ctx->d_pairs.p, NP, ctx->l_done.p, ctx->l_b10.p, ctx->l_slot.p, ctx->l_cut.p, ctx->l_smask.p, ctx->l_scnt.p, st);
+  const bool count_only = !(sw_get("ITSX_TOPUP_COUNT_ONLY") && atoi(sw_get("ITSX_TOPUP_COUNT_ONLY")) == 0);
   PairList sub; int64_t nsel = 0;
-  { const int rc = select_compact(ctx, ctx->d_pairs.p, NP, P, tu.seg_start, ctx->w_seg_start.p, sub, nsel); if (rc != ITSX_OK) return rc; }
+  { const int rc = select_compact(ctx, ctx->d_pairs.p, NP, P, tu.seg_start, ctx->w_seg_start.p, sub, nsel, count_only); if (rc != ITSX_OK) return rc; }
   if (sub.NP == 0) return ITSX_OK;
+  if (count_only) {
+    HIPCHK(ctx->l_dmask.alloc((size_t)nch + 1)); HIPCHK(ctx->l_defn.alloc(2));
+    if (!rest) HIPCHK(hipMemsetAsync(ctx->l_dmask.p, 0, ((size_t)nch + 1) * sizeof(unsigned long long), st));
+    HIPCHK(hipMemsetAsync(ctx->l_defn.p, 0, 2 * sizeof(unsigned long long), st));
+  }
   const int32_t *d_sorted = (ctx->share_on ? ctx->sh_order.p : ctx->d_sorted_uniq.p) + tu.u0;
   ctx->trace_u0 = tu.u0;
-  { StageTimer tp(st); const int rc = domain_pipeline(ctx, sub, d_sorted, ctx->T, ctx->sF1, ctx->sF3, nullptr); if (rc != ITSX_OK) return rc; S.ms_lazy_topup_stages += tp.stop(); }
-  std::vector<int32_t> dz32((size_t)P * ctx->S, 0);
-  HIPCHK(hipMemcpyAsync(dz32.data(), ctx->d_domz32.p, dz32.size() * 4, hipMemcpyDeviceToHost, st));
-  HIPCHK(upload(ctx->w_idx, tu.seg_start, st)); HIPCHK(upload(ctx->w_rcnt, tu.total, st));
-  { const int rc = count_done(ndone); if (rc != ITSX_OK) return rc; }
-  for (size_t z = 0; z < dz32.size(); z++) { ctx->domz_loc[z] = dz32[z]; ctx->domz[z] = dz32[z]; }
-  for (int k = 0; k < ns; k++) {
-    const int p = prof_of[(size_t)k];
-    const int64_t left = (int64_t)tu.total[(size_t)p] - (int64_t)ndone[(size_t)k];
-    const int64_t hi = (int64_t)dz32[(size_t)p] + std::max<int64_t>(0, left);
-    if (hi < ctx->domz_ub[(size_t)p]) { ctx->domz_ub[(size_t)p] = hi; ctx->domz_ub_loc[(size_t)p] = hi; }
-    if (sw_get("ITSX_LAZY_HIST")) fprintf(stderr, "[itsx] top-up: profile %d now %d .. %lld\n", p, dz32[(size_t)p], (long long)ctx->domz_ub[(size_t)p]);
-  }
+  { StageTimer tp(st); const int rc = domain_pipeline(ctx, sub, d_sorted, ctx->T, ctx->sF1, ctx->sF3, nullptr, count_only); if (rc != ITSX_OK) return rc; S.ms_lazy_topup_stages += tp.stop(); }
+  unsigned long long ndef = 0;
+  if (count_only) HIPCHK(hipMemcpyAsync(&ndef, ctx->l_defn.p, sizeof(ndef), hipMemcpyDeviceToHost, st));
+  if (!rest) ctx->topup_profs = prof_of;
+  { const int rc = topup_bounds(ctx, count_only); if (rc != ITSX_OK) return rc; }
+  if (rest && count_only) {
+    unsigned long long again = 0;
+    HIPCHK(hipMemcpy(&again, ctx->l_defn.p + 1, sizeof(again), hipMemcpyDeviceToHost));
+    nsel -= (int64_t)again;
+  }
+  nsel -= (int64_t)ndef;
+  if (rest) { ctx->n_topup_deferred += (int64_t)ndef; ctx->topup_deferred_live += (int64_t)ndef; }
+  else { ctx->n_topup_deferred = (int64_t)ndef; ctx->topup_deferred_live = (int64_t)ndef; }
   S.n_lazy_evaluated += nsel; S.n_lazy_topup += nsel;
   S.n_rows_resident = 0;
   for (int64_t r : ctx->dom_n) S.n_rows_resident += r;
   S.ms_lazy_topup += tm.stop();
   *ran = true;
+  return ITSX_OK;
+}
+
+static int lazy_topup_deferred(itsx_ctx *ctx)
+{
+  const auto &tu = ctx->topup;
+  hipStream_t st = ctx->st;
+  itsx_stats &S = ctx->stats;
+  StageTimer tm(st);
+  ctx->topup_deferred_live = 0;
+  launch_topup_deferred_select(ctx->l_dmask.p, tu.NP, ctx->l_smask.p, ctx->l_scnt.p, ctx->l_done.p, st);
+  PairList sub; int64_t nsel = 0;
+  { const int rc = select_compact(ctx, ctx->d_pairs.p, tu.NP, ctx->P, tu.seg_start, ctx->w_seg_start.p, sub, nsel); if (rc != ITSX_OK) return rc; }
+  if (sub.NP == 0) return ITSX_OK;
+  const int32_t *d_sorted = (ctx->share_on ? ctx->sh_order.p : ctx->d_sorted_uniq.p) + tu.u0;
+  ctx->trace_u0 = tu.u0;
+  { StageTimer tp(st); const int rc = domain_pipeline(ctx, sub, d_sorted, ctx->T, ctx->sF1, ctx->sF3, nullptr); if (rc != ITSX_OK) return rc; S.ms_lazy_topup_stages += tp.stop(); }
+  { const int rc = topup_bounds(ctx, false); if (rc != ITSX_OK) return rc; }
+  S.n_lazy_evaluated += nsel; S.n_lazy_topup += nsel;
+  ctx->n_topup_ensemble = 1;
+  S.n_rows_resident = 0;
+  for (int64_t r : ctx->dom_n) S.n_rows_resident += r;
+  S.ms_lazy_topup += tm.stop();
   return ITSX_OK;
 }
 
@@ -3929,6 +4004,30 @@
         if (ran) {
           { const int rc = finalize_lazy(ctx, domE); if (rc != ITSX_OK) return rc; }
           ctx->stats.n_lazy_pending = pend;
+          bool more = false;
+          if (ctx->lazy_pending > 0) for (int32_t p : ctx->topup_partial) more = more || ctx->lazy_pending_prof[(size_t)p] != 0;
+          if (more) {
+            bool ran2 = false;
+            { const int rc = lazy_topup(ctx, domE, &ran2, true); if (rc != ITSX_OK) return rc; }
+            if (ran2) { const int rc = finalize_lazy(ctx, domE); if (rc != ITSX_OK) return rc; ctx->stats.n_lazy_pending = pend; }
+          }
+          bool second = sw_get("ITSX_TOPUP_FORCE_SECOND") && atoi(sw_get("ITSX_TOPUP_FORCE_SECOND")) != 0;
+          if (ctx->lazy_pending > 0 && ctx->S == 1)
+            for (int32_t p : ctx->topup_profs) {
+              const int64_t nd = (size_t)p < ctx->topup_defp.size() ? ctx->topup_defp[(size_t)p] : 0;
+              if (!ctx->lazy_pending_prof[(size_t)p] || nd <= 0) continue;
+              const unsigned long long zl = ctx->h_zneed[(size_t)2 * p], zh = ctx->h_zneed[(size_t)2 * p + 1];
+              if (zl == 0 && zh == ~0ull) continue;
+              const int64_t lo = ctx->domz[(size_t)p], hi = std::max(ctx->domz_ub[(size_t)p], lo);
+              const bool below = zl == 0 || (int64_t)zl <= lo || (int64_t)zl - lo + 1 <= nd;
+              const bool above = zh == ~0ull || hi <= (int64_t)zh || hi - (int64_t)zh + 1 <= nd;
+              second = second || (below && above);
+            }
+          if (second && ctx->topup_deferred_live > 0) {
+            { const int rc = lazy_topup_deferred(ctx); if (rc != ITSX_OK) return rc; }
+            { const int rc = finalize_lazy(ctx, domE); if (rc != ITSX_OK) return rc; }
+            ctx->stats.n_lazy_pending = pend;
+          }
           if (ctx->lazy_pending == 0) {
             ctx->stats.ms_finalize = tm.stop();
             ctx->have_final = true;
diff --git a/itsxpress_amd/csrc/k_api.h b/itsxpress_amd/csrc/k_api.h
--- a/itsxpress_amd/csrc/k_api.h
+++ b/itsxpress_amd/csrc/k_api.h
@@ -604,7 +604,7 @@
 void launch_pad_b10(int32_t P, const int64_t *seg_start , const int32_t *total , uint32_t *b10, hipStream_t st);
 void launch_lazy_mark(const LazyArgs &a, int round, hipStream_t st);
 void launch_lazy_scatter(const PairRec *pairs, int64_t NP, const unsigned long long *smask, const int32_t *spos, const int64_t *seg_old, const int64_t *seg_new,
-                         PairRec *out, hipStream_t st);
+                         PairRec *out, hipStream_t st, int32_t *src = nullptr );
 void launch_finalize_lazy(itsx_domain *dom, int64_t n, const int64_t *zlb, const int64_t *zub, double domE, const int32_t *usample, int P, hipStream_t st);
 void launch_lazy_sure(const itsx_domain *dom, int64_t n, const int8_t *cls, int ncls, unsigned long long *sure, int32_t *has, hipStream_t st);
 void launch_lazy_pending(const itsx_domain *dom, int64_t n, const int8_t *cls, int ncls, const unsigned long long *sure, const int32_t *has,
@@ -613,5 +613,8 @@
 void launch_topup_keys(const PairRec *pairs, int64_t NP, const uint8_t *done, const uint32_t *b10, const int32_t *slot_of_prof, unsigned long long *smask, int32_t *scnt, const int32_t *spos ,
                        unsigned long long *keys, int32_t *vals, hipStream_t st);
 void launch_topup_mark(const PairRec *pairs, int64_t NP, uint8_t *done, const uint32_t *b10, const int32_t *slot_of_prof, const uint32_t *cutoff, unsigned long long *smask, int32_t *scnt, hipStream_t st);
+void launch_topup_defer(PairOut *pout, const int32_t *mrcnt, const int32_t *src, int64_t npairs, uint8_t *done, unsigned long long *dmask, unsigned long long *n, hipStream_t st);
+void launch_topup_count_mask(const unsigned long long *dmask, const int64_t *seg_start, const int32_t *total, const int32_t *prof_of_slot, int nslots, unsigned long long *cnt, hipStream_t st);
+void launch_topup_deferred_select(const unsigned long long *dmask, int64_t NP, unsigned long long *smask, int32_t *scnt, uint8_t *done, hipStream_t st);
 
 }
diff --git a/itsxpress_amd/csrc/k_float.hip b/itsxpress_amd/csrc/k_float.hip
--- a/itsxpress_amd/csrc/k_float.hip
+++ b/itsxpress_amd/csrc/k_float.hip
@@ -1052,6 +1052,7 @@
                      float domcorr, int dom_idx, int ndom, int poflags, float nullsc, float seq_score, float final_bias, int seq_rep,
                      int L, double lognn3, double log_omega)
 {
+  if (!a.dom) return;
   itsx_domain o;
   const int Ld = rg.jenv - rg.ienv + 1;
   float bits = (float)((double)ro.envsc + (double)(L - Ld) * lognn3);
diff --git a/itsxpress_amd/csrc/k_lazy.hip b/itsxpress_amd/csrc/k_lazy.hip
--- a/itsxpress_amd/csrc/k_lazy.hip
+++ b/itsxpress_amd/csrc/k_lazy.hip
@@ -490,7 +490,7 @@
 constexpr int SCATTER_CHUNKS = 16;
 __global__ void __launch_bounds__(256) k_lazy_scatter(const PairRec *__restrict__ pairs, int64_t NP, const unsigned long long *__restrict__ smask,
                                                       const int32_t *__restrict__ spos, const int64_t *__restrict__ seg_old,
-                                                      const int64_t *__restrict__ seg_new, PairRec *__restrict__ out)
+                                                      const int64_t *__restrict__ seg_new, PairRec *__restrict__ out, int32_t *__restrict__ src)
 {
   const int lane = threadIdx.x & 63;
   const int64_t nch = (NP + 63) >> 6;
@@ -504,6 +504,7 @@
     const PairRec pr = pairs[i];
     const int32_t rank = spos[c] + (int32_t)__popcll(m & ((1ull << lane) - 1ull)) - spos[seg_old[pr.prof] >> 6];
     out[seg_new[pr.prof] + (int64_t)rank] = pr;
+    if (src) src[seg_new[pr.prof] + (int64_t)rank] = (int32_t)i;
   }
 }
 
@@ -587,10 +588,10 @@
   }
 }
 void launch_lazy_scatter(const PairRec *pairs, int64_t NP, const unsigned long long *smask, const int32_t *spos, const int64_t *seg_old, const int64_t *seg_new,
-                         PairRec *out, hipStream_t st)
+                         PairRec *out, hipStream_t st, int32_t *src)
 {
   const int64_t nch = (NP + 63) >> 6, per_block = 4 * SCATTER_CHUNKS;
-  if (NP > 0) hipLaunchKernelGGL(k_lazy_scatter, dim3((unsigned)((nch + per_block - 1) / per_block)), dim3(256), 0, st, pairs, NP, smask, spos, seg_old, seg_new, out);
+  if (NP > 0) hipLaunchKernelGGL(k_lazy_scatter, dim3((unsigned)((nch + per_block - 1) / per_block)), dim3(256), 0, st, pairs, NP, smask, spos, seg_old, seg_new, out, src);
 }
 void launch_finalize_lazy(itsx_domain *dom, int64_t n, const int64_t *zlb, const int64_t *zub, double domE, const int32_t *usample, int P, hipStream_t st)
 {
@@ -698,4 +699,48 @@
   hipLaunchKernelGGL(k_topup_mark, dim3(select_grid(NP)), dim3(256), 0, st, pairs, NP, done, b10, slot_of_prof, cutoff, smask, scnt);
 }
 
-}
+__global__ void __launch_bounds__(256) k_topup_defer(PairOut *__restrict__ pout, const int32_t *__restrict__ mrcnt, const int32_t *__restrict__ src, int64_t npairs,
+                                                     uint8_t *__restrict__ done, unsigned long long *__restrict__ dmask, unsigned long long *__restrict__ n)
+{
+  const int64_t pi = (int64_t)blockIdx.x * blockDim.x + threadIdx.x;
+  if (pi >= npairs || mrcnt[pi] <= 0) return;
+  pout[pi].ndom = 0;
+  const int64_t i = src[pi];
+  done[i] = 0;
+  const unsigned long long bit = 1ull << (i & 63);
+  atomicAdd(&n[(atomicOr(&dmask[i >> 6], bit) & bit) ? 1 : 0], 1ull);
+}
+__global__ void __launch_bounds__(256) k_topup_deferred_select(const unsigned long long *__restrict__ dmask, int64_t nch, unsigned long long *__restrict__ smask,
+                                                               int32_t *__restrict__ scnt, uint8_t *__restrict__ done)
+{
+  const int64_t c = (int64_t)blockIdx.x * blockDim.x + threadIdx.x;
+  if (c > nch) return;
+  unsigned long long m = c < nch ? dmask[c] : 0ull;
+  smask[c] = m; scnt[c] = (int32_t)__popcll(m);
+  while (m) { const int b = __ffsll((long long)m) - 1; done[c * 64 + b] = 1; m &= m - 1; }
+}
+__global__ void __launch_bounds__(256) k_topup_count_mask(const unsigned long long *__restrict__ dmask, const int64_t *__restrict__ seg_start, const int32_t *__restrict__ total,
+                                                          const int32_t *__restrict__ prof_of_slot, unsigned long long *__restrict__ cnt)
+{
+  const int sl = blockIdx.y, p = prof_of_slot[sl];
+  const int64_t c0 = seg_start[p] >> 6, n = ((int64_t)total[p] + 63) >> 6;
+  unsigned long long c = 0;
+  for (int64_t i = (int64_t)blockIdx.x * 256 + threadIdx.x; i < n; i += (int64_t)gridDim.x * 256) c += (unsigned long long)__popcll(dmask[c0 + i]);
+  for (int o = 32; o >= 1; o >>= 1) c += __shfl_xor(c, o, 64);
+  if ((threadIdx.x & 63) == 0 && c) atomicAdd(&cnt[sl], c);
+}
+void launch_topup_count_mask(const unsigned long long *dmask, const int64_t *seg_start, const int32_t *total, const int32_t *prof_of_slot, int nslots, unsigned long long *cnt, hipStream_t st)
+{
+  if (nslots > 0) hipLaunchKernelGGL(k_topup_count_mask, dim3(64, (unsigned)nslots), dim3(256), 0, st, dmask, seg_start, total, prof_of_slot, cnt);
+}
+void launch_topup_defer(PairOut *pout, const int32_t *mrcnt, const int32_t *src, int64_t npairs, uint8_t *done, unsigned long long *dmask, unsigned long long *n, hipStream_t st)
+{
+  if (npairs > 0) hipLaunchKernelGGL(k_topup_defer, dim3((unsigned)((npairs + 255) / 256)), dim3(256), 0, st, pout, mrcnt, src, npairs, done, dmask, n);
+}
+void launch_topup_deferred_select(const unsigned long long *dmask, int64_t NP, unsigned long long *smask, int32_t *scnt, uint8_t *done, hipStream_t st)
+{
+  const int64_t nch = (NP + 63) >> 6;
+  hipLaunchKernelGGL(k_topup_deferred_select, dim3((unsigned)((nch + 1 + 255) / 256)), dim3(256), 0, st, dmask, nch, smask, scnt, done);
+}
+
+}
diff --git a/itsxpress_amd/csrc/switches.cpp b/itsxpress_amd/csrc/switches.cpp
--- a/itsxpress_amd/csrc/switches.cpp
+++ b/itsxpress_amd/csrc/switches.cpp
@@ -15,6 +15,7 @@
   {"ITSX_PASSA_DBG", SW_HOOK, "pass A diagnostic bits (no rows / no restore / no join): timings only, scores are garbage; 64: the shared MSV kernel counts its floored wave-rows, those with the xB branch and its waves by word layout (results unchanged; one stderr line per search)"},
   {"ITSX_MSV_PB", SW_HOOK, "profiles one block of the MSV filter takes its sequences through (1 .. 32; default: by the job's size, 1 for a small job): same cells"},
   {"ITSX_TWRITER_HOST_SLICE", SW_HOOK, "=1: a streamed writer with a device (itsx_twriter_set_device) slices every unit on the host, as it does a unit its line index does not fit (same file bytes)"},
+  {"ITSX_TOPUP_FORCE_SECOND", SW_HOOK, "=1: the top-up round's second sub-round (the deferred pairs through the ensemble stage) runs as if the count-only sub-round had left rows undecided (same rows)"},
   {"ITSX_ROWS", SW_MODE, "rows mode when the caller did not call itsx_set_rows_mode: full | compact | lazy (coordinates identical in all three)"},
   {"ITSX_COMPACT_ROWS", SW_MODE, "=1: rows mode compact (older spelling of ITSX_ROWS=compact)"},
   {"ITSX_QMASK", SW_MODE, "=none: vsearch's --qmask none for cluster_size / orient seeds (default dust, as vsearch)"},
@@ -58,7 +59,8 @@
   {"ITSX_MR_LONG_FRAC", SW_TUNING, "ensemble stage: share of regions taken as 'long'"},
   {"ITSX_MR_LONG_LANES", SW_TUNING, "ensemble stage: lanes per long region"},
   {"ITSX_MSV_BWD_WHOLE", SW_TUNING, "=1: the MSV filter's Backward chains copy their whole read to LDS first (A/B arm: same cells)"},
-  {"ITSX_LAZY_TOPUP_ALL", SW_TUNING, "=0: a profile whose undecided rows need most of its pairs is left to the full count (itsx_lazy_complete) instead of taking all its unevaluated pairs in the top-up round (same rows)"},
+  {"ITSX_LAZY_TOPUP_ALL", SW_TUNING, "=0: a profile whose undecided rows need most of its pairs is left to the full count (itsx_lazy_complete) instead of taking all its unevaluated pairs in the top-up round; =2 (with the count-only round): such a profile takes what its row needs like any other, and its remaining pairs follow in a count-only sub-round of their own only if the row is still undecided (same coordinates; read at every call)"},
+  {"ITSX_TOPUP_COUNT_ONLY", SW_TUNING, "=0: the top-up round sends its pairs through the whole domain pipeline like a third lazy round (rows kept, an ensemble invocation of its own) instead of counting reported targets only and deferring the pairs with a multidomain region (A/B arm and cross-check: same coordinates)"},
   {"ITSX_MR_WAVES", SW_TUNING, "ensemble stage: waves a batch is spread over (lanes per wave = regions / this, 2 .. 64); 0 = waves of 64 lanes"},
   {"ITSX_MR_ONE_MAX", SW_TUNING, "ensemble stage: a batch of at most this many regions (default 2048) is walked one region per wave with the matrix in LDS; 0 = never"},
   {"ITSX_CIGAR_MB", SW_TUNING, "itsx_align_clusters: byte budget of one batch of pairs (direction bits and border rows), MB (default 2048; a small value forces several batches, and a pair larger than it runs alone: same alignments)"},
diff --git a/itsxpress_amd/engine.py b/itsxpress_amd/engine.py
--- a/itsxpress_amd/engine.py
+++ b/itsxpress_amd/engine.py
@@ -704,7 +704,11 @@
     def stats(self):
         s = np.zeros(1, STATS_DTYPE_ALL)
         self._chk(self.L.itsx_get_stats(self.h, s.ctypes.data, STATS_DTYPE_ALL.itemsize))
-        return {k: (s[0][k].item() if s[0][k].ndim == 0 else s[0][k].tolist()) for k in STATS_DTYPE_ALL.names}
+        out = {k: (s[0][k].item() if s[0][k].ndim == 0 else s[0][k].tolist()) for k in STATS_DTYPE_ALL.names}
+        t = np.zeros(2, np.int64)
+        self._chk(self.L.itsx_topup_counters(self.h, t.ctypes.data))
+        out["n_topup_deferred"], out["n_topup_ensemble"] = int(t[0]), int(t[1])
+        return out
 
     def release_scratch(self):
         self._chk(self.L.itsx_release_scratch(self.h))
```
